# TrevorS/voxtral-mini-realtime-rs

Hardware: NVIDIA H100
Metric: decode_tokens_per_sec (higher is better)
Workload: dtype f32

## Files before the change

### voxtral_mini_realtime_rs_b200/csrc/capi.cu

```cuda
#include <cuda_profiler_api.h>
#include <cuda_runtime.h>

#include <cstring>
#include <memory>
#include <string>
#include <vector>

#include "audio_host.h"
#include "common.h"
#include "gguf.h"
#include "kernels.h"
#include "model.h"
#include "stream.h"
#include "tokenizer.h"

namespace vox {
static thread_local std::string g_last_error;
void set_last_error(const std::string &m) { g_last_error = m; }
}

using namespace vox;

#define VOX_API_BEGIN try {
#define VOX_API_END                                \
    }                                              \
    catch (const vox::Error &e) {                  \
        vox::set_last_error(e.what());             \
        return e.code;                             \
    }                                              \
    catch (const std::bad_alloc &) {               \
        vox::set_last_error("out of host memory"); \
        return VOX_ENOMEM;                         \
    }                                              \
    catch (const std::exception &e) {              \
        vox::set_last_error(e.what());             \
        return VOX_EINVAL;                         \
    }                                              \
    return VOX_OK;

#define REQUIRE(p) VOX_CHECK((p) != nullptr, VOX_EINVAL, "null argument: " #p)

struct vox_gguf { Gguf *g; };
struct vox_mel {
    int device;
    DeviceArena arena;
    MelTables tables;
    cudaStream_t st = nullptr;
    float *in = nullptr, *out = nullptr;
    size_t in_cap = 0, out_cap = 0;
};
struct vox_q4 {
    int device;
    DeviceArena arena;
    Q4Weight w;
    float *x = nullptr, *y = nullptr, *bias = nullptr;
    size_t x_cap = 0, y_cap = 0;
    TcWork wk;
    void *xt = nullptr;
    size_t xt_elems = 0;
    GemmWork gw;
};
struct vox_model { Model *m; };
struct vox_session { Session *s; };
struct vox_tokenizer { Tokenizer *t; };
struct vox_stream_pool { StreamPool *p; };

static void require_device(int device) {
    int n = 0;
    cudaError_t e = cudaGetDeviceCount(&n);
    VOX_CHECK(e == cudaSuccess && n > 0, VOX_ECUDA, "no CUDA device available (%s); this library has no CPU fallback",
              cudaGetErrorString(e));
    VOX_CHECK(device >= 0 && device < n, VOX_EINVAL, "device %d out of range (have %d)", device, n);
    CUDA_OK(cudaSetDevice(device));
}

extern "C" {

const char *vox_last_error(void) { return g_last_error.c_str(); }
int32_t vox_version(void) { return 100; }
int32_t vox_device_count(void) {
    int n = 0;
    if (cudaGetDeviceCount(&n) != cudaSuccess) { cudaGetLastError(); return 0; }
    return n;
}

int32_t vox_gguf_open(const char *path, vox_gguf **out) {
    VOX_API_BEGIN
    REQUIRE(path); REQUIRE(out);
    Gguf *g = Gguf::open_file(path);
    *out = new vox_gguf{g};
    VOX_API_END
}
int32_t vox_gguf_open_shards(const void *const *bufs, const size_t *lens, size_t n, vox_gguf **out) {
    VOX_API_BEGIN
    REQUIRE(bufs); REQUIRE(lens); REQUIRE(out);
    Gguf *g = Gguf::open_shards(bufs, lens, n);
    *out = new vox_gguf{g};
    VOX_API_END
}
int32_t vox_gguf_version(const vox_gguf *g, uint32_t *v) {
    VOX_API_BEGIN
    REQUIRE(g); REQUIRE(v);
    *v = g->g->version();
    VOX_API_END
}
int32_t vox_gguf_tensor_count(const vox_gguf *g, uint64_t *c) {
    VOX_API_BEGIN
    REQUIRE(g); REQUIRE(c);
    *c = g->g->tensor_count();
    VOX_API_END
}
int32_t vox_gguf_tensor_name(const vox_gguf *g, uint64_t i, const char **name) {
    VOX_API_BEGIN
    REQUIRE(g); REQUIRE(name);
    VOX_CHECK(i < g->g->names().size(), VOX_EINVAL, "tensor index %llu out of range", (unsigned long long)i);
    *name = g->g->names()[(size_t)i].c_str();
    VOX_API_END
}
int32_t vox_gguf_tensor_info(const vox_gguf *g, const char *name, uint32_t *dtype, uint32_t *ndim, uint64_t dims[4],
                             uint64_t *nbytes) {
    VOX_API_BEGIN
    REQUIRE(g); REQUIRE(name);
    const GgufTensorInfo *t = g->g->find(name);
    VOX_CHECK(t != nullptr, VOX_ENOTFOUND, "Tensor '%s' not found in GGUF", name);
    if (dtype) *dtype = t->dtype;
    if (ndim) *ndim = (uint32_t)t->dims.size();
    if (dims)
        for (size_t i = 0; i < 4; ++i) dims[i] = i < t->dims.size() ? t->dims[i] : 1;
    if (nbytes) *nbytes = t->byte_size();
    VOX_API_END
}
int32_t vox_gguf_tensor_data(vox_gguf *g, const char *name, void *dst, size_t cap) {
    VOX_API_BEGIN
    REQUIRE(g); REQUIRE(name); REQUIRE(dst);
    const GgufTensorInfo *t = g->g->find(name);
    VOX_CHECK(t != nullptr, VOX_ENOTFOUND, "Tensor '%s' not found in GGUF", name);
    VOX_CHECK(cap >= t->byte_size(), VOX_ECAPACITY, "buffer too small for '%s' (%zu < %llu)", name, cap,
              (unsigned long long)t->byte_size());
    g->g->read_tensor(*t, dst);
    VOX_API_END
}
void vox_gguf_close(vox_gguf *g) {
    if (!g) return;
    delete g->g;
    delete g;
}

int32_t vox_peak_normalize(float *s, size_t n, float target) {
    VOX_API_BEGIN
    if (n) REQUIRE(s);
    peak_normalize(s, n, target);
    VOX_API_END
}
void vox_pad_config_default(vox_pad_config *c) { if (c) pad_config_default(c); }
size_t vox_pad_audio_len(size_t n, const vox_pad_config *cfg) {
    vox_pad_config c;
    if (cfg) c = *cfg; else pad_config_default(&c);
    return pad_audio_len(n, c);
}
int32_t vox_pad_audio(const float *in, size_t n, const vox_pad_config *cfg, float *out, size_t cap, size_t *out_len) {
    VOX_API_BEGIN
    REQUIRE(out);
    if (n) REQUIRE(in);
    vox_pad_config c;
    if (cfg) c = *cfg; else pad_config_default(&c);
    VOX_CHECK(c.frame_rate > 0 && c.sample_rate > 0, VOX_EINVAL, "bad pad config");
    const size_t total = pad_audio_len(n, c);
    VOX_CHECK(cap >= total, VOX_ECAPACITY, "pad_audio: capacity %zu < %zu", cap, total);
    memset(out, 0, sizeof(float) * total);
    if (n) memcpy(out + pad_left(c), in, sizeof(float) * n);
    if (out_len) *out_len = total;
    VOX_API_END
}
int32_t vox_chunk_plan(size_t n, size_t max_mel_frames, size_t overlap, vox_chunk *out, size_t cap, size_t *n_chunks) {
    VOX_API_BEGIN
    REQUIRE(n_chunks);
    std::vector<vox_chunk> v = chunk_plan(n, max_mel_frames, overlap);
    *n_chunks = v.size();
    if (out) {
        VOX_CHECK(cap >= v.size(), VOX_ECAPACITY, "chunk_plan: capacity %zu < %zu", cap, v.size());
        for (size_t i = 0; i < v.size(); ++i) out[i] = v[i];
    }
    VOX_API_END
}
int32_t vox_stream_progress(size_t n_samples, int32_t ended, int32_t reshape_factor, int32_t prefix_len, int64_t out[5]) {
    VOX_API_BEGIN
    REQUIRE(out);
    VOX_CHECK(reshape_factor > 0 && prefix_len > 0, VOX_EINVAL, "stream_progress: reshape_factor %d / prefix_len %d must be positive",
              reshape_factor, prefix_len);
    stream_progress(n_samples, ended != 0, reshape_factor, prefix_len, out);
    VOX_API_END
}
int32_t vox_time_embedding(float t, int32_t dim, float *out) {
    VOX_API_BEGIN
    REQUIRE(out);
    VOX_CHECK(dim > 0 && dim % 2 == 0, VOX_EINVAL, "time_embedding: dim %d must be even", dim);
    time_embedding(t, dim, out);
    VOX_API_END
}

int32_t vox_mel_create(int32_t device, vox_mel **out) {
    VOX_API_BEGIN
    REQUIRE(out);
    require_device(device);
    std::unique_ptr<vox_mel> m(new vox_mel());
    m->device = device;
    m->arena.device = device;
    m->tables.build(m->arena);
    CUDA_OK(cudaStreamCreateWithFlags(&m->st, cudaStreamNonBlocking));
    *out = m.release();
    VOX_API_END
}
size_t vox_mel_num_frames(size_t n) { return mel_num_frames(n); }
int32_t vox_mel_compute_log(vox_mel *mel, const float *samples, size_t n, float *out, size_t cap) {
    VOX_API_BEGIN
    REQUIRE(mel); REQUIRE(out);
    if (n) REQUIRE(samples);
    const size_t frames = mel_num_frames(n);
    VOX_CHECK(cap >= frames * kMelBins, VOX_ECAPACITY, "mel: capacity %zu < %zu", cap, frames * kMelBins);
    if (frames == 0) return VOX_OK;
    CUDA_OK(cudaSetDevice(mel->device));
    if (n > mel->in_cap) {
        mel->in = mel->arena.alloc_n<float>(n);
        mel->in_cap = n;
    }
    if (frames * kMelBins > mel->out_cap) {
        mel->out = mel->arena.alloc_n<float>(frames * kMelBins);
        mel->out_cap = frames * kMelBins;
    }
    CUDA_OK(cudaMemcpyAsync(mel->in, samples, sizeof(float) * n, cudaMemcpyHostToDevice, mel->st));
    launch_mel(mel->in, 1, n, n, mel->tables.window, mel->tables.fb_vals, mel->tables.fb_start, mel->tables.fb_len,
               mel->tables.fb_stride, mel->out, (int)frames, 0, mel->st);
    CUDA_OK(cudaMemcpyAsync(out, mel->out, sizeof(float) * frames * kMelBins, cudaMemcpyDeviceToHost, mel->st));
    CUDA_OK(cudaStreamSynchronize(mel->st));
    VOX_API_END
}
int32_t vox_mel_compute_log_dev(vox_mel *mel, const float *samples_dev, size_t n, float *out_dev, int32_t layout,
                                void *stream) {
    VOX_API_BEGIN
    REQUIRE(mel); REQUIRE(samples_dev); REQUIRE(out_dev);
    VOX_CHECK(layout == 0 || layout == 1, VOX_EINVAL, "mel layout must be 0 or 1");
    CUDA_OK(cudaSetDevice(mel->device));
    const size_t frames = mel_num_frames(n);
    launch_mel(samples_dev, 1, n, n, mel->tables.window, mel->tables.fb_vals, mel->tables.fb_start, mel->tables.fb_len,
               mel->tables.fb_stride, out_dev, (int)frames, layout, stream ? (cudaStream_t)stream : mel->st);
    VOX_API_END
}
int32_t vox_mel_filterbank(const vox_mel *mel, float *out) {
    VOX_API_BEGIN
    REQUIRE(mel); REQUIRE(out);
    memcpy(out, mel->tables.fb_dense.data(), sizeof(float) * kMelBins * kMelFreqs);
    VOX_API_END
}
int32_t vox_mel_window(const vox_mel *mel, float *out) {
    VOX_API_BEGIN
    REQUIRE(mel); REQUIRE(out);
    memcpy(out, mel->tables.window_host.data(), sizeof(float) * kMelNfft);
    VOX_API_END
}
void vox_mel_free(vox_mel *mel) {
    if (!mel) return;
    cudaSetDevice(mel->device);
    if (mel->st) cudaStreamDestroy(mel->st);
    delete mel;
}

int32_t vox_q4_tensor_create(const uint8_t *bytes, size_t nbytes, int64_t n, int64_t k, int32_t device, vox_q4 **out) {
    VOX_API_BEGIN
    REQUIRE(bytes); REQUIRE(out);
    VOX_CHECK(n > 0 && k > 0, VOX_EINVAL, "Q4 tensor shape must be positive");
    VOX_CHECK((n * k) % 32 == 0, VOX_EINVAL, "Q4_0 requires element count divisible by 32, got %lld", (long long)(n * k));
    VOX_CHECK(k % 32 == 0, VOX_EINVAL, "Q4_0 rows must be block aligned: K=%lld is not a multiple of 32", (long long)k);
    const size_t expect = (size_t)(n * k / 32) * 18;
    VOX_CHECK(nbytes == expect, VOX_EINVAL, "Q4_0 byte count mismatch: expected %zu for %lld blocks, got %zu", expect,
              (long long)(n * k / 32), nbytes);
    require_device(device);
    std::unique_ptr<vox_q4> q(new vox_q4());
    q->device = device;
    q->arena.device = device;
    q->w = upload_q4(q->arena, {bytes}, {(int)n}, (int)k, false, true);
    q->wk = q4_matvec_tc_work_size(q->w.N, q->w.K);
    alloc_split_k(q->arena, q->wk);
    *out = q.release();
    VOX_API_END
}
int32_t vox_q4_tensor_shape(const vox_q4 *w, int64_t *n, int64_t *k) {
    VOX_API_BEGIN
    REQUIRE(w);
    if (n) *n = w->w.N;
    if (k) *k = w->w.K;
    VOX_API_END
}
int32_t vox_q4_tensor_dequantize(const vox_q4 *w, float *out) {
    VOX_API_BEGIN
    REQUIRE(w); REQUIRE(out);
    CUDA_OK(cudaSetDevice(w->device));
    const size_t nb = (size_t)w->w.N * (w->w.K / 32);
    std::vector<uint8_t> qs(nb * 16);
    std::vector<__half> ds(nb);
    CUDA_OK(cudaMemcpy(qs.data(), w->w.qs, qs.size(), cudaMemcpyDeviceToHost));
    CUDA_OK(cudaMemcpy(ds.data(), w->w.d, ds.size() * sizeof(__half), cudaMemcpyDeviceToHost));
    for (size_t b = 0; b < nb; ++b) {
        const float d = __half2float(ds[b]);
        for (int i = 0; i < 16; ++i) {
            const uint8_t byte = qs[b * 16 + i];
            out[b * 32 + i] = ((float)(byte & 0xF) - 8.0f) * d;
            out[b * 32 + i + 16] = ((float)(byte >> 4) - 8.0f) * d;
        }
    }
    VOX_API_END
}
static Q4Path g_q4_path = {!(getenv("VOX_MATVEC") && std::string(getenv("VOX_MATVEC")) == "simt"), true};
static Q4Scratch q4_scratch(vox_q4 *h, int rows) {
    if (rows > 8) {
        const size_t need = gemm_tc5_split_elems(rows, h->w.K);
        if (need > h->xt_elems) {
            h->xt = h->arena.alloc(need * 2);
            h->xt_elems = need;
        }
        if (!h->gw.partial) {
            h->gw = gemm_tc5_work_size();
            alloc_split_k(h->arena, h->gw);
        }
    }
    return Q4Scratch{h->xt, h->xt_elems, &h->gw, &h->wk};
}
int32_t vox_q4_set_matvec_mode(int32_t mode) {
    VOX_API_BEGIN
    VOX_CHECK(mode >= 0 && mode <= 3, VOX_EINVAL, "mode bits: 1 = SIMT matvec (M<=8), 2 = SIMT GEMM (M>8)");
    g_q4_path.matvec_tc = (mode & 1) == 0;
    g_q4_path.gemm_tc = (mode & 2) == 0;
    VOX_API_END
}
int32_t vox_q4_matmul(const vox_q4 *w, const float *x_dev, float *y_dev, int32_t b, int32_t m, const float *bias_dev,
                      void *stream) {
    VOX_API_BEGIN
    REQUIRE(w); REQUIRE(x_dev); REQUIRE(y_dev);
    VOX_CHECK(b > 0 && m > 0, VOX_EINVAL, "q4_matmul: B and M must be positive");
    CUDA_OK(cudaSetDevice(w->device));
    launch_q4_linear(w->w, x_dev, b * m, y_dev, w->w.N, bias_dev, nullptr, EPI_NONE, nullptr, nullptr, 0.0f, nullptr,
                     q4_scratch(const_cast<vox_q4 *>(w), b * m), g_q4_path, (cudaStream_t)stream);
    VOX_API_END
}
int32_t vox_q4_matmul_host(const vox_q4 *wc, const float *x, float *y, int32_t b, int32_t m, const float *bias) {
    VOX_API_BEGIN
    vox_q4 *w = const_cast<vox_q4 *>(wc);
    REQUIRE(w); REQUIRE(x); REQUIRE(y);
    VOX_CHECK(b > 0 && m > 0, VOX_EINVAL, "q4_matmul: B and M must be positive");
    CUDA_OK(cudaSetDevice(w->device));
    const size_t rows = (size_t)b * m, xn = rows * w->w.K, yn = rows * w->w.N;
    if (xn > w->x_cap) { w->x = w->arena.alloc_n<float>(xn); w->x_cap = xn; }
    if (yn > w->y_cap) { w->y = w->arena.alloc_n<float>(yn); w->y_cap = yn; }
    if (bias && !w->bias) w->bias = w->arena.alloc_n<float>(w->w.N);
    CUDA_OK(cudaMemcpyAsync(w->x, x, sizeof(float) * xn, cudaMemcpyHostToDevice, 0));
    if (bias) CUDA_OK(cudaMemcpyAsync(w->bias, bias, sizeof(float) * w->w.N, cudaMemcpyHostToDevice, 0));
    launch_q4_linear(w->w, w->x, (int)rows, w->y, w->w.N, bias ? w->bias : nullptr, nullptr, EPI_NONE, nullptr, nullptr,
                     0.0f, nullptr, q4_scratch(w, (int)rows), g_q4_path, 0);
    CUDA_OK(cudaMemcpyAsync(y, w->y, sizeof(float) * yn, cudaMemcpyDeviceToHost, 0));
    CUDA_OK(cudaStreamSynchronize(0));
    VOX_API_END
}
void vox_q4_tensor_free(vox_q4 *w) {
    if (!w) return;
    cudaSetDevice(w->device);
    delete w;
}

int32_t vox_dev_malloc(int32_t device, size_t bytes, void **p) {
    VOX_API_BEGIN
    REQUIRE(p);
    require_device(device);
    cudaError_t e = cudaMalloc(p, bytes ? bytes : 16);
    VOX_CHECK(e == cudaSuccess, VOX_ENOMEM, "cudaMalloc(%zu) failed: %s", bytes, cudaGetErrorString(e));
    VOX_API_END
}
int32_t vox_dev_free(int32_t device, void *p) {
    VOX_API_BEGIN
    require_device(device);
    CUDA_OK(cudaFree(p));
    VOX_API_END
}
int32_t vox_dev_upload(int32_t device, void *dst, const void *src, size_t bytes) {
    VOX_API_BEGIN
    require_device(device);
    CUDA_OK(cudaMemcpy(dst, src, bytes, cudaMemcpyHostToDevice));
    VOX_API_END
}
int32_t vox_dev_download(int32_t device, void *dst, const void *src, size_t bytes) {
    VOX_API_BEGIN
    require_device(device);
    CUDA_OK(cudaMemcpy(dst, src, bytes, cudaMemcpyDeviceToHost));
    VOX_API_END
}
int32_t vox_dev_sync(int32_t device) {
    VOX_API_BEGIN
    require_device(device);
    CUDA_OK(cudaDeviceSynchronize());
    VOX_API_END
}
int32_t vox_profiler_start(void) {
    VOX_API_BEGIN
    CUDA_OK(cudaProfilerStart());
    VOX_API_END
}
int32_t vox_profiler_stop(void) {
    VOX_API_BEGIN
    CUDA_OK(cudaProfilerStop());
    VOX_API_END
}
int32_t vox_host_alloc_pinned(size_t bytes, void **p) {
    VOX_API_BEGIN
    REQUIRE(p);
    cudaError_t e = cudaHostAlloc(p, bytes ? bytes : 16, cudaHostAllocDefault);
    VOX_CHECK(e == cudaSuccess, VOX_ECUDA, "cudaHostAlloc(%zu) failed: %s", bytes, cudaGetErrorString(e));
    VOX_API_END
}
int32_t vox_host_free_pinned(void *p) {
    VOX_API_BEGIN
    CUDA_OK(cudaFreeHost(p));
    VOX_API_END
}
int32_t vox_q4_matmul_bench(const vox_q4 *const *ws, int32_t n_w, int32_t m, int32_t iters, int32_t warmup, float *avg_ms) {
    VOX_API_BEGIN
    REQUIRE(ws); REQUIRE(avg_ms);
    VOX_CHECK(n_w > 0 && m > 0 && iters > 0, VOX_EINVAL, "bad bench arguments");
    const vox_q4 *w0 = ws[0];
    CUDA_OK(cudaSetDevice(w0->device));
    DeviceArena arena;
    arena.device = w0->device;
    const int K = w0->w.K, N = w0->w.N;
    std::vector<float> hx((size_t)m * K);
    for (size_t i = 0; i < hx.size(); ++i) hx[i] = sinf((float)i * 0.001f) * 0.1f;
    float *x = arena.upload(hx.data(), hx.size());
    float *y = arena.alloc_n<float>((size_t)m * N);
    cudaStream_t st;
    CUDA_OK(cudaStreamCreateWithFlags(&st, cudaStreamNonBlocking));
    cudaEvent_t e0, e1;
    CUDA_OK(cudaEventCreate(&e0));
    CUDA_OK(cudaEventCreate(&e1));
    auto run = [&](int i) {
        launch_q4_linear(ws[i % n_w]->w, x, m, y, ws[i % n_w]->w.N, nullptr, nullptr, EPI_NONE, nullptr, nullptr, 0.0f, nullptr,
                         Q4Scratch{}, g_q4_path, st);
    };
    for (int i = 0; i < warmup; ++i) run(i);
    CUDA_OK(cudaStreamSynchronize(st));
    CUDA_OK(cudaEventRecord(e0, st));
    for (int i = 0; i < iters; ++i) run(i);
    CUDA_OK(cudaEventRecord(e1, st));
    CUDA_OK(cudaStreamSynchronize(st));
    float ms = 0;
    CUDA_OK(cudaEventElapsedTime(&ms, e0, e1));
    *avg_ms = ms / iters;
    cudaEventDestroy(e0);
    cudaEventDestroy(e1);
    cudaStreamDestroy(st);
    VOX_API_END
}

int32_t vox_model_load_gguf_handle(vox_gguf *g, int32_t device, vox_model **out) {
    VOX_API_BEGIN
    REQUIRE(g); REQUIRE(out);
    Model *m = Model::load(*g->g, device);
    *out = new vox_model{m};
    VOX_API_END
}
int32_t vox_model_load_gguf(const char *path, int32_t device, vox_model **out) {
    VOX_API_BEGIN
    REQUIRE(path); REQUIRE(out);
    std::unique_ptr<Gguf> g(Gguf::open_file(path));
    Model *m = Model::load(*g, device);
    *out = new vox_model{m};
    VOX_API_END
}
int32_t vox_model_get_info(const vox_model *m, vox_model_info *info) {
    VOX_API_BEGIN
    REQUIRE(m); REQUIRE(info);
    *info = m->m->info;
    VOX_API_END
}
void vox_model_free(vox_model *m) {
    if (!m) return;
    cudaSetDevice(m->m->device);
    delete m->m;
    delete m;
}

int32_t vox_session_create(vox_model *m, int32_t max_batch, int32_t max_mel_frames, vox_session **out) {
    VOX_API_BEGIN
    REQUIRE(m); REQUIRE(out);
    Session *s = Session::create(m->m, max_batch, max_mel_frames);
    *out = new vox_session{s};
    VOX_API_END
}
int32_t vox_session_set_delay(vox_session *s, float delay) {
    VOX_API_BEGIN
    REQUIRE(s);
    s->s->set_delay(delay);
    VOX_API_END
}
static void require_any_device();
int32_t vox_session_set_delays(vox_session *s, const float *delays, int32_t b) {
    VOX_API_BEGIN
    require_any_device();
    REQUIRE(s); REQUIRE(delays);
    s->s->set_delays(delays, b);
    VOX_API_END
}

static void upload_mel(Session *s, const float *mel, int b, int t) {
    const vox_model_info &c = s->m->info;
    VOX_CHECK(b >= 1 && b <= s->max_batch, VOX_EINVAL, "batch %d exceeds session max_batch %d", b, s->max_batch);
    VOX_CHECK(t >= 1 && t <= s->max_mel_frames, VOX_EINVAL, "mel frames %d exceed session max_mel_frames %d", t,
              s->max_mel_frames);
    CUDA_OK(cudaSetDevice(s->m->device));
    CUDA_OK(cudaMemcpyAsync(s->mel, mel, sizeof(float) * (size_t)b * c.n_mels * t, cudaMemcpyHostToDevice, s->st));
    launch_transpose_mel(s->mel, s->mel_tm, b, c.n_mels, t, s->st);
}

int32_t vox_encode_audio(vox_session *sh, const float *mel, int32_t b, int32_t t, float *audio_embeds, size_t cap,
                         int32_t *seq_len) {
    VOX_API_BEGIN
    REQUIRE(sh); REQUIRE(mel);
    Session *s = sh->s;
    upload_mel(s, mel, b, t);
    s->encode(b, t);
    const size_t n = (size_t)b * s->cur_S4 * s->m->info.dec_dim;
    if (audio_embeds) {
        VOX_CHECK(cap >= n, VOX_ECAPACITY, "audio_embeds capacity %zu < %zu", cap, n);
        if (n) CUDA_OK(cudaMemcpyAsync(audio_embeds, s->audio, sizeof(float) * n, cudaMemcpyDeviceToHost, s->st));
    }
    CUDA_OK(cudaStreamSynchronize(s->st));
    if (seq_len) *seq_len = s->cur_S4;
    VOX_API_END
}

static void fill_timings(Session *s, vox_timings *tm) {
    if (!tm) return;
    float pre = 0, enc = 0, dec = 0, pf = 0;
    CUDA_OK(cudaEventElapsedTime(&pf, s->ev[2], s->ev[4]));
    tm->prefill_ms = pf;
    CUDA_OK(cudaEventElapsedTime(&pre, s->ev[0], s->ev[1]));
    CUDA_OK(cudaEventElapsedTime(&enc, s->ev[1], s->ev[2]));
    CUDA_OK(cudaEventElapsedTime(&dec, s->ev[2], s->ev[3]));
    tm->preprocess_ms = pre;
    tm->encode_ms = enc;
    tm->decode_ms = dec;
    tm->total_ms = pre + enc + dec;
}

int32_t vox_transcribe_streaming(vox_session *sh, const float *mel, int32_t b, int32_t t, int32_t *out_ids, size_t cap,
                                 int32_t *n_out, vox_timings *tm) {
    VOX_API_BEGIN
    REQUIRE(sh); REQUIRE(mel); REQUIRE(out_ids); REQUIRE(n_out);
    Session *s = sh->s;
    CUDA_OK(cudaSetDevice(s->m->device));
    CUDA_OK(cudaEventRecord(s->ev[0], s->st));
    upload_mel(s, mel, b, t);
    CUDA_OK(cudaEventRecord(s->ev[1], s->st));
    *n_out = s->transcribe_from_mel(b, t, out_ids, cap, tm, true);
    fill_timings(s, tm);
    VOX_API_END
}

static int32_t transcribe_pcm_impl(Session *s, const float *host, const float *dev, int b, size_t n, int normalize,
                                   int32_t *out_ids, size_t cap, int32_t *n_out, vox_timings *tm) {
    const vox_model_info &c = s->m->info;
    VOX_CHECK(b >= 1 && b <= s->max_batch, VOX_EINVAL, "batch %d exceeds session max_batch %d", b, s->max_batch);
    VOX_CHECK(n >= 1, VOX_EINVAL, "empty audio");
    CUDA_OK(cudaSetDevice(s->m->device));
    vox_pad_config pc;
    pad_config_default(&pc);
    const size_t padded = pad_audio_len(n, pc), left = pad_left(pc);
    const size_t frames = mel_num_frames(padded);
    VOX_CHECK(frames >= 1, VOX_EINVAL, "Audio too short to produce mel frames");
    VOX_CHECK(frames <= (size_t)s->max_mel_frames, VOX_EINVAL,
              "audio needs %zu mel frames > session max_mel_frames %d (chunk it: vox_chunk_plan)", frames, s->max_mel_frames);
    if ((size_t)b * padded > s->pcm_pad_cap) {
        s->pcm_pad = s->arena.alloc_n<float>((size_t)b * padded);
        s->pcm_pad_cap = (size_t)b * padded;
    }
    CUDA_OK(cudaEventRecord(s->ev[0], s->st));
    const float *src = dev;
    if (host) {
        if ((size_t)b * n > s->pcm_cap) {
            s->pcm = s->arena.alloc_n<float>((size_t)b * n);
            s->pcm_cap = (size_t)b * n;
        }
        CUDA_OK(cudaMemcpyAsync(s->pcm, host, sizeof(float) * (size_t)b * n, cudaMemcpyHostToDevice, s->st));
        src = s->pcm;
    }
    launch_peak_normalize_pad(src, b, n, 0.95f, normalize, s->pcm_pad, padded, left, s->peak_scale, s->st);
    launch_mel(s->pcm_pad, b, padded, padded, s->m->mel.window, s->m->mel.fb_vals, s->m->mel.fb_start, s->m->mel.fb_len,
               s->m->mel.fb_stride, s->mel_tm, (int)frames, 0, s->st);
    CUDA_OK(cudaEventRecord(s->ev[1], s->st));
    (void)c;
    *n_out = s->transcribe_from_mel(b, (int)frames, out_ids, cap, tm, true);
    fill_timings(s, tm);
    return VOX_OK;
}

int32_t vox_transcribe_pcm(vox_session *sh, const float *samples, int32_t b, size_t n, int32_t normalize,
                           int32_t *out_ids, size_t cap, int32_t *n_out, vox_timings *tm) {
    VOX_API_BEGIN
    REQUIRE(sh); REQUIRE(samples); REQUIRE(out_ids); REQUIRE(n_out);
    return transcribe_pcm_impl(sh->s, samples, nullptr, b, n, normalize, out_ids, cap, n_out, tm);
    VOX_API_END
}
int32_t vox_transcribe_pcm_dev(vox_session *sh, const float *samples_dev, int32_t b, size_t n, int32_t *out_ids,
                               size_t cap, int32_t *n_out, vox_timings *tm) {
    VOX_API_BEGIN
    REQUIRE(sh); REQUIRE(samples_dev); REQUIRE(out_ids); REQUIRE(n_out);
    return transcribe_pcm_impl(sh->s, nullptr, samples_dev, b, n, 1, out_ids, cap, n_out, tm);
    VOX_API_END
}

int32_t vox_generate_step_with_cache(vox_session *sh, const int32_t *ids, int32_t b, int32_t m, float *logits, size_t cap) {
    VOX_API_BEGIN
    REQUIRE(sh); REQUIRE(ids); REQUIRE(logits);
    Session *s = sh->s;
    const vox_model_info &c = s->m->info;
    VOX_CHECK(b >= 1 && b <= s->max_batch, VOX_EINVAL, "batch %d exceeds session max_batch %d", b, s->max_batch);
    VOX_CHECK(m >= 1 && m <= s->M_max, VOX_EINVAL, "M=%d out of range [1,%d]", m, s->M_max);
    VOX_CHECK(s->cache_len + m <= s->out_ld, VOX_EINVAL, "KV cache full (%d + %d > %d)", s->cache_len, m, s->out_ld);
    for (int i = 0; i < b * m; ++i)
        VOX_CHECK(ids[i] >= 0 && ids[i] < c.vocab, VOX_EINVAL, "token id %d out of range", ids[i]);
    const size_t n = (size_t)b * m * c.vocab;
    VOX_CHECK(cap >= n, VOX_ECAPACITY, "logits capacity %zu < %zu", cap, n);
    CUDA_OK(cudaSetDevice(s->m->device));
    if (n > s->logits_all_cap) {
        s->logits_all = s->arena.alloc_n<float>(n);
        s->logits_all_cap = n;
    }
    CUDA_OK(cudaMemcpyAsync(s->d_ids, ids, sizeof(int) * (size_t)b * m, cudaMemcpyHostToDevice, s->st));
    launch_embed(s->m->tok_emb, s->d_ids, nullptr, 0, b, m, nullptr, s->x_dec, s->fused_decode(b * m) ? s->ssq_x : nullptr, s->st);
    const bool pending = s->decoder_forward(b, m);
    s->lm_head_rows(b * m, pending, s->logits_all);
    launch_advance(s->d_pos, m, nullptr, 0, b, s->st);
    CUDA_OK(cudaMemcpyAsync(logits, s->logits_all, sizeof(float) * n, cudaMemcpyDeviceToHost, s->st));
    CUDA_OK(cudaStreamSynchronize(s->st));
    s->cache_len += m;
    VOX_API_END
}
int32_t vox_forward_streaming(vox_session *sh, const float *mel, int32_t b, int32_t t, const int32_t *ids, int32_t n_ids,
                              float *logits, size_t cap) {
    VOX_API_BEGIN
    REQUIRE(sh); REQUIRE(mel); REQUIRE(ids); REQUIRE(logits);
    Session *s = sh->s;
    const vox_model_info &c = s->m->info;
    upload_mel(s, mel, b, t);
    s->encode(b, t);
    const int S4 = s->cur_S4;
    VOX_CHECK(n_ids == S4, VOX_EINVAL, "forward_streaming needs one token id per audio position (%d), got %d", S4, n_ids);
    VOX_CHECK(S4 <= s->out_ld, VOX_EINVAL, "sequence %d exceeds the session KV capacity %d", S4, s->out_ld);
    for (int i = 0; i < b * n_ids; ++i) VOX_CHECK(ids[i] >= 0 && ids[i] < c.vocab, VOX_EINVAL, "token id %d out of range", ids[i]);
    const size_t n = (size_t)b * S4 * c.vocab;
    VOX_CHECK(cap >= n, VOX_ECAPACITY, "logits capacity %zu < %zu", cap, n);
    s->reset();
    const int Mc = s->M_max;
    const size_t chunk_floats = (size_t)b * Mc * c.vocab;
    if (chunk_floats > s->logits_all_cap) {
        s->logits_all = s->arena.alloc_n<float>(chunk_floats);
        s->logits_all_cap = chunk_floats;
    }
    std::vector<int> chunk_ids;
    for (int p0 = 0; p0 < S4; p0 += Mc) {
        const int m = std::min(Mc, S4 - p0);
        chunk_ids.resize((size_t)b * m);
        for (int bb = 0; bb < b; ++bb)
            for (int i = 0; i < m; ++i) chunk_ids[(size_t)bb * m + i] = ids[(size_t)bb * S4 + p0 + i];
        CUDA_OK(cudaMemcpyAsync(s->d_ids, chunk_ids.data(), sizeof(int) * chunk_ids.size(), cudaMemcpyHostToDevice, s->st));
        launch_embed(s->m->tok_emb, s->d_ids, s->audio, S4, b, m, s->d_pos, s->x_dec, s->fused_decode(b * m) ? s->ssq_x : nullptr, s->st);
        const bool pending = s->decoder_forward(b, m);
        s->lm_head_rows(b * m, pending, s->logits_all);
        launch_advance(s->d_pos, m, nullptr, 0, b, s->st);
        for (int bb = 0; bb < b; ++bb)
            CUDA_OK(cudaMemcpyAsync(logits + ((size_t)bb * S4 + p0) * c.vocab, s->logits_all + (size_t)bb * m * c.vocab,
                                    sizeof(float) * (size_t)m * c.vocab, cudaMemcpyDeviceToHost, s->st));
        CUDA_OK(cudaStreamSynchronize(s->st));
    }
    s->cache_len = S4;
    VOX_API_END
}

static void record_step_scores(Session *s, int b) {
    s->scores_k = s->top_k;
    s->scores_b = b;
    s->scores_n = 1;
    s->scores_pos.assign(s->out_rows.begin(), s->out_rows.begin() + b);
    for (int &p : s->scores_pos) p -= 1;
}

int32_t vox_prefill(vox_session *sh, const int32_t *ids, int32_t b, int32_t m, int32_t add_audio, int32_t *next_tok) {
    VOX_API_BEGIN
    REQUIRE(sh); REQUIRE(ids);
    Session *s = sh->s;
    const vox_model_info &c = s->m->info;
    VOX_CHECK(b >= 1 && b <= s->max_batch, VOX_EINVAL, "batch %d exceeds session max_batch %d", b, s->max_batch);
    VOX_CHECK(m >= 1 && m <= s->M_max, VOX_EINVAL, "M=%d out of range [1,%d]", m, s->M_max);
    VOX_CHECK(s->cache_len + m <= s->out_ld, VOX_EINVAL, "KV cache full (%d + %d > %d)", s->cache_len, m, s->out_ld);
    if (add_audio)
        VOX_CHECK(b == s->cur_B && s->cache_len + m <= s->cur_S4, VOX_EINVAL,
                  "add_audio: positions %d..%d need audio embeddings of %d streams (have %d positions for %d streams; call vox_encode_audio first)",
                  s->cache_len, s->cache_len + m, b, s->cur_S4, s->cur_B);
    for (int i = 0; i < b * m; ++i) VOX_CHECK(ids[i] >= 0 && ids[i] < c.vocab, VOX_EINVAL, "token id %d out of range", ids[i]);
    CUDA_OK(cudaSetDevice(s->m->device));
    s->prefill(b, m, ids, add_audio != 0);
    s->cache_len += m;
    record_step_scores(s, b);
    if (next_tok) CUDA_OK(cudaMemcpyAsync(next_tok, s->d_tok, sizeof(int) * b, cudaMemcpyDeviceToHost, s->st));
    CUDA_OK(cudaStreamSynchronize(s->st));
    VOX_API_END
}
int32_t vox_decode_step(vox_session *sh, const int32_t *tok, int32_t b, int32_t add_audio, int32_t *next_tok) {
    VOX_API_BEGIN
    REQUIRE(sh);
    Session *s = sh->s;
    const vox_model_info &c = s->m->info;
    VOX_CHECK(b >= 1 && b <= s->max_batch, VOX_EINVAL, "batch %d exceeds session max_batch %d", b, s->max_batch);
    VOX_CHECK(s->cache_len + 1 <= s->out_ld, VOX_EINVAL, "KV cache full (%d + 1 > %d)", s->cache_len, s->out_ld);
    if (add_audio)
        VOX_CHECK(b == s->cur_B && s->cache_len < s->cur_S4, VOX_EINVAL,
                  "add_audio: position %d has no audio embedding (%d positions, %d streams encoded)", s->cache_len, s->cur_S4, s->cur_B);
    CUDA_OK(cudaSetDevice(s->m->device));
    if (tok) {
        for (int i = 0; i < b; ++i) VOX_CHECK(tok[i] >= 0 && tok[i] < c.vocab, VOX_EINVAL, "token id %d out of range", tok[i]);
        CUDA_OK(cudaMemcpyAsync(s->d_tok, tok, sizeof(int) * b, cudaMemcpyHostToDevice, s->st));
    }
    s->decode_step(b, add_audio != 0);
    s->mega_steps_host += 1;
    s->cache_len += 1;
    record_step_scores(s, b);
    if (next_tok) CUDA_OK(cudaMemcpyAsync(next_tok, s->d_tok, sizeof(int) * b, cudaMemcpyDeviceToHost, s->st));
    if (next_tok || tok) CUDA_OK(cudaStreamSynchronize(s->st));
    VOX_API_END
}
static_assert(VOX_MAX_TOP_K == TOPK_MAX, "the score buffers hold VOX_MAX_TOP_K entries per position");
int32_t vox_session_set_top_k(vox_session *s, int32_t k) {
    VOX_API_BEGIN
    REQUIRE(s);
    s->s->set_top_k(k);
    VOX_API_END
}
int32_t vox_session_token_scores(vox_session *sh, int32_t *top_ids, float *top_logprobs, size_t cap, int32_t *b, int32_t *n,
                                 int32_t *k) {
    VOX_API_BEGIN
// ... 327 lines not shown
```

### voxtral_mini_realtime_rs_b200/csrc/gemm_tc5.cu

```cuda
#include <cuda_fp16.h>

#include "common.h"
#include "kernels.h"

namespace vox {

void tc_count_launch(const char *name);

namespace {

constexpr int G5_WGS = 4;
constexpr int G5_THREADS = G5_WGS * 128;
constexpr int G5_BM = 128;
constexpr int G5_BN = 128;
constexpr int G5_BK = 64;
constexpr int G5_TILE_BYTES = G5_BM * G5_BK * 2;
constexpr int G5_PIECES = 2;
constexpr int G5_STAGES = 3;
constexpr int G5_STAGE_BYTES = 2 * G5_PIECES * G5_TILE_BYTES;
constexpr int G5_SMEM_BYTES = G5_STAGES * G5_STAGE_BYTES;
constexpr float G5_WSCALE = 256.0f;

__device__ __forceinline__ uint32_t smem_u32(const void *p) { return (uint32_t)__cvta_generic_to_shared(p); }
__device__ __forceinline__ void mbar_init(uint64_t *bar, uint32_t count) {
    asm volatile("mbarrier.init.shared::cta.b64 [%0], %1;\n" ::"r"(smem_u32(bar)), "r"(count));
}
__device__ __forceinline__ void mbar_expect_tx(uint64_t *bar, uint32_t bytes) {
    asm volatile("mbarrier.arrive.expect_tx.shared::cta.b64 _, [%0], %1;\n" ::"r"(smem_u32(bar)), "r"(bytes) : "memory");
}
__device__ __forceinline__ void mbar_wait(uint64_t *bar, uint32_t parity) {
    asm volatile(
        "{\n"
        ".reg .pred p;\n"
        "G5_WAIT:\n"
        "mbarrier.try_wait.parity.shared::cta.b64 p, [%0], %1;\n"
        "@p bra G5_DONE;\n"
        "bra G5_WAIT;\n"
        "G5_DONE:\n"
        "}\n" ::"r"(smem_u32(bar)), "r"(parity) : "memory");
}
__device__ __forceinline__ void bulk_g2s(void *dst_smem, const void *src_gmem, uint32_t bytes, uint64_t *bar) {
    asm volatile("cp.async.bulk.shared::cluster.global.mbarrier::complete_tx::bytes [%0], [%1], %2, [%3];\n" ::"r"(
                     smem_u32(dst_smem)),
                 "l"(src_gmem), "r"(bytes), "r"(smem_u32(bar))
                 : "memory");
}

__device__ __forceinline__ uint64_t gmma_desc(uint32_t smem_addr, uint32_t lbo_bytes, uint32_t sbo_bytes) {
    uint64_t d = 0;
    d |= (uint64_t)((smem_addr >> 4) & 0x3FFF);
    d |= (uint64_t)((lbo_bytes >> 4) & 0x3FFF) << 16;
    d |= (uint64_t)((sbo_bytes >> 4) & 0x3FFF) << 32;
    return d;
}
__device__ __forceinline__ void wgmma_m64n64k16(float (&d)[32], uint64_t adesc, uint64_t bdesc) {
    asm volatile(
        "{\n"
        ".reg .pred p;\n"
        "setp.ne.b32 p, %34, 0;\n"
        "wgmma.mma_async.sync.aligned.m64n64k16.f32.f16.f16 "
        "{%0,%1,%2,%3,%4,%5,%6,%7,%8,%9,%10,%11,%12,%13,%14,%15,%16,%17,%18,%19,%20,%21,%22,%23,%24,%25,%26,%27,%28,%29,%30,%31}, "
        "%32, %33, p, 1, 1, 0, 0;\n"
        "}\n"
        : "+f"(d[0]), "+f"(d[1]), "+f"(d[2]), "+f"(d[3]), "+f"(d[4]), "+f"(d[5]), "+f"(d[6]), "+f"(d[7]), "+f"(d[8]),
          "+f"(d[9]), "+f"(d[10]), "+f"(d[11]), "+f"(d[12]), "+f"(d[13]), "+f"(d[14]), "+f"(d[15]), "+f"(d[16]),
          "+f"(d[17]), "+f"(d[18]), "+f"(d[19]), "+f"(d[20]), "+f"(d[21]), "+f"(d[22]), "+f"(d[23]), "+f"(d[24]),
          "+f"(d[25]), "+f"(d[26]), "+f"(d[27]), "+f"(d[28]), "+f"(d[29]), "+f"(d[30]), "+f"(d[31])
        : "l"(adesc), "l"(bdesc), "r"(1)
        : "memory");
}
__device__ __forceinline__ void wgmma_fence() { asm volatile("wgmma.fence.sync.aligned;\n" ::: "memory"); }
__device__ __forceinline__ void wgmma_commit() { asm volatile("wgmma.commit_group.sync.aligned;\n" ::: "memory"); }
template <int N>
__device__ __forceinline__ void wgmma_wait() { asm volatile("wgmma.wait_group.sync.aligned %0;\n" ::"n"(N) : "memory"); }
__device__ __forceinline__ void acc_fence(float (&d)[32]) {
#pragma unroll
    for (int i = 0; i < 32; ++i) asm volatile("" : "+f"(d[i])::"memory");
}

__device__ __forceinline__ uint32_t g5_pack_f16x2(const float v0, const float v1) {
    const uint32_t b0 = __float_as_uint(v0), b1 = __float_as_uint(v1);
    const uint32_t em = ((b0 >> 13) & 0x00007FFFu) | ((b1 << 3) & 0x7FFF0000u);
    const uint32_t sg = ((b0 >> 16) & 0x00008000u) | (b1 & 0x80000000u);
    return em | sg;
}

struct G5Args {
    const uint4 *qs;
    const __half *ds;
    int N, K, M;
    const __half *xt;
    const float *oscale;
    int TT, KC;
    float *y;
    int ldy;
    const float *bias, *res;
    int SK, KCs;
    float *partial;
    int *counters;
};

template <int EPI>
__global__ void __launch_bounds__(G5_THREADS, 1) gemm_tc5_kernel(const G5Args a) {
    extern __shared__ __align__(1024) unsigned char smem[];
    __shared__ __align__(8) uint64_t full_bar[G5_STAGES];
    const int tid = threadIdx.x, warp = tid >> 5, lane = tid & 31, wg = tid >> 7;
    const int f0 = blockIdx.x * G5_BM, tt = blockIdx.y, tok0 = tt * G5_BN;
    const int bpr = a.K >> 5;
    const int kc_begin = blockIdx.z * a.KCs, kc_end = min(a.KC, kc_begin + a.KCs), nk = kc_end - kc_begin;
    const size_t xt_piece = (size_t)a.TT * a.KC * (G5_TILE_BYTES / 2);

    auto fetch_x = [&](int it) {
        const int s = it % G5_STAGES;
        unsigned char *dst = smem + (size_t)s * G5_STAGE_BYTES + G5_PIECES * G5_TILE_BYTES;
        mbar_expect_tx(&full_bar[s], G5_PIECES * G5_TILE_BYTES);
#pragma unroll
        for (int p = 0; p < G5_PIECES; ++p) {
            const __half *src = a.xt + p * xt_piece + ((size_t)tt * a.KC + kc_begin + it) * (G5_TILE_BYTES / 2);
            bulk_g2s(dst + p * G5_TILE_BYTES, src, G5_TILE_BYTES, &full_bar[s]);
        }
    };
    if (tid == 0) {
        for (int s = 0; s < G5_STAGES; ++s) mbar_init(&full_bar[s], 1);
        asm volatile("fence.mbarrier_init.release.cluster;\n" ::: "memory");
        if (nk > 0) fetch_x(0);
    }
    __syncthreads();

    const int drow = tid >> 2, dblk = (tid >> 1) & 1, dhalf = tid & 1;
    const int gn = f0 + drow;
    const int fq = wg & 1, tq = wg >> 1;
    float acc[32];
#pragma unroll
    for (int i = 0; i < 32; ++i) acc[i] = 0.0f;

    uint4 q_cur = make_uint4(0x88888888u, 0x88888888u, 0x88888888u, 0x88888888u);
    __half d_cur = __float2half(0.0f);
    if (gn < a.N && nk > 0) {
        const size_t blk = (size_t)gn * bpr + (size_t)kc_begin * 2 + dblk;
        q_cur = __ldg(a.qs + blk);
        d_cur = __ldg(a.ds + blk);
    }
    for (int it = 0; it < nk; ++it) {
        const int kc = kc_begin + it, s = it % G5_STAGES;
        unsigned char *stage = smem + (size_t)s * G5_STAGE_BYTES;
        const uint4 q = q_cur;
        const float dd = __half2float(d_cur) * G5_WSCALE * 1.92592994438723585305597794258492732e-34f;
        if (gn < a.N && kc + 1 < kc_end) {
            const size_t blk = (size_t)gn * bpr + (size_t)(kc + 1) * 2 + dblk;
            q_cur = __ldg(a.qs + blk);
            d_cur = __ldg(a.ds + blk);
        }
        const uint32_t w4[4] = {q.x, q.y, q.z, q.w};
        uint32_t ph[8], pl[8];
#pragma unroll
        for (int wi = 0; wi < 4; ++wi) {
            const uint32_t nib = dhalf ? (w4[wi] >> 4) : w4[wi];
            float hi[4], lo[4];
#pragma unroll
            for (int t = 0; t < 4; ++t) {
                const uint32_t n = (nib >> (8 * t)) & 0xFu;
                const float w = __fmul_rn(__fsub_rn(__uint_as_float(0x4B000000u | n), 8388616.0f), dd);
                const float c = __fmul_rn(w, 8193.0f);
                hi[t] = __fsub_rn(c, __fsub_rn(c, w));
                lo[t] = __fsub_rn(w, hi[t]);
            }
            ph[wi * 2 + 0] = g5_pack_f16x2(hi[0], hi[1]);
            ph[wi * 2 + 1] = g5_pack_f16x2(hi[2], hi[3]);
            pl[wi * 2 + 0] = g5_pack_f16x2(lo[0], lo[1]);
            pl[wi * 2 + 1] = g5_pack_f16x2(lo[2], lo[3]);
        }
        wgmma_wait<1>();
        unsigned char *thi = stage, *tlo = stage + G5_TILE_BYTES;
#pragma unroll
        for (int c = 0; c < 2; ++c) {
            const int off = (dblk * 4 + dhalf * 2 + c) * (G5_BM * 16) + drow * 16;
            *reinterpret_cast<uint4 *>(thi + off) = make_uint4(ph[4 * c + 0], ph[4 * c + 1], ph[4 * c + 2], ph[4 * c + 3]);
            *reinterpret_cast<uint4 *>(tlo + off) = make_uint4(pl[4 * c + 0], pl[4 * c + 1], pl[4 * c + 2], pl[4 * c + 3]);
        }
        asm volatile("fence.proxy.async.shared::cta;\n" ::: "memory");
        __syncthreads();
        if (tid == 0 && it + 1 < nk) fetch_x(it + 1);
        mbar_wait(&full_bar[s], (uint32_t)((it / G5_STAGES) & 1));
        const uint32_t wbase = smem_u32(stage) + fq * 64 * 16, xbase = smem_u32(stage + G5_PIECES * G5_TILE_BYTES) + tq * 64 * 16;
        const uint32_t lbo = G5_BM * 16, sbo = 128;
        acc_fence(acc);
        wgmma_fence();
#pragma unroll
        for (int ks = 0; ks < G5_BK / 16; ++ks) {
            const uint32_t koff = (uint32_t)ks * 2u * lbo;
            const uint64_t whi = gmma_desc(wbase + 0 * G5_TILE_BYTES + koff, lbo, sbo);
            const uint64_t wlo = gmma_desc(wbase + 1 * G5_TILE_BYTES + koff, lbo, sbo);
            const uint64_t xh = gmma_desc(xbase + 0 * G5_TILE_BYTES + koff, lbo, sbo);
            const uint64_t xm = gmma_desc(xbase + 1 * G5_TILE_BYTES + koff, lbo, sbo);
            wgmma_m64n64k16(acc, wlo, xh);
            wgmma_m64n64k16(acc, whi, xm);
            wgmma_m64n64k16(acc, whi, xh);
        }
        wgmma_commit();
        acc_fence(acc);
    }
    wgmma_wait<0>();
    acc_fence(acc);

    {
        __shared__ int is_last;
        const int frow = fq * 64 + (warp & 3) * 16 + (lane >> 2);
        const int tcol = tq * 64 + (lane & 3) * 2;
        auto fr = [&](int i) { return frow + ((i >> 1) & 1) * 8; };
        auto tc = [&](int i) { return tcol + (i >> 2) * 8 + (i & 1); };
        auto emit = [&](float (&r)[32]) {
#pragma unroll
            for (int i = 0; i < 32; ++i) {
                const int feat = f0 + fr(i), tok = tok0 + tc(i);
                float v = r[i] * a.oscale[tok];
                if (EPI == EPI_SILU_MUL) {
                    const float other = __shfl_xor_sync(0xffffffffu, v, 4);
                    if (((lane >> 2) & 1) == 0 && tok < a.M && feat + 1 < a.N)
                        a.y[(size_t)tok * a.ldy + (feat >> 1)] = (v / (1.0f + expf(-v))) * other;
                } else if (tok < a.M && feat < a.N) {
                    if (a.bias) v += a.bias[feat];
                    if (EPI == EPI_RESIDUAL) v += a.res[(size_t)tok * a.ldy + feat];
                    if (EPI == EPI_GELU) v = 0.5f * v * (1.0f + erff(v * 0.70710678118654752440f));
                    a.y[(size_t)tok * a.ldy + feat] = v;
                }
            }
        };
        if (a.SK <= 1) {
            emit(acc);
        } else {
            const int tile_id = blockIdx.y * gridDim.x + blockIdx.x, n_tile = gridDim.x * gridDim.y;
            float *ptile = a.partial + ((size_t)blockIdx.z * n_tile + tile_id) * (G5_BM * G5_BN);
#pragma unroll
            for (int i = 0; i < 32; ++i) __stcg(ptile + (size_t)tc(i) * G5_BM + fr(i), acc[i]);
            __syncthreads();
            if (tid == 0) {
                __threadfence();
                const int old = atomicAdd(&a.counters[tile_id], 1);
                const int last = (old == a.SK - 1);
                if (last) {
                    a.counters[tile_id] = 0;
                    __threadfence();
                }
                is_last = last;
            }
            __syncthreads();
            if (is_last != 0) {
#pragma unroll
                for (int i = 0; i < 32; ++i) {
                    float v = 0.0f;
                    for (int z = 0; z < a.SK; ++z)
                        v += __ldcg(a.partial + ((size_t)z * n_tile + tile_id) * (G5_BM * G5_BN) + (size_t)tc(i) * G5_BM + fr(i));
                    acc[i] = v;
                }
                emit(acc);
            }
        }
    }
}

template <bool ROWS>
__device__ __forceinline__ void split_tiles_body(const float *__restrict__ x, int M, int K, const float *__restrict__ gamma,
                                                 const float *__restrict__ ada_shared, const AdaRows &ada_rows, float eps,
                                                 __half *__restrict__ xt, float *__restrict__ oscale, int TT, int KC, int BN) {
    __shared__ float ssq_part[32][8], max_part[32][8];
    __shared__ float rms_s[8], sc_s[8];
    const int r8 = threadIdx.x & 7, cth = threadIdx.x >> 3;
    const int row = blockIdx.x * 8 + r8;
    const int nchunk = K >> 3;
    const bool valid = row < M;
    const float *xr = x + (size_t)(valid ? row : 0) * K;
    const float *__restrict__ ada = ROWS ? (valid ? ada_rows.row(row) : nullptr) : ada_shared;
    {
        float ssq = 0.0f, mx = 0.0f;
        if (valid)
            for (int c = cth; c < nchunk; c += 32) {
                const float4 v0 = *reinterpret_cast<const float4 *>(xr + c * 8);
                const float4 v1 = *reinterpret_cast<const float4 *>(xr + c * 8 + 4);
                float v[8] = {v0.x, v0.y, v0.z, v0.w, v1.x, v1.y, v1.z, v1.w};
#pragma unroll
                for (int e = 0; e < 8; ++e) {
                    ssq = fmaf(v[e], v[e], ssq);
                    float g = v[e];
                    if (gamma) {
                        g *= gamma[c * 8 + e];
                        if (ada) g *= ada[c * 8 + e];
                    }
                    mx = fmaxf(mx, fabsf(g));
                }
            }
        ssq_part[cth][r8] = ssq;
        max_part[cth][r8] = mx;
        __syncthreads();
        if (threadIdx.x < 8) {
            float s = 0.0f, m = 0.0f;
            for (int i = 0; i < 32; ++i) {
                s += ssq_part[i][threadIdx.x];
                m = fmaxf(m, max_part[i][threadIdx.x]);
            }
            const float rms = gamma ? sqrtf(s / (float)K + eps) : 1.0f;
            rms_s[threadIdx.x] = rms;
            m = m / rms * 1.0001f;
            int e = (int)((__float_as_uint(m) >> 23) & 0xFF) - 127;
            if (!(m > 0.0f) || m > 3.0e38f) e = 7;
            e = e < -100 ? -100 : (e > 100 ? 100 : e);
            sc_s[threadIdx.x] = __uint_as_float((uint32_t)(7 - e + 127) << 23);
            const int grow = blockIdx.x * 8 + threadIdx.x;
            oscale[grow] = __uint_as_float((uint32_t)(e - 7 - 8 + 127) << 23);
        }
        __syncthreads();
    }
    const float rms = rms_s[r8], sc = sc_s[r8];
    const int tt = row / BN, rin = row % BN;
    const size_t tile_el = (size_t)BN * G5_BK;
    const size_t piece = (size_t)TT * KC * tile_el;
    for (int c = cth; c < nchunk; c += 32) {
        float v[8] = {0.f, 0.f, 0.f, 0.f, 0.f, 0.f, 0.f, 0.f};
        if (valid) {
            const float4 v0 = *reinterpret_cast<const float4 *>(xr + c * 8);
            const float4 v1 = *reinterpret_cast<const float4 *>(xr + c * 8 + 4);
            v[0] = v0.x; v[1] = v0.y; v[2] = v0.z; v[3] = v0.w; v[4] = v1.x; v[5] = v1.y; v[6] = v1.z; v[7] = v1.w;
            if (gamma) {
#pragma unroll
                for (int e = 0; e < 8; ++e) {
                    v[e] = (v[e] / rms) * gamma[c * 8 + e];
                    if (ada) v[e] *= ada[c * 8 + e];
                }
            }
        }
        uint32_t p[2][4];
#pragma unroll
        for (int e = 0; e < 4; ++e) {
            const float f0 = v[2 * e] * sc, f1 = v[2 * e + 1] * sc;
            const __half2 h = __floats2half2_rn(f0, f1);
            const float2 hf = __half22float2(h);
            const __half2 m = __floats2half2_rn(f0 - hf.x, f1 - hf.y);
            p[0][e] = *reinterpret_cast<const uint32_t *>(&h);
            p[1][e] = *reinterpret_cast<const uint32_t *>(&m);
        }
        const size_t off = ((size_t)tt * KC + (c >> 3)) * tile_el + (size_t)((c & 7) * BN + rin) * 8;
#pragma unroll
        for (int s = 0; s < G5_PIECES; ++s)
            *reinterpret_cast<uint4 *>(xt + s * piece + off) = make_uint4(p[s][0], p[s][1], p[s][2], p[s][3]);
    }
}

__global__ void __launch_bounds__(256) split_tiles_kernel(const float *__restrict__ x, int M, int K, const float *__restrict__ gamma,
                                                          const float *__restrict__ ada, float eps, __half *__restrict__ xt,
                                                          float *__restrict__ oscale, int TT, int KC, int BN) {
    split_tiles_body<false>(x, M, K, gamma, ada, AdaRows{}, eps, xt, oscale, TT, KC, BN);
}

__global__ void __launch_bounds__(256) split_tiles_rows_kernel(const float *__restrict__ x, int M, int K, const float *__restrict__ gamma,
                                                               const AdaRows ada_rows, float eps, __half *__restrict__ xt,
                                                               float *__restrict__ oscale, int TT, int KC, int BN) {
    split_tiles_body<true>(x, M, K, gamma, nullptr, ada_rows, eps, xt, oscale, TT, KC, BN);
}

}

bool gemm_tc5_supported(const Q4Weight &w, int M) { return w.N % G5_BM == 0 && w.K % G5_BK == 0 && M >= 1; }

static size_t g5_tiles_elems(int M, int K) {
    const size_t TT = (size_t)(M + G5_BN - 1) / G5_BN;
    return G5_PIECES * TT * (size_t)(K / G5_BK) * ((size_t)G5_BN * G5_BK);
}
size_t gemm_tc5_split_elems(int M, int K) {
    const size_t TT = (size_t)(M + G5_BN - 1) / G5_BN;
    return g5_tiles_elems(M, K) + 2 * TT * G5_BN + 16;
}
GemmWork gemm_tc5_work_size() {
    GemmWork w;
    w.partial_floats = (size_t)VOX_NUM_SMS * G5_BM * G5_BN;
    w.n_counters = 128;
    return w;
}
static float *g5_oscale_ptr(void *xt, int M, int K) {
    size_t off = g5_tiles_elems(M, K) * 2;
    off = (off + 15) & ~(size_t)15;
    return reinterpret_cast<float *>(reinterpret_cast<unsigned char *>(xt) + off);
}

void launch_split_tiles(const float *x, int M, int K, const float *gamma, const float *ada, float eps, void *xt,
                        cudaStream_t st, const AdaRows &ada_rows) {
    VOX_CHECK(K % G5_BK == 0, VOX_EINVAL, "split_tiles: K=%d not a multiple of 64", K);
    const int TT = (M + G5_BN - 1) / G5_BN, KC = K / G5_BK;
    if (ada_rows.rows)
        split_tiles_rows_kernel<<<TT * (G5_BN / 8), 256, 0, st>>>(x, M, K, gamma, ada_rows, eps, (__half *)xt, g5_oscale_ptr(xt, M, K),
                                                                  TT, KC, G5_BN);
    else
        split_tiles_kernel<<<TT * (G5_BN / 8), 256, 0, st>>>(x, M, K, gamma, ada, eps, (__half *)xt, g5_oscale_ptr(xt, M, K), TT, KC,
                                                             G5_BN);
    tc_count_launch("split_tiles");
}

void launch_q4_gemm_tc5(const Q4Weight &w, const void *xt, int M, float *y, int ldy, const float *bias, const float *res,
                        int epi, const GemmWork *gw, cudaStream_t st) {
    VOX_CHECK(gemm_tc5_supported(w, M), VOX_EINVAL, "gemm_tc5: unsupported shape N=%d K=%d", w.N, w.K);
    G5Args a{};
    a.qs = w.qs;
    a.ds = w.d;
    a.N = w.N;
    a.K = w.K;
    a.M = M;
    a.xt = (const __half *)xt;
    a.oscale = g5_oscale_ptr(const_cast<void *>(xt), M, w.K);
    a.TT = (M + G5_BN - 1) / G5_BN;
    a.KC = w.K / G5_BK;
    a.y = y;
    a.ldy = ldy;
    a.bias = bias;
    a.res = res;
    const size_t smem = (size_t)G5_SMEM_BYTES;
    const int tiles = (w.N / G5_BM) * a.TT;
    int SK = 1;
    if (gw && gw->partial && gw->counters && tiles < VOX_NUM_SMS * 2 / 3) {
        SK = VOX_NUM_SMS / tiles;
        SK = SK > 8 ? 8 : SK;
        while (SK > 1 && a.KC / SK < 4) --SK;
        while (SK > 1 && ((size_t)SK * tiles * G5_BM * G5_BN > gw->partial_floats || tiles > gw->n_counters)) --SK;
    }
    a.KCs = (a.KC + SK - 1) / SK;
    SK = (a.KC + a.KCs - 1) / a.KCs;
    a.SK = SK;
    a.partial = SK > 1 ? gw->partial : nullptr;
    a.counters = SK > 1 ? gw->counters : nullptr;
    dim3 grid(w.N / G5_BM, a.TT, SK);
#define G5_CASE(E)                                                                      \
    case E: {                                                                           \
        static SmemAttr attr;                                                           \
        smem_attr_check(ensure_dyn_smem(gemm_tc5_kernel<E>, smem, attr), "gemm_tc5");   \
        gemm_tc5_kernel<E><<<grid, G5_THREADS, smem, st>>>(a);                          \
        break;                                                                          \
    }
    switch (epi) {
        G5_CASE(EPI_NONE)
        G5_CASE(EPI_RESIDUAL)
        G5_CASE(EPI_SILU_MUL)
        G5_CASE(EPI_GELU)
        default: fail(VOX_EINVAL, "bad epilogue");
    }
#undef G5_CASE
    tc_count_launch("gemm_tc5");
}

}
```

### voxtral_mini_realtime_rs_b200/csrc/kernels.cu

```cuda
#include "kernels.h"

#include <atomic>
#include <cfloat>
#include <cmath>
#include <string>

#include "common.h"

namespace vox {

void smem_attr_check(cudaError_t e, const char *what) {
    if (e != cudaSuccess) fail(VOX_ECUDA, fmt("cudaFuncSetAttribute(%s, MaxDynamicSharedMemorySize): %s", what, cudaGetErrorString(e)));
}


static std::atomic<uint64_t> g_launches{0};
uint64_t kernel_launch_count() { return g_launches.load(); }
void add_graph_launches(int64_t n) { g_launches.fetch_add((uint64_t)n, std::memory_order_relaxed); }

static inline void post_launch(const char *name) {
    g_launches.fetch_add(1, std::memory_order_relaxed);
    cudaError_t e = cudaGetLastError();
    if (e != cudaSuccess) fail(VOX_ECUDA, fmt("%s launch failed: %s", name, cudaGetErrorString(e)));
}
// ... 135 lines not shown
                        y[(size_t)m * ldy + r1] = v;
                    }
                }
            }
        }
    };

    if (n_chunks == 1) {
        const int nb = stage(0);
        for (int rg = blockIdx.x; rg < n_rg; rg += gridDim.x) {
            float acc0[M], acc1[M];
#pragma unroll
            for (int m = 0; m < M; ++m) acc0[m] = acc1[m] = 0.0f;
            accumulate(rg, 0, nb, acc0, acc1);
            epilogue(rg, acc0, acc1);
        }
    } else {
        const int rg = blockIdx.x;
        float acc0[M], acc1[M];
#pragma unroll
        for (int m = 0; m < M; ++m) acc0[m] = acc1[m] = 0.0f;
        for (int c = 0; c < n_chunks; ++c) {
            const int nb = stage(c);
            accumulate(rg, c, nb, acc0, acc1);
            __syncthreads();
        }
        epilogue(rg, acc0, acc1);
    }
}

template <int M, int EPI>
static void matvec_launch_t(const Q4Weight &w, const float *x, float *y, int ldy, const float *bias,
                            const float *res, cudaStream_t st) {
    const int bpr = w.K / 32;
    const size_t budget = 96 * 1024;
    int kcb = (int)(budget / ((size_t)M * (XPAD + 1) * sizeof(float)));
    if (kcb >= bpr) kcb = bpr;
    else kcb = (kcb / 32) * 32;
    const int n_chunks = (bpr + kcb - 1) / kcb;
    const size_t smem = (size_t)M * kcb * (XPAD + 1) * sizeof(float);
    static SmemAttr attr;
    smem_attr_check(ensure_dyn_smem(q4_matvec_kernel<M, EPI>, 100 * 1024, attr), "q4_matvec");
    const int n_rg = (w.N + MV_ROWS - 1) / MV_ROWS;
    int grid = n_rg;
    if (n_chunks == 1 && grid > VOX_NUM_SMS * 8) grid = VOX_NUM_SMS * 8;
    q4_matvec_kernel<M, EPI><<<grid, MV_THREADS, smem, st>>>(w.qs, w.d, w.N, w.K, x, y, ldy, bias, res, kcb, n_chunks);
    post_launch("q4_matvec");
}

template <int M>
static void matvec_launch_m(const Q4Weight &w, const float *x, float *y, int ldy, const float *bias,
                            const float *res, int epi, cudaStream_t st) {
    switch (epi) {
        case EPI_NONE: matvec_launch_t<M, EPI_NONE>(w, x, y, ldy, bias, res, st); break;
        case EPI_RESIDUAL: matvec_launch_t<M, EPI_RESIDUAL>(w, x, y, ldy, bias, res, st); break;
        case EPI_SILU_MUL: matvec_launch_t<M, EPI_SILU_MUL>(w, x, y, ldy, bias, res, st); break;
        case EPI_GELU: matvec_launch_t<M, EPI_GELU>(w, x, y, ldy, bias, res, st); break;
        default: fail(VOX_EINVAL, "bad epilogue");
    }
}

void launch_q4_matvec(const Q4Weight &w, const float *x, int M, float *y, int ldy, const float *bias,
                      const float *res, int epi, cudaStream_t st) {
    VOX_CHECK(M >= 1 && M <= 8, VOX_EINVAL, "q4_matvec: M=%d out of range", M);
    VOX_CHECK(w.K % 32 == 0, VOX_EINVAL, "q4_matvec: K=%d not a multiple of 32", w.K);
    switch (M) {
        case 1: matvec_launch_m<1>(w, x, y, ldy, bias, res, epi, st); break;
        case 2: matvec_launch_m<2>(w, x, y, ldy, bias, res, epi, st); break;
        case 3: matvec_launch_m<3>(w, x, y, ldy, bias, res, epi, st); break;
        case 4: matvec_launch_m<4>(w, x, y, ldy, bias, res, epi, st); break;
        case 5: matvec_launch_m<5>(w, x, y, ldy, bias, res, epi, st); break;
        case 6: matvec_launch_m<6>(w, x, y, ldy, bias, res, epi, st); break;
        case 7: matvec_launch_m<7>(w, x, y, ldy, bias, res, epi, st); break;
        default: matvec_launch_m<8>(w, x, y, ldy, bias, res, epi, st); break;
    }
}

constexpr int GB_M = 64, GB_N = 64, GB_K = 32, GB_PAD = 4, GB_THREADS = 256;

struct GemmArgs {
    const float *a;
    int M, N, K, lda;
    const uint4 *qs;
    const __half *ds;
    const float *wf;
    float *y;
    int ldy;
    const float *bias;
    const float *res;
    int T_in, T_out, C_in;
    int t_off;
    int in0;
};

template <int BMODE, int AMODE, int EPI>
__global__ void __launch_bounds__(GB_THREADS) gemm_kernel(const GemmArgs p) {
    __shared__ __align__(16) float As[GB_K][GB_M + GB_PAD];
    __shared__ __align__(16) float Ws[GB_K][GB_N + GB_PAD];
    const int tid = threadIdx.x;
    const int tx = tid & 15, ty = tid >> 4;
    const int m0 = blockIdx.y * GB_M, n0 = blockIdx.x * GB_N;
    const int bpr = p.K >> 5;
    float c[4][4];
#pragma unroll
    for (int i = 0; i < 4; ++i)
#pragma unroll
        for (int j = 0; j < 4; ++j) c[i][j] = 0.0f;

    for (int k0 = 0; k0 < p.K; k0 += GB_K) {
#pragma unroll
        for (int it = 0; it < 2; ++it) {
            const int idx = tid + it * GB_THREADS;
            const int row = idx >> 3, kq = idx & 7;
            const int gm = m0 + row;
            float4 v = make_float4(0.f, 0.f, 0.f, 0.f);
            if (gm < p.M) {
                if (AMODE == 0) {
                    v = *reinterpret_cast<const float4 *>(p.a + (size_t)gm * p.lda + k0 + kq * 4);
                } else {
                    const int b = gm / p.T_out, t = gm - b * p.T_out;
                    const int tap = k0 / p.C_in, c0 = k0 - tap * p.C_in;
                    const int tin = 2 * (t + p.t_off) - 1 + tap;
                    if (tin >= 0 && tin < p.T_in)
                        v = *reinterpret_cast<const float4 *>(p.a + ((size_t)b * p.T_in + (tin - p.in0)) * p.C_in + c0 + kq * 4);
                }
            }
            As[kq * 4 + 0][row] = v.x;
            As[kq * 4 + 1][row] = v.y;
            As[kq * 4 + 2][row] = v.z;
            As[kq * 4 + 3][row] = v.w;
        }
        if (BMODE == 0) {
            const int row = tid >> 2, wi = tid & 3;
            const int gn = n0 + row;
            float lo[4] = {0.f, 0.f, 0.f, 0.f}, hi[4] = {0.f, 0.f, 0.f, 0.f};
            if (gn < p.N) {
                const size_t blk = (size_t)gn * bpr + (k0 >> 5);
                const uint32_t w = reinterpret_cast<const uint32_t *>(p.qs + blk)[wi];
                const float dd = __half2float(p.ds[blk]);
#pragma unroll
                for (int t = 0; t < 4; ++t) {
                    const uint32_t byte = (w >> (8 * t)) & 0xFFu;
                    lo[t] = ((float)(byte & 0xFu) - 8.0f) * dd;
                    hi[t] = ((float)(byte >> 4) - 8.0f) * dd;
                }
            }
#pragma unroll
            for (int t = 0; t < 4; ++t) {
                Ws[wi * 4 + t][row] = lo[t];
                Ws[16 + wi * 4 + t][row] = hi[t];
            }
        } else {
#pragma unroll
            for (int it = 0; it < 2; ++it) {
                const int idx = tid + it * GB_THREADS;
                const int row = idx >> 3, kq = idx & 7;
                const int gn = n0 + row;
                float4 v = make_float4(0.f, 0.f, 0.f, 0.f);
                if (gn < p.N) v = *reinterpret_cast<const float4 *>(p.wf + (size_t)gn * p.K + k0 + kq * 4);
                Ws[kq * 4 + 0][row] = v.x;
                Ws[kq * 4 + 1][row] = v.y;
                Ws[kq * 4 + 2][row] = v.z;
                Ws[kq * 4 + 3][row] = v.w;
            }
        }
        __syncthreads();
#pragma unroll
        for (int k = 0; k < GB_K; ++k) {
            const float4 a = *reinterpret_cast<const float4 *>(&As[k][ty * 4]);
            const float4 b = *reinterpret_cast<const float4 *>(&Ws[k][tx * 4]);
            const float av[4] = {a.x, a.y, a.z, a.w};
            const float bv[4] = {b.x, b.y, b.z, b.w};
#pragma unroll
            for (int i = 0; i < 4; ++i)
#pragma unroll
                for (int j = 0; j < 4; ++j) c[i][j] = fmaf(av[i], bv[j], c[i][j]);
        }
        __syncthreads();
    }
#pragma unroll
    for (int i = 0; i < 4; ++i) {
        const int gm = m0 + ty * 4 + i;
        if (gm >= p.M) continue;
        if (EPI == EPI_SILU_MUL) {
#pragma unroll
            for (int j = 0; j < 4; j += 2) {
                const int gn = n0 + tx * 4 + j;
                if (gn + 1 < p.N) p.y[(size_t)gm * p.ldy + (gn >> 1)] = silu_f(c[i][j]) * c[i][j + 1];
            }
        } else {
#pragma unroll
            for (int j = 0; j < 4; ++j) {
                const int gn = n0 + tx * 4 + j;
                if (gn >= p.N) continue;
                float v = c[i][j] + (p.bias ? p.bias[gn] : 0.0f);
                if (EPI == EPI_RESIDUAL) v += p.res[(size_t)gm * p.ldy + gn];
                if (EPI == EPI_GELU) v = gelu_erf(v);
                p.y[(size_t)gm * p.ldy + gn] = v;
            }
        }
    }
}

template <int BMODE, int AMODE>
static void gemm_launch(const GemmArgs &p, int epi, cudaStream_t st) {
    dim3 grid((p.N + GB_N - 1) / GB_N, (p.M + GB_M - 1) / GB_M);
    switch (epi) {
        case EPI_NONE: gemm_kernel<BMODE, AMODE, EPI_NONE><<<grid, GB_THREADS, 0, st>>>(p); break;
        case EPI_RESIDUAL: gemm_kernel<BMODE, AMODE, EPI_RESIDUAL><<<grid, GB_THREADS, 0, st>>>(p); break;
        case EPI_SILU_MUL: gemm_kernel<BMODE, AMODE, EPI_SILU_MUL><<<grid, GB_THREADS, 0, st>>>(p); break;
        case EPI_GELU: gemm_kernel<BMODE, AMODE, EPI_GELU><<<grid, GB_THREADS, 0, st>>>(p); break;
        default: fail(VOX_EINVAL, "bad epilogue");
    }
    post_launch("gemm");
}

void launch_q4_gemm(const Q4Weight &w, const float *a, int M, float *y, int ldy, const float *bias,
                    const float *res, int epi, cudaStream_t st) {
    VOX_CHECK(w.K % 32 == 0, VOX_EINVAL, "q4_gemm: K=%d not a multiple of 32", w.K);
    if (M <= 0) return;
    GemmArgs p{};
    p.a = a; p.M = M; p.N = w.N; p.K = w.K; p.lda = w.K;
    p.qs = w.qs; p.ds = w.d; p.y = y; p.ldy = ldy; p.bias = bias; p.res = res;
    gemm_launch<0, 0>(p, epi, st);
}

void launch_conv2_gemm(const float *in, const float *w, const float *bias, float *out, int B, int T_in,
                       int T_out, int C_in, int C_out, cudaStream_t st, int t_off, int in0) {
    VOX_CHECK(C_in % 32 == 0, VOX_EINVAL, "conv2: C_in=%d not a multiple of 32", C_in);
    VOX_CHECK((t_off == 0 && in0 == 0) || B == 1, VOX_EINVAL, "conv2: a frame offset needs B == 1");
    VOX_CHECK(in0 <= 2 * t_off - 1 || in0 == 0, VOX_EINVAL, "conv2: input row %d is no longer resident", 2 * t_off - 1);
    if (B * T_out <= 0) return;
    GemmArgs p{};
    p.a = in; p.M = B * T_out; p.N = C_out; p.K = 3 * C_in; p.lda = 0;
    p.wf = w; p.y = out; p.ldy = C_out; p.bias = bias; p.res = nullptr;
    p.T_in = T_in; p.T_out = T_out; p.C_in = C_in; p.t_off = t_off; p.in0 = in0;
    gemm_launch<1, 1>(p, EPI_GELU, st);
}

__global__ void transpose_mel_kernel(const float *__restrict__ in, float *__restrict__ out, int C, int T) {
    __shared__ float tile[32][33];
    const int b = blockIdx.z, c0 = blockIdx.y * 32, t0 = blockIdx.x * 32;
    for (int i = threadIdx.y; i < 32; i += blockDim.y) {
        const int c = c0 + i, t = t0 + threadIdx.x;
        tile[i][threadIdx.x] = (c < C && t < T) ? in[((size_t)b * C + c) * T + t] : 0.0f;
    }
    __syncthreads();
    for (int i = threadIdx.y; i < 32; i += blockDim.y) {
        const int t = t0 + i, c = c0 + threadIdx.x;
        if (t < T && c < C) out[((size_t)b * T + t) * C + c] = tile[threadIdx.x][i];
    }
}
void launch_transpose_mel(const float *in, float *out, int B, int C, int T, cudaStream_t st) {
    dim3 grid((T + 31) / 32, (C + 31) / 32, B), block(32, 8);
    transpose_mel_kernel<<<grid, block, 0, st>>>(in, out, C, T);
    post_launch("transpose_mel");
}

__device__ __forceinline__ void rmsnorm_row(const float *__restrict__ xr, const float *__restrict__ gamma,
                                            const float *__restrict__ scale, float *__restrict__ yr, int dim, float eps) {
    __shared__ float red[32];
    float s = 0.0f;
    for (int i = threadIdx.x; i < dim; i += blockDim.x) s = fmaf(xr[i], xr[i], s);
    s = warp_sum(s);
    if ((threadIdx.x & 31) == 0) red[threadIdx.x >> 5] = s;
    __syncthreads();
    if (threadIdx.x < 32) {
        float v = threadIdx.x < (blockDim.x >> 5) ? red[threadIdx.x] : 0.0f;
        v = warp_sum(v);
        if (threadIdx.x == 0) red[0] = v;
    }
    __syncthreads();
    const float rms = sqrtf(red[0] / (float)dim + eps);
    for (int i = threadIdx.x; i < dim; i += blockDim.x) {
        float v = (xr[i] / rms) * gamma[i];
        if (scale) v *= scale[i];
        yr[i] = v;
    }
}

__global__ void rmsnorm_kernel(const float *__restrict__ x, const float *__restrict__ gamma,
                               const float *__restrict__ scale, float *__restrict__ y, int dim, float eps) {
    rmsnorm_row(x + (size_t)blockIdx.x * dim, gamma, scale, y + (size_t)blockIdx.x * dim, dim, eps);
}

__global__ void rmsnorm_rows_kernel(const float *__restrict__ x, const float *__restrict__ gamma, const AdaRows ada_rows,
                                    float *__restrict__ y, int dim, float eps) {
    rmsnorm_row(x + (size_t)blockIdx.x * dim, gamma, ada_rows.row(blockIdx.x), y + (size_t)blockIdx.x * dim, dim, eps);
}

void launch_rmsnorm(const float *x, const float *gamma, const float *scale, float *y, int rows, int dim,
                    float eps, cudaStream_t st, const AdaRows &ada_rows) {
    if (rows <= 0) return;
    if (ada_rows.rows) rmsnorm_rows_kernel<<<rows, 256, 0, st>>>(x, gamma, ada_rows, y, dim, eps);
    else rmsnorm_kernel<<<rows, 256, 0, st>>>(x, gamma, scale, y, dim, eps);
    post_launch("rmsnorm");
}

void launch_q4_linear(const Q4Weight &w, const float *x, int M, float *y, int ldy, const float *bias, const float *res,
                      int epi, const float *gamma, const float *ada, float eps, float *tmp, const Q4Scratch &sc,
                      const Q4Path &path, cudaStream_t st, const AdaRows &ada_rows) {
    VOX_CHECK(!ada_rows.rows || (gamma && !ada), VOX_EINVAL, "q4_linear: per-row ADA vectors need a norm and no shared vector");
    if (M > 8 && path.gemm_tc && gemm_tc5_supported(w, M) && gemm_tc5_split_elems(M, w.K) <= sc.xt_elems) {
        launch_split_tiles(x, M, w.K, gamma, ada, gamma ? eps : 0.0f, sc.xt, st, ada_rows);
        launch_q4_gemm_tc5(w, sc.xt, M, y, ldy, bias, res, epi, sc.gw, st);
        return;
    }
    const bool tc = M <= 8 && path.matvec_tc && w.qs_tc;
    AdaRows rows = ada_rows;
    if (gamma && !(tc && sc.tc && sc.tc->ssq_in)) {
        launch_rmsnorm(x, gamma, ada, tmp, M, w.K, eps, st, rows);
        x = tmp;
        gamma = ada = nullptr;
        rows = AdaRows{};
    }
    if (tc) launch_q4_matvec_tc_ex(w, x, M, y, ldy, bias, res, epi, gamma, ada, gamma ? eps : 0.0f, sc.tc, st, rows);
    else if (M <= 8) launch_q4_matvec(w, x, M, y, ldy, bias, res, epi, st);
    else launch_q4_gemm(w, x, M, y, ldy, bias, res, epi, st);
}

__global__ void rope_inplace_kernel(float *buf, int ld, int q_off, int n_q, int k_off, int n_k, int hd,
                                    int seq, int pos0, const float *__restrict__ cos_t,
                                    const float *__restrict__ sin_t) {
    const int r = blockIdx.x;
    const int pos = pos0 + (r % seq);
    const int half = hd >> 1;
    float *row = buf + (size_t)r * ld;
    const int total = (n_q + n_k) * half;
    for (int i = threadIdx.x; i < total; i += blockDim.x) {
        const int h = i / half, p = i - h * half;
        float *v = (h < n_q) ? row + q_off + h * hd + 2 * p : row + k_off + (h - n_q) * hd + 2 * p;
        const float c = cos_t[(size_t)pos * half + p], s = sin_t[(size_t)pos * half + p];
        const float xr = v[0], xi = v[1];
        v[0] = xr * c - xi * s;
        v[1] = xr * s + xi * c;
    }
}

void launch_rope_inplace(float *buf, int rows, int ld, int q_off, int n_q, int k_off, int n_k, int hd,
                         int seq, int pos0, const float *cos_t, const float *sin_t, cudaStream_t st) {
    if (rows <= 0) return;
    rope_inplace_kernel<<<rows, 256, 0, st>>>(buf, ld, q_off, n_q, k_off, n_k, hd, seq, pos0, cos_t, sin_t);
    post_launch("rope");
}

constexpr int EA_BQ = 32, EA_BK = 64, EA_THREADS = 128;

template <int HD>
__global__ void __launch_bounds__(EA_THREADS)
enc_attention_kernel(const float *__restrict__ qkv, float *__restrict__ out, int S, int H, int ld, int q_off,
                     int k_off, int v_off, int window, float scale) {
    extern __shared__ __align__(16) float sm[];
    float *Qs = sm;
    float *Ks = Qs + EA_BQ * (HD + 1);
    float *Vs = Ks + EA_BK * (HD + 1);
    float *Ps = Vs + EA_BK * HD;
    const int b = blockIdx.z, h = blockIdx.y, q0 = blockIdx.x * EA_BQ;
    const int tid = threadIdx.x, r = tid >> 2, c = tid & 3;
    constexpr int DQ = HD / 4;
    const float *base = qkv + (size_t)b * S * ld;
    for (int i = tid; i < EA_BQ * HD; i += EA_THREADS) {
        const int rr = i / HD, d = i - rr * HD;
        const int gi = q0 + rr;
        Qs[rr * (HD + 1) + d] = gi < S ? base[(size_t)gi * ld + q_off + h * HD + d] : 0.0f;
    }
    const int gi = q0 + r;
    float o[DQ];
#pragma unroll
    for (int d = 0; d < DQ; ++d) o[d] = 0.0f;
    float m_run = -INFINITY, l_run = 0.0f;
    const int q_last = min(q0 + EA_BQ - 1, S - 1);
    int j_begin = q0 - window;
    if (j_begin < 0) j_begin = 0;
    j_begin = (j_begin / EA_BK) * EA_BK;
    for (int j0 = j_begin; j0 <= q_last; j0 += EA_BK) {
        __syncthreads();
        for (int i = tid; i < EA_BK * HD; i += EA_THREADS) {
            const int kk = i / HD, d = i - kk * HD;
            const int gj = j0 + kk;
            float kv = 0.0f, vv = 0.0f;
            if (gj < S) {
                kv = base[(size_t)gj * ld + k_off + h * HD + d];
                vv = base[(size_t)gj * ld + v_off + h * HD + d];
            }
            Ks[kk * (HD + 1) + d] = kv;
            Vs[kk * HD + d] = vv;
        }
        __syncthreads();
        float s[16];
        float m_t = -INFINITY;
#pragma unroll
        for (int jj = 0; jj < 16; ++jj) {
            const int kk = c + 4 * jj;
            const int gj = j0 + kk;
            const float *qr = Qs + r * (HD + 1);
            const float *kr = Ks + kk * (HD + 1);
            float acc = 0.0f;
#pragma unroll 16
            for (int d = 0; d < HD; ++d) acc = fmaf(qr[d], kr[d], acc);
            const bool valid = (gj < S) && (gj <= gi) && (gi - gj <= window);
            s[jj] = valid ? acc * scale : -INFINITY;
            m_t = fmaxf(m_t, s[jj]);
        }
        m_t = fmaxf(m_t, __shfl_xor_sync(0xffffffffu, m_t, 1));
        m_t = fmaxf(m_t, __shfl_xor_sync(0xffffffffu, m_t, 2));
        const float m_new = fmaxf(m_run, m_t);
        float alpha = 1.0f, psum = 0.0f;
        if (m_new == -INFINITY) {
#pragma unroll
            for (int jj = 0; jj < 16; ++jj) Ps[r * (EA_BK + 1) + c + 4 * jj] = 0.0f;
        } else {
            alpha = expf(m_run - m_new);
#pragma unroll
            for (int jj = 0; jj < 16; ++jj) {
                const float pv = expf(s[jj] - m_new);
                psum += pv;
                Ps[r * (EA_BK + 1) + c + 4 * jj] = pv;
            }
        }
        psum += __shfl_xor_sync(0xffffffffu, psum, 1);
        psum += __shfl_xor_sync(0xffffffffu, psum, 2);
        l_run = l_run * alpha + psum;
        m_run = m_new;
#pragma unroll
        for (int d = 0; d < DQ; ++d) o[d] *= alpha;
        __syncwarp();
        for (int kk = 0; kk < EA_BK; ++kk) {
            const float pv = Ps[r * (EA_BK + 1) + kk];
            const float *vr = Vs + kk * HD + c;
#pragma unroll
            for (int d = 0; d < DQ; ++d) o[d] = fmaf(pv, vr[4 * d], o[d]);
        }
    }
    if (gi < S) {
        const float inv = 1.0f / l_run;
        float *orow = out + ((size_t)b * S + gi) * (H * HD) + h * HD + c;
#pragma unroll
        for (int d = 0; d < DQ; ++d) orow[4 * d] = o[d] * inv;
    }
}

void launch_enc_attention(const float *qkv, float *out, int B, int S, int H, int hd, int ld, int q_off,
                          int k_off, int v_off, int window, float scale, cudaStream_t st) {
    if (S <= 0) return;
    dim3 grid((S + EA_BQ - 1) / EA_BQ, H, B);
    const size_t smem = (size_t)(EA_BQ * (hd + 1) + EA_BK * (hd + 1) + EA_BK * hd + EA_BQ * (EA_BK + 1)) * sizeof(float);
#define ENC_ATTN_CASE(HD)                                                                                   \
    case HD: {                                                                                              \
        static SmemAttr attr;                                                                               \
        smem_attr_check(ensure_dyn_smem(enc_attention_kernel<HD>, smem, attr), "enc_attention");              \
        enc_attention_kernel<HD><<<grid, EA_THREADS, smem, st>>>(qkv, out, S, H, ld, q_off, k_off, v_off,   \
                                                                 window, scale);                            \
        break;                                                                                              \
    }
    switch (hd) {
        ENC_ATTN_CASE(32)
        ENC_ATTN_CASE(64)
        ENC_ATTN_CASE(128)
        default: fail(VOX_EINVAL, fmt("enc_attention: unsupported head_dim %d", hd));
    }
#undef ENC_ATTN_CASE
    post_launch("enc_attention");
}

template <bool RING>
__global__ void dec_rope_append_kernel(float *qkv, int M, int ld, int H, int Hkv, int hd, const KvView kv, const RopeView rope) {
    const int i = blockIdx.x, b = blockIdx.y;
    const int pos = kv.pos[b] + i;
    if (!RING && pos >= kv.max_seq()) return;
    const int half = hd >> 1;
    float *row = qkv + ((size_t)b * M + i) * ld;
    const size_t rr = (size_t)(RING ? pos % rope.rows : pos) * half;
    const float *cr = rope.cos_t + rr, *sr = rope.sin_t + rr;
    for (int t = threadIdx.x; t < H * half; t += blockDim.x) {
        const int h = t / half, p = t - h * half;
        float *v = row + h * hd + 2 * p;
        const float xr = v[0], xi = v[1];
        v[0] = xr * cr[p] - xi * sr[p];
        v[1] = xr * sr[p] + xi * cr[p];
    }
    const float *krow = row + H * hd;
    const float *vrow = krow + Hkv * hd;
    for (int t = threadIdx.x; t < Hkv * half; t += blockDim.x) {
        const int h = t / half, p = t - h * half;
        const float xr = krow[h * hd + 2 * p], xi = krow[h * hd + 2 * p + 1];
        float *dst = kv.k + kv_index<RING>(kv, b, Hkv, h, pos, hd) + 2 * p;
        dst[0] = xr * cr[p] - xi * sr[p];
        dst[1] = xr * sr[p] + xi * cr[p];
    }
    for (int t = threadIdx.x; t < Hkv * hd; t += blockDim.x) {
        const int h = t / hd, d = t - h * hd;
        kv.v[kv_index<RING>(kv, b, Hkv, h, pos, hd) + d] = vrow[t];
    }
}

void launch_dec_rope_append(float *qkv, int B, int M, int ld, int H, int Hkv, int hd, const KvView &kv,
                            const RopeView &rope, cudaStream_t st) {
    dim3 grid(M, B);
    if (kv.ring) dec_rope_append_kernel<true><<<grid, 256, 0, st>>>(qkv, M, ld, H, Hkv, hd, kv, rope);
    else dec_rope_append_kernel<false><<<grid, 256, 0, st>>>(qkv, M, ld, H, Hkv, hd, kv, rope);
    post_launch("dec_rope_append");
}

template <bool RING>
__global__ void dec_attention_kernel(const float *__restrict__ qkv, int M, int ld, int H, int Hkv, int hd, const KvView kv,
                                     int window, float scale, float *__restrict__ out) {
    extern __shared__ float sm[];
    const int kvh = blockIdx.x, i = blockIdx.y, b = blockIdx.z;
    const int G = H / Hkv;
    const int warp = threadIdx.x >> 5, lane = threadIdx.x & 31;
    const int pos = kv.pos[b] + i;
    const int max_seq = kv.max_seq();
    if (!RING && pos >= max_seq) return;
    float *qsm = sm + warp * hd;
    float *sc = sm + G * hd + (size_t)warp * max_seq;
    const int h = kvh * G + warp;
    const float *qrow = qkv + ((size_t)b * M + i) * ld + h * hd;
    for (int d = lane; d < hd; d += 32) qsm[d] = qrow[d];
    __syncwarp();
    const int j_lo = pos - window > 0 ? pos - window : 0;
    const int base = RING ? j_lo : 0;
    float mx = -INFINITY;
    for (int j = j_lo + lane; j <= pos; j += 32) {
        const float4 *kr = reinterpret_cast<const float4 *>(kv.k + kv_index<RING>(kv, b, Hkv, kvh, j, hd));
        const float4 *q4 = reinterpret_cast<const float4 *>(qsm);
        float acc = 0.0f;
        for (int d = 0; d < (hd >> 2); ++d) {
            const float4 kk = kr[d];
            const float4 qv = q4[d];
            acc = fmaf(qv.x, kk.x, acc);
            acc = fmaf(qv.y, kk.y, acc);
            acc = fmaf(qv.z, kk.z, acc);
            acc = fmaf(qv.w, kk.w, acc);
        }
        acc *= scale;
        sc[j - base] = acc;
        mx = fmaxf(mx, acc);
    }
    mx = warp_max(mx);
    float sum = 0.0f;
    for (int j = j_lo + lane; j <= pos; j += 32) {
        const float pv = expf(sc[j - base] - mx);
        sc[j - base] = pv;
        sum += pv;
    }
    sum = warp_sum(sum);
    __syncwarp();
    const float inv = 1.0f / sum;
    float *orow = out + ((size_t)b * M + i) * (H * hd) + h * hd;
    for (int d = lane; d < hd; d += 32) {
        float acc = 0.0f;
        for (int j = j_lo; j <= pos; ++j) acc = fmaf(sc[j - base], kv.v[kv_index<RING>(kv, b, Hkv, kvh, j, hd) + d], acc);
        orow[d] = acc * inv;
    }
}

void launch_dec_attention(const float *qkv, int B, int M, int ld, int H, int Hkv, int hd, const KvView &kv, int window,
                          float scale, float *out, cudaStream_t st) {
    const int G = H / Hkv;
    dim3 grid(Hkv, M, B);
    const size_t smem = (size_t)G * (hd + kv.max_seq()) * sizeof(float);
    VOX_CHECK(smem <= 200 * 1024, VOX_EINVAL, "dec_attention: max_seq %d too large for the v1 kernel", kv.max_seq());
    static SmemAttr attr, attr_ring;
    if (kv.ring) {
        VOX_CHECK(window < kv.max_seq(), VOX_EINVAL, "dec_attention: window %d does not fit the KV ring", window);
        if (smem > 48 * 1024) smem_attr_check(ensure_dyn_smem(dec_attention_kernel<true>, smem, attr_ring), "dec_attention");
        dec_attention_kernel<true><<<grid, 32 * G, smem, st>>>(qkv, M, ld, H, Hkv, hd, kv, window, scale, out);
    } else {
        if (smem > 48 * 1024) smem_attr_check(ensure_dyn_smem(dec_attention_kernel<false>, smem, attr), "dec_attention");
        dec_attention_kernel<false><<<grid, 32 * G, smem, st>>>(qkv, M, ld, H, Hkv, hd, kv, window, scale, out);
    }
    post_launch("dec_attention");
}

__global__ void embed_kernel(const uint4 *__restrict__ qs, const __half *__restrict__ ds, int K,
                             const int *__restrict__ ids, const float *__restrict__ audio, int audio_seq, int M,
                             const int *__restrict__ pos_ptr, float *__restrict__ x, float *__restrict__ ssq_out,
                             const int rows_total, const float *const *__restrict__ audio_rows) {
    asm volatile("griddepcontrol.launch_dependents;\n" ::: "memory");
    const int i = blockIdx.x, b = blockIdx.y;
    const int r = b * M + i;
    const int id = ids[r];
    const int bpr = K >> 5;
    const float *arow = nullptr;
    if (audio_rows) {
        arow = audio_rows[b] ? audio_rows[b] + (size_t)i * K : nullptr;
    } else if (audio) {
        const int pos = (pos_ptr ? pos_ptr[b] : 0) + i;
        arow = audio + ((size_t)b * audio_seq + pos) * K;
    }
    for (int t = threadIdx.x; t < bpr * 16; t += blockDim.x) {
        const int blk = t >> 4, j = t & 15;
        const uint8_t byte = reinterpret_cast<const uint8_t *>(qs + (size_t)id * bpr + blk)[j];
        const float dd = __half2float(ds[(size_t)id * bpr + blk]);
        const int k = blk * 32 + j;
        float lo = ((float)(byte & 0xF) - 8.0f) * dd;
        float hi = ((float)(byte >> 4) - 8.0f) * dd;
        if (arow) {
            lo = arow[k] + lo;
            hi = arow[k + 16] + hi;
        }
        x[(size_t)r * K + k] = lo;
        x[(size_t)r * K + k + 16] = hi;
    }
    if (ssq_out) {
        __syncthreads();
        for (int t = threadIdx.x; t < (K >> 4); t += blockDim.x) {
            const float *p = x + (size_t)r * K + 16 * t;
            float s = 0.0f;
#pragma unroll
            for (int j = 0; j < 16; ++j) s = fmaf(p[j], p[j], s);
// ... 463 lines not shown
```

### voxtral_mini_realtime_rs_b200/csrc/kernels.h

```cpp
#pragma once
#include <cuda_fp16.h>
#include <cuda_runtime.h>

#include <atomic>

#include <cstdint>

namespace vox {

constexpr int VOX_NUM_SMS = 132;

struct SmemAttr {
    std::atomic<size_t> bytes[64];
};
template <typename F>
inline cudaError_t ensure_dyn_smem(F func, size_t bytes, SmemAttr &st) {
    int dev = 0;
    cudaError_t e = cudaGetDevice(&dev);
    if (e != cudaSuccess) return e;
    if (dev < 0 || dev >= 64) return cudaFuncSetAttribute(func, cudaFuncAttributeMaxDynamicSharedMemorySize, (int)bytes);
    if (st.bytes[dev].load(std::memory_order_acquire) >= bytes) return cudaSuccess;
    e = cudaFuncSetAttribute(func, cudaFuncAttributeMaxDynamicSharedMemorySize, (int)bytes);
    if (e == cudaSuccess) {
        size_t cur = st.bytes[dev].load(std::memory_order_relaxed);
        while (cur < bytes && !st.bytes[dev].compare_exchange_weak(cur, bytes, std::memory_order_release)) {}
    }
    return e;
}
void smem_attr_check(cudaError_t e, const char *what);


struct Q4Weight {
    const uint4 *qs = nullptr;
    const __half *d = nullptr;
    const uint4 *qs_tc = nullptr;
    const uint2 *d_tc = nullptr;
    int N = 0, K = 0;
    size_t bytes() const { return (size_t)N * (K / 32) * 18; }
};

enum Epi : int {
    EPI_NONE = 0,
    EPI_RESIDUAL = 1,
    EPI_SILU_MUL = 2,
    EPI_GELU = 3,
};

struct AdaRows {
    const float *const *rows = nullptr;
    int m = 1;
    size_t off = 0;
    __host__ __device__ const float *row(int r) const { return rows[r / m] + off; }
};

void launch_q4_matvec(const Q4Weight &w, const float *x, int M, float *y, int ldy, const float *bias,
                      const float *res, int epi, cudaStream_t st);
struct TcWork {
    float *partial = nullptr;
    size_t partial_floats = 0;
    int *counters = nullptr;
    int n_counters = 0;
    const float *ssq_in = nullptr;
    int ssq_in_parts = 0;
    float *ssq_out = nullptr;
};
void launch_q4_matvec_tc_ex(const Q4Weight &w, const float *x, int M, float *y, int ldy, const float *bias,
                            const float *res, int epi, const float *gamma, const float *ada, float eps,
                            const TcWork *wk, cudaStream_t st, const AdaRows &ada_rows = AdaRows{});
TcWork q4_matvec_tc_work_size(int N, int K);
constexpr int KV_PAGE = 16;
struct KvView {
    float *k = nullptr, *v = nullptr;
    const int *page_table = nullptr;
    int max_pages = 0;
    bool ring = false;
    const int *pos = nullptr;
    __host__ __device__ int max_seq() const { return max_pages * KV_PAGE; }
};
#ifdef __CUDACC__
template <bool RING = false>
__device__ __forceinline__ size_t kv_index(const KvView &kv, const int b, const int Hkv, const int kvh, const int j, const int hd) {
    const int lp = j / KV_PAGE;
    const int phys = kv.page_table[(size_t)b * kv.max_pages + (RING ? lp % kv.max_pages : lp)];
    return (((size_t)phys * Hkv + kvh) * KV_PAGE + (j % KV_PAGE)) * hd;
}
#endif
struct RopeView {
    const float *cos_t = nullptr, *sin_t = nullptr;
    int rows = 0;
};
bool dec_attn_fused_supported(int H, int Hkv, int hd);
void launch_dec_attn_fused(float *qkv, int B, int ld, int H, int Hkv, int hd, const KvView &kv, int window, float scale,
                           const RopeView &rope, float *out, cudaStream_t st);
void launch_q4_gemm(const Q4Weight &w, const float *a, int M, float *y, int ldy, const float *bias,
                    const float *res, int epi, cudaStream_t st);
bool gemm_tc5_supported(const Q4Weight &w, int M);
size_t gemm_tc5_split_elems(int M, int K);
void launch_split_tiles(const float *x, int M, int K, const float *gamma, const float *ada, float eps, void *xt,
                        cudaStream_t st, const AdaRows &ada_rows = AdaRows{});
struct GemmWork {
    float *partial = nullptr;
    size_t partial_floats = 0;
    int *counters = nullptr;
    int n_counters = 0;
};
void launch_q4_gemm_tc5(const Q4Weight &w, const void *xt, int M, float *y, int ldy, const float *bias, const float *res,
                        int epi, const GemmWork *gw, cudaStream_t st);
GemmWork gemm_tc5_work_size();

struct Q4Path {
    bool matvec_tc = true;
    bool gemm_tc = true;
};
struct Q4Scratch {
    void *xt = nullptr;
    size_t xt_elems = 0;
    const GemmWork *gw = nullptr;
    const TcWork *tc = nullptr;
};
void launch_q4_linear(const Q4Weight &w, const float *x, int M, float *y, int ldy, const float *bias, const float *res,
                      int epi, const float *gamma, const float *ada, float eps, float *tmp, const Q4Scratch &sc,
                      const Q4Path &path, cudaStream_t st, const AdaRows &ada_rows = AdaRows{});
void launch_conv2_gemm(const float *in, const float *w, const float *bias, float *out, int B, int T_in,
                       int T_out, int C_in, int C_out, cudaStream_t st, int t_off = 0, int in0 = 0);
void launch_transpose_mel(const float *in, float *out, int B, int C, int T, cudaStream_t st);
void launch_rmsnorm(const float *x, const float *gamma, const float *scale, float *y, int rows, int dim,
                    float eps, cudaStream_t st, const AdaRows &ada_rows = AdaRows{});
void launch_rope_inplace(float *buf, int rows, int ld, int q_off, int n_q, int k_off, int n_k, int hd,
                         int seq, int pos0, const float *cos_t, const float *sin_t, cudaStream_t st);
void launch_enc_attention(const float *qkv, float *out, int B, int S, int H, int hd, int ld, int q_off,
                          int k_off, int v_off, int window, float scale, cudaStream_t st);
bool enc_attention_tc_supported(int hd, int ld, int q_off, int k_off, int v_off);
void launch_enc_attention_tc(const float *qkv, float *out, int B, int S, int H, int hd, int ld, int q_off,
                             int k_off, int v_off, int window, float scale, cudaStream_t st);
void launch_dec_rope_append(float *qkv, int B, int M, int ld, int H, int Hkv, int hd, const KvView &kv,
                            const RopeView &rope, cudaStream_t st);
void launch_dec_attention(const float *qkv, int B, int M, int ld, int H, int Hkv, int hd, const KvView &kv, int window,
                          float scale, float *out, cudaStream_t st);
void launch_embed(const Q4Weight &emb, const int *ids, const float *audio, int audio_seq, int B, int M,
                  const int *pos, float *x, float *ssq_out, cudaStream_t st, const float *const *audio_rows = nullptr);
void launch_argmax(const float *logits, int B, int V, int *tok, int *out_ids, int out_ld,
                   const int *out_pos_ptr, cudaStream_t st);
constexpr int ARGMAX_PARTS = 64;
void launch_argmax_multi(const float *logits, int B, int V, int *tok, int *out_ids, int out_ld,
                         const int *out_pos_ptr, float *scratch_vals, int *scratch_idx, int *counters,
                         cudaStream_t st);
constexpr int TOPK_MAX = 8;
struct ScoreWork {
    float *m = nullptr, *l = nullptr, *vals = nullptr;
    int *idx = nullptr, *counters = nullptr;
};
void launch_token_scores(const float *logits, int B, int V, int k, const int *out_pos_ptr, int out_ld, int *top_ids,
                         float *top_logprobs, const ScoreWork &w, cudaStream_t st);
void launch_advance(int *a, int da, int *b, int db, int n, cudaStream_t st);
void launch_gather_last(const float *src, float *dst, int B, int M, int dim, cudaStream_t st);
void launch_reshape_rows(const float *src, float *dst, int B, int S, int S_out, int dim, int factor,
                         cudaStream_t st);
void launch_mul_vec(const float *a, const float *b, float *out, size_t n, cudaStream_t st);

void launch_mel(const float *samples, int B, size_t n, size_t sample_stride, const float *window,
                const float *fb_vals, const int *fb_start, const int *fb_len, int fb_stride, float *out,
                int frames, int layout, cudaStream_t st, int frame0 = 0, size_t sample0 = 0, int out0 = 0);
void launch_peak_normalize_pad(const float *in, int B, size_t n, float target, int do_norm, float *out,
                               size_t out_stride, size_t left, float *scale_buf, cudaStream_t st);

uint64_t kernel_launch_count();
void add_graph_launches(int64_t n);

}
```

### voxtral_mini_realtime_rs_b200/csrc/model.cu

```cuda
#include "model.h"

#include <algorithm>
#include <cmath>
#include <cstring>

#include "common.h"

namespace vox {

void cuda_check(cudaError_t e, const char *what) {
    if (e != cudaSuccess) fail(VOX_ECUDA, fmt("CUDA error: %s: %s", what, cudaGetErrorString(e)));
}

void *DeviceArena::alloc(size_t bytes) {
    if (bytes == 0) bytes = 16;
    void *p = nullptr;
    cudaError_t e = cudaMalloc(&p, bytes);
    if (e != cudaSuccess) fail(VOX_ENOMEM, fmt("cudaMalloc(%zu) failed: %s", bytes, cudaGetErrorString(e)));
    ptrs.push_back(p);
    total += bytes;
    return p;
}

void DeviceArena::release() {
    for (void *p : ptrs) cudaFree(p);
    ptrs.clear();
    total = 0;
}

void MelTables::build(DeviceArena &arena) {
    fb_dense.resize((size_t)kMelBins * kMelFreqs);
    mel_filterbank(fb_dense.data());
    window_host.resize(kMelNfft);
    hann_window(kMelNfft, window_host.data());
    std::vector<int> start(kMelBins), len(kMelBins);
    int maxlen = 1;
    for (int m = 0; m < kMelBins; ++m) {
        int lo = kMelFreqs, hi = -1;
        for (int j = 0; j < kMelFreqs; ++j)
            if (fb_dense[(size_t)m * kMelFreqs + j] != 0.0f) { lo = std::min(lo, j); hi = std::max(hi, j); }
        if (hi < 0) { lo = 0; hi = -1; }
        start[m] = lo;
        len[m] = hi - lo + 1;
        maxlen = std::max(maxlen, len[m]);
    }
    fb_stride = maxlen;
    std::vector<float> vals((size_t)kMelBins * maxlen, 0.0f);
    for (int m = 0; m < kMelBins; ++m)
        for (int j = 0; j < len[m]; ++j) vals[(size_t)m * maxlen + j] = fb_dense[(size_t)m * kMelFreqs + start[m] + j];
    window = arena.upload(window_host.data(), window_host.size());
    fb_vals = arena.upload(vals.data(), vals.size());
    fb_start = arena.upload(start.data(), start.size());
    fb_len = arena.upload(len.data(), len.size());
}

static void build_tc_layout(DeviceArena &arena, Q4Weight &w, const std::vector<uint8_t> &qs,
                            const std::vector<uint16_t> &ds);

Q4Weight upload_q4(DeviceArena &arena, const std::vector<const uint8_t *> &raw, const std::vector<int> &n_rows,
                   int K, bool interleave, bool tc_layout) {
    VOX_CHECK(K % 32 == 0, VOX_EINVAL, "Q4 weight with K=%d (not a multiple of 32)", K);
    const int bpr = K / 32;
    int N = 0;
    for (int n : n_rows) N += n;
    if (interleave) VOX_CHECK(raw.size() == 2 && n_rows[0] == n_rows[1], VOX_EINVAL, "interleave needs two equal parts");
    std::vector<uint8_t> qs((size_t)N * bpr * 16);
    std::vector<uint16_t> ds((size_t)N * bpr);
    int row_base = 0;
    for (size_t p = 0; p < raw.size(); ++p) {
        for (int r = 0; r < n_rows[p]; ++r) {
            const int dst_row = interleave ? 2 * r + (int)p : row_base + r;
            const uint8_t *src = raw[p] + (size_t)r * bpr * 18;
            uint8_t *qd = qs.data() + (size_t)dst_row * bpr * 16;
            uint16_t *dd = ds.data() + (size_t)dst_row * bpr;
            for (int b = 0; b < bpr; ++b) {
                memcpy(dd + b, src + (size_t)b * 18, 2);
                memcpy(qd + (size_t)b * 16, src + (size_t)b * 18 + 2, 16);
            }
        }
        row_base += n_rows[p];
    }
    Q4Weight w;
    w.N = N;
    w.K = K;
    w.qs = (const uint4 *)arena.upload(qs.data(), qs.size());
    w.d = (const __half *)arena.upload(ds.data(), ds.size());
    if (tc_layout) build_tc_layout(arena, w, qs, ds);
    return w;
}

static void build_tc_layout(DeviceArena &arena, Q4Weight &w, const std::vector<uint8_t> &qs,
                            const std::vector<uint16_t> &ds) {
    const int bpr = w.K / 32;
    const int n_tiles = (w.N + 15) / 16, n_pairs = (bpr + 1) / 2;
    std::vector<uint32_t> q((size_t)n_tiles * n_pairs * 32 * 4, 0u);
    std::vector<uint16_t> d((size_t)n_tiles * n_pairs * 8 * 4, 0);
    const uint32_t *src = reinterpret_cast<const uint32_t *>(qs.data());
    for (int T = 0; T < n_tiles; ++T)
        for (int P = 0; P < n_pairs; ++P) {
            uint32_t *qd = q.data() + ((size_t)T * n_pairs + P) * 128;
            uint16_t *dd = d.data() + ((size_t)T * n_pairs + P) * 32;
            for (int g = 0; g < 8; ++g)
                for (int bb = 0; bb < 2; ++bb) {
                    const int b = 2 * P + bb;
                    if (b >= bpr) continue;
                    for (int h = 0; h < 2; ++h) {
                        const int row = 16 * T + g + 8 * h;
                        if (row >= w.N) continue;
                        const size_t blk = (size_t)row * bpr + b;
                        for (int t = 0; t < 4; ++t) qd[(g * 4 + t) * 4 + bb * 2 + h] = src[blk * 4 + t];
                        dd[g * 4 + bb * 2 + h] = ds[blk];
                    }
                }
        }
    w.qs_tc = (const uint4 *)arena.upload(q.data(), q.size());
    w.d_tc = (const uint2 *)arena.upload(d.data(), d.size());
}

namespace {

const char *kEnc = "mm_streams_embeddings.embedding_module.whisper_encoder";
const char *kAdapter = "mm_streams_embeddings.embedding_module.audio_language_projection";
const char *kTokEmb = "mm_streams_embeddings.embedding_module.tok_embeddings.weight";
const char *kFinalNorm = "norm.weight";

float f16_to_f32(uint16_t h) {
    uint32_t sign = (uint32_t)(h & 0x8000u) << 16, exp = (h >> 10) & 0x1Fu, man = h & 0x3FFu, bits;
    if (exp == 0) {
        if (man == 0) bits = sign;
        else {
            int e = -1;
            do { e++; man <<= 1; } while ((man & 0x400u) == 0);
            man &= 0x3FFu;
            bits = sign | ((uint32_t)(127 - 15 - e) << 23) | (man << 13);
        }
    } else if (exp == 31) bits = sign | 0x7F800000u | (man << 13);
    else bits = sign | ((exp + 127 - 15) << 23) | (man << 13);
    float f;
    memcpy(&f, &bits, 4);
    return f;
}

struct Loader {
    const Gguf &g;
    Model &m;
    uint64_t q4_bytes = 0;

    const GgufTensorInfo &info(const std::string &name) {
        const GgufTensorInfo *t = g.find(name);
        VOX_CHECK(t != nullptr, VOX_ENOTFOUND, "Tensor '%s' not found in GGUF", name.c_str());
        return *t;
    }
    bool has(const std::string &name) { return g.find(name) != nullptr; }

    std::vector<float> f32(const std::string &name, const std::vector<int64_t> &shape) {
        const GgufTensorInfo &t = info(name);
        VOX_CHECK(t.dtype != VOX_DTYPE_Q4_0, VOX_EFORMAT, "Cannot load Q4_0 tensor '%s' as f32", name.c_str());
        VOX_CHECK(t.shape() == shape, VOX_EINVAL, "Tensor '%s' has unexpected shape", name.c_str());
        std::vector<uint8_t> raw((size_t)t.byte_size());
        g.read_tensor(t, raw.data());
        size_t n = (size_t)t.num_elements();
        std::vector<float> out(n);
        if (t.dtype == VOX_DTYPE_F32) memcpy(out.data(), raw.data(), n * 4);
        else
            for (size_t i = 0; i < n; ++i) {
                uint16_t h;
                memcpy(&h, raw.data() + 2 * i, 2);
                out[i] = f16_to_f32(h);
            }
        return out;
    }
    float *f32_dev(const std::string &name, const std::vector<int64_t> &shape) {
        std::vector<float> v = f32(name, shape);
        return m.arena.upload(v.data(), v.size());
    }
    std::vector<uint8_t> q4_raw(const std::string &name, int N, int K) {
        const GgufTensorInfo &t = info(name);
        VOX_CHECK(t.dtype == VOX_DTYPE_Q4_0, VOX_EFORMAT, "Expected Q4_0 for '%s', got dtype %u", name.c_str(), t.dtype);
        std::vector<int64_t> shp = t.shape();
        VOX_CHECK(shp.size() == 2 && shp[0] == N && shp[1] == K, VOX_EINVAL, "Tensor '%s' has unexpected shape (want [%d,%d])",
                  name.c_str(), N, K);
        std::vector<uint8_t> raw((size_t)t.byte_size());
        g.read_tensor(t, raw.data());
        q4_bytes += raw.size();
        return raw;
    }
    Q4Weight q4(const std::string &name, int N, int K, bool tc = false) {
        std::vector<uint8_t> raw = q4_raw(name, N, K);
        return upload_q4(m.arena, {raw.data()}, {N}, K, false, tc);
    }
    Q4Weight q4_concat(const std::vector<std::string> &names, const std::vector<int> &ns, int K, bool tc = false) {
        std::vector<std::vector<uint8_t>> raws;
        std::vector<const uint8_t *> ptrs;
        for (size_t i = 0; i < names.size(); ++i) raws.push_back(q4_raw(names[i], ns[i], K));
        for (auto &r : raws) ptrs.push_back(r.data());
        return upload_q4(m.arena, ptrs, ns, K, false, tc);
    }
    Q4Weight q4_interleave(const std::string &a, const std::string &b, int N, int K, bool tc = false) {
        std::vector<uint8_t> ra = q4_raw(a, N, K), rb = q4_raw(b, N, K);
        return upload_q4(m.arena, {ra.data(), rb.data()}, {N, N}, K, true, tc);
    }
    std::vector<float> bias_or_zero(const std::string &name, int n) {
        if (has(name)) return f32(name, {n});
        return std::vector<float>((size_t)n, 0.0f);
    }
};

void build_rope(DeviceArena &arena, int hd, int max_seq, float theta, float **cos_d, float **sin_d) {
    const int half = hd / 2;
    std::vector<float> c((size_t)max_seq * half), s((size_t)max_seq * half);
    rope_rows(hd, theta, 0, max_seq, c.data(), s.data());
    *cos_d = arena.upload(c.data(), c.size());
    *sin_d = arena.upload(s.data(), s.size());
}

}

void rope_rows(int hd, float theta, int64_t p0, int n, float *cos_out, float *sin_out) {
    const int half = hd / 2;
    std::vector<float> inv(half);
    for (int i = 0; i < half; ++i) inv[i] = 1.0f / powf(theta, (float)(2 * i) / (float)hd);
    for (int r = 0; r < n; ++r)
        for (int i = 0; i < half; ++i) {
            const float f = (float)(p0 + r) * inv[i];
            cos_out[(size_t)r * half + i] = cosf(f);
            sin_out[(size_t)r * half + i] = sinf(f);
        }
}

Model *Model::load(const Gguf &g, int device) {
    int ndev = 0;
    cudaError_t e = cudaGetDeviceCount(&ndev);
    VOX_CHECK(e == cudaSuccess && ndev > 0, VOX_ECUDA, "no CUDA device available (%s); this library has no CPU fallback",
              cudaGetErrorString(e));
    VOX_CHECK(device >= 0 && device < ndev, VOX_EINVAL, "device %d out of range (have %d)", device, ndev);
    CUDA_OK(cudaSetDevice(device));
    Model *mp = new Model();
    try {
        Model &m = *mp;
        m.device = device;
        m.arena.device = device;
        Loader L{g, m};
        vox_model_info &c = m.info;
        auto kv = [&](const char *k, int dflt) { uint32_t v; return g.kv_u32(k, &v) ? (int)v : dflt; };
        c.enc_layers = kv("voxtral.enc.n_layers", 32);
        c.enc_heads = kv("voxtral.enc.n_heads", 32);
        c.enc_head_dim = kv("voxtral.enc.head_dim", 64);
        c.enc_window = kv("voxtral.enc.sliding_window", 750);
        c.dec_layers = kv("voxtral.dec.n_layers", 26);
        c.dec_heads = kv("voxtral.dec.n_heads", 32);
        c.dec_kv_heads = kv("voxtral.dec.n_kv_heads", 8);
        c.dec_head_dim = kv("voxtral.dec.head_dim", 128);
        c.dec_window = kv("voxtral.dec.sliding_window", 8192);
        c.reshape_factor = kv("voxtral.reshape_factor", 4);
        c.prefix_len = 38;
        const std::string E = kEnc;
        {
            std::vector<int64_t> s = L.info(E + ".conv_layers.0.conv.weight").shape();
            VOX_CHECK(s.size() == 3 && s[2] == 3, VOX_EINVAL, "conv_layers.0 weight must be [C,mels,3]");
            c.enc_dim = (int)s[0];
            c.n_mels = (int)s[1];
            VOX_CHECK(c.n_mels == kMelBins, VOX_EINVAL, "n_mels=%d unsupported (mel front-end is 128-bin)", c.n_mels);
        }
        auto dim2 = [&](const std::string &name, int axis) {
            std::vector<int64_t> s = L.info(name).shape();
            VOX_CHECK(s.size() == 2, VOX_EINVAL, "Tensor '%s' must be 2-D (has %zu dims)", name.c_str(), s.size());
            VOX_CHECK(s[axis] >= 1 && s[axis] <= (1 << 24), VOX_EINVAL, "Tensor '%s' dim %d = %lld out of range", name.c_str(), axis,
                      (long long)s[axis]);
            return (int)s[axis];
        };
        c.enc_ffn = dim2(E + ".transformer.layers.0.feed_forward.w1.weight", 0);
        c.vocab = dim2(kTokEmb, 0);
        c.dec_dim = dim2(kTokEmb, 1);
        c.dec_ffn = dim2("layers.0.feed_forward.w1.weight", 0);
        c.t_cond_dim = dim2("layers.0.ada_rms_norm_t_cond.0.weight", 0);
        for (int v : {c.enc_layers, c.enc_heads, c.enc_head_dim, c.dec_layers, c.dec_heads, c.dec_kv_heads, c.dec_head_dim,
                      c.reshape_factor, c.enc_dim})
            VOX_CHECK(v >= 1 && v <= (1 << 20), VOX_EINVAL, "model dimension %d out of range (voxtral.* metadata)", v);
        VOX_CHECK(c.enc_window >= 0 && c.dec_window >= 0, VOX_EINVAL, "negative sliding window");
        VOX_CHECK(c.dec_heads % c.dec_kv_heads == 0, VOX_EINVAL, "dec_heads %% dec_kv_heads != 0");
        VOX_CHECK(c.enc_head_dim == 32 || c.enc_head_dim == 64 || c.enc_head_dim == 128, VOX_EINVAL,
                  "encoder head_dim %d unsupported", c.enc_head_dim);
        VOX_CHECK(c.dec_head_dim % 4 == 0, VOX_EINVAL, "decoder head_dim %d unsupported", c.dec_head_dim);

        const int d = c.enc_dim, hdq = c.enc_heads * c.enc_head_dim, D = c.dec_dim;
        {
            std::vector<float> w = L.f32(E + ".conv_layers.0.conv.weight", {d, c.n_mels, 3});
            std::vector<float> r((size_t)d * 3 * c.n_mels);
            for (int o = 0; o < d; ++o)
                for (int ci = 0; ci < c.n_mels; ++ci)
                    for (int t = 0; t < 3; ++t)
                        r[(size_t)o * 3 * c.n_mels + (size_t)t * c.n_mels + ci] = w[((size_t)o * c.n_mels + ci) * 3 + t];
            m.conv1_w = m.arena.upload(r.data(), r.size());
        }
        m.conv1_b = L.f32_dev(E + ".conv_layers.0.conv.bias", {d});
        {
            std::vector<float> w = L.f32(E + ".conv_layers.1.conv.weight", {d, d, 3});
            std::vector<float> r((size_t)d * 3 * d);
            for (int o = 0; o < d; ++o)
                for (int ci = 0; ci < d; ++ci)
                    for (int t = 0; t < 3; ++t) r[(size_t)o * 3 * d + (size_t)t * d + ci] = w[((size_t)o * d + ci) * 3 + t];
            m.conv2_w = m.arena.upload(r.data(), r.size());
        }
        m.conv2_b = L.f32_dev(E + ".conv_layers.1.conv.bias", {d});
        m.enc.resize(c.enc_layers);
        for (int i = 0; i < c.enc_layers; ++i) {
            const std::string p = E + ".transformer.layers." + std::to_string(i);
            EncLayerW &l = m.enc[i];
            l.attn_norm = L.f32_dev(p + ".attention_norm.weight", {d});
            l.ffn_norm = L.f32_dev(p + ".ffn_norm.weight", {d});
            l.wqkv = L.q4_concat({p + ".attention.wq.weight", p + ".attention.wk.weight", p + ".attention.wv.weight"},
                                 {hdq, hdq, hdq}, d);
            std::vector<float> bq = L.bias_or_zero(p + ".attention.wq.bias", hdq);
            std::vector<float> bv = L.bias_or_zero(p + ".attention.wv.bias", hdq);
            std::vector<float> bqkv((size_t)3 * hdq, 0.0f);
            memcpy(bqkv.data(), bq.data(), sizeof(float) * hdq);
            memcpy(bqkv.data() + 2 * hdq, bv.data(), sizeof(float) * hdq);
            l.bqkv = m.arena.upload(bqkv.data(), bqkv.size());
            l.wo = L.q4(p + ".attention.wo.weight", d, hdq);
            std::vector<float> bo = L.bias_or_zero(p + ".attention.wo.bias", d);
            l.bo = m.arena.upload(bo.data(), bo.size());
            l.w13 = L.q4_interleave(p + ".feed_forward.w1.weight", p + ".feed_forward.w3.weight", c.enc_ffn, d);
            l.w2 = L.q4(p + ".feed_forward.w2.weight", d, c.enc_ffn);
            std::vector<float> b2 = L.bias_or_zero(p + ".feed_forward.w2.bias", d);
            l.b2 = m.arena.upload(b2.data(), b2.size());
        }
        m.enc_norm = L.f32_dev(E + ".transformer.norm.weight", {d});
        m.adapter0 = L.q4(std::string(kAdapter) + ".0.weight", D, d * c.reshape_factor);
        m.adapter2 = L.q4(std::string(kAdapter) + ".2.weight", D, D);
        {
            const GgufTensorInfo &t = L.info(kTokEmb);
            VOX_CHECK(t.dtype == VOX_DTYPE_Q4_0, VOX_EFORMAT,
                      "tok_embeddings must be Q4_0 in this build (got dtype %u)", t.dtype);
            m.tok_emb = L.q4(kTokEmb, c.vocab, D, true);
        }
        const int qd = c.dec_heads * c.dec_head_dim, kvd = c.dec_kv_heads * c.dec_head_dim;
        m.dec.resize(c.dec_layers);
        uint64_t dec_q4 = 0;
        for (int j = 0; j < c.dec_layers; ++j) {
            const std::string p = "layers." + std::to_string(j);
            DecLayerW &l = m.dec[j];
            const uint64_t before = L.q4_bytes;
            l.ada0 = L.q4(p + ".ada_rms_norm_t_cond.0.weight", c.t_cond_dim, D);
            l.ada2 = L.q4(p + ".ada_rms_norm_t_cond.2.weight", D, c.t_cond_dim);
            l.attn_norm = L.f32_dev(p + ".attention_norm.weight", {D});
            l.ffn_norm = L.f32_dev(p + ".ffn_norm.weight", {D});
            l.wqkv = L.q4_concat({p + ".attention.wq.weight", p + ".attention.wk.weight", p + ".attention.wv.weight"},
                                 {qd, kvd, kvd}, D, true);
            l.wo = L.q4(p + ".attention.wo.weight", D, qd, true);
            l.w13 = L.q4_interleave(p + ".feed_forward.w1.weight", p + ".feed_forward.w3.weight", c.dec_ffn, D, true);
            l.w2 = L.q4(p + ".feed_forward.w2.weight", D, c.dec_ffn, true);
            dec_q4 += L.q4_bytes - before;
        }
        m.dec_norm = L.f32_dev(kFinalNorm, {D});
        build_rope(m.arena, c.enc_head_dim, m.enc_rope_len, m.rope_theta, &m.enc_cos, &m.enc_sin);
        build_rope(m.arena, c.dec_head_dim, m.dec_rope_len, m.rope_theta, &m.dec_cos, &m.dec_sin);
        m.mel.build(m.arena);
        c.q4_bytes = L.q4_bytes;
        c.device_bytes = m.arena.total;
        c.decode_step_bytes = dec_q4 + m.tok_emb.bytes();
        CUDA_OK(cudaDeviceSynchronize());
    } catch (...) {
        delete mp;
        throw;
    }
    return mp;
}

static int conv_out(int t) { return (t + 2 - 3) / 2 + 1; }

Session *Session::create(Model *m, int max_batch, int max_mel_frames, bool kv_ring) {
    VOX_CHECK(max_batch >= 1 && max_batch <= 64, VOX_EINVAL, "max_batch %d out of range [1,64]", max_batch);
    VOX_CHECK(max_mel_frames >= 16, VOX_EINVAL, "max_mel_frames %d too small", max_mel_frames);
    CUDA_OK(cudaSetDevice(m->device));
    Session *s = new Session();
    try {
        const vox_model_info &c = m->info;
        s->m = m;
        s->arena.device = m->device;
        s->max_batch = max_batch;
        s->max_mel_frames = max_mel_frames;
        s->T1_max = conv_out(max_mel_frames);
        s->S_max = conv_out(s->T1_max);
        s->S4_max = s->S_max / c.reshape_factor;
        s->M_max = std::max(c.prefix_len, 64);
        VOX_CHECK(s->S_max <= m->enc_rope_len, VOX_EINVAL, "max_mel_frames %d exceeds the encoder RoPE table", max_mel_frames);
        CUDA_OK(cudaStreamCreateWithFlags(&s->st, cudaStreamNonBlocking));
        for (auto &e : s->ev) CUDA_OK(cudaEventCreate(&e));
        const size_t B = max_batch;
        const int hdq = c.enc_heads * c.enc_head_dim;
        s->mel = s->arena.alloc_n<float>(B * c.n_mels * max_mel_frames);
        s->mel_tm = s->arena.alloc_n<float>(B * c.n_mels * max_mel_frames);
        s->peak_scale = s->arena.alloc_n<float>(B);
        s->h1 = s->arena.alloc_n<float>(B * s->T1_max * c.enc_dim);
        const size_t rows = B * s->S_max;
        s->x_enc = s->arena.alloc_n<float>(rows * c.enc_dim);
        s->h_enc = s->arena.alloc_n<float>(rows * c.enc_dim);
        s->qkv_enc = s->arena.alloc_n<float>(rows * 3 * hdq);
        s->attn_enc = s->arena.alloc_n<float>(rows * hdq);
        s->act_enc = s->arena.alloc_n<float>(rows * c.enc_ffn);
        const size_t rows4 = B * std::max(s->S4_max, 1);
        s->packed = s->arena.alloc_n<float>(rows4 * c.enc_dim * c.reshape_factor);
        s->adapter_h = s->arena.alloc_n<float>(rows4 * c.dec_dim);
        s->audio = s->arena.alloc_n<float>(rows4 * c.dec_dim);
        const int kv_cap = std::max(s->S4_max, s->M_max) + s->M_max;
        s->kv_max_pages = kv_ring ? (c.dec_window + s->M_max) / KV_PAGE + 1 : (kv_cap + KV_PAGE - 1) / KV_PAGE;
        s->kv_n_pages = max_batch * s->kv_max_pages;
        s->out_ld = s->kv_max_pages * KV_PAGE;
        s->kv_ring = kv_ring;
        s->dec_rope = m->dec_rope();
        const size_t kv_elems = (size_t)c.dec_layers * s->kv_n_pages * c.dec_kv_heads * KV_PAGE * c.dec_head_dim;
        s->kc = s->arena.alloc_n<float>(kv_elems);
        s->vc = s->arena.alloc_n<float>(kv_elems);
        s->page_table_host.resize((size_t)max_batch * s->kv_max_pages);
        for (int b = 0; b < max_batch; ++b)
            for (int pg = 0; pg < s->kv_max_pages; ++pg) s->page_table_host[(size_t)b * s->kv_max_pages + pg] = b * s->kv_max_pages + pg;
        s->d_page_table = s->arena.upload(s->page_table_host.data(), s->page_table_host.size());
        const size_t drows = B * s->M_max;
        const int qkvd = (c.dec_heads + 2 * c.dec_kv_heads) * c.dec_head_dim;
        s->x_dec = s->arena.alloc_n<float>(drows * c.dec_dim);
        s->h_dec = s->arena.alloc_n<float>(drows * c.dec_dim);
        s->qkv_dec = s->arena.alloc_n<float>(drows * qkvd);
        s->attn_dec = s->arena.alloc_n<float>(drows * c.dec_heads * c.dec_head_dim);
        s->act_dec = s->arena.alloc_n<float>(drows * c.dec_ffn);
        s->last_h = s->arena.alloc_n<float>(B * c.dec_dim);
        s->logits = s->arena.alloc_n<float>(B * c.vocab);
        s->ada = s->arena.alloc_n<float>((size_t)c.dec_layers * c.dec_dim);
        s->ffn_gamma_ada = s->arena.alloc_n<float>((size_t)c.dec_layers * c.dec_dim);
        s->ada_sets = s->arena.alloc_n<float>(B * s->ada_set_floats());
        s->delays.assign(B, 0.0f);
        s->d_ada_rows = (const float **)s->arena.alloc(sizeof(float *) * B);
        s->d_fga_rows = (const float **)s->arena.alloc(sizeof(float *) * B);
        s->t_embed = s->arena.alloc_n<float>(c.dec_dim);
        s->ada_tmp = s->arena.alloc_n<float>(c.t_cond_dim);
        s->d_pos = s->arena.alloc_n<int>(B);
        s->d_outpos = s->arena.alloc_n<int>(B);
        s->d_tok = s->arena.alloc_n<int>(B);
        s->d_ids = s->arena.alloc_n<int>(drows);
        s->d_out = s->arena.alloc_n<int>(B * s->out_ld);
        {
            const int rows_e = max_batch * s->S_max, rows_d = max_batch * s->M_max;
            size_t e = 0;
            for (int K : {c.enc_dim, c.enc_heads * c.enc_head_dim, c.enc_ffn}) e = std::max(e, gemm_tc5_split_elems(rows_e, K / 64 * 64));
            e = std::max(e, gemm_tc5_split_elems(max_batch * std::max(s->S4_max, 1), c.enc_dim * c.reshape_factor / 64 * 64));
            for (int K : {c.dec_dim, c.dec_heads * c.dec_head_dim, c.dec_ffn}) e = std::max(e, gemm_tc5_split_elems(std::max(rows_d, max_batch * std::max(s->S4_max, 1)), K / 64 * 64));
            s->xt_elems = e;
            s->xt_buf = s->arena.alloc(e * 2);
            s->gemm_work = gemm_tc5_work_size();
            alloc_split_k(s->arena, s->gemm_work);
            const char *gv = getenv("VOX_GEMM");
            s->path.gemm_tc = !(gv && std::string(gv) == "simt");
            const char *tv = getenv("VOX_MATVEC");
            s->path.matvec_tc = !(tv && std::string(tv) == "simt");
            const char *av = getenv("VOX_ENC_ATTN");
            s->use_enc_attn_tc = !(av && std::string(av) == "simt");
        }
        {
            std::vector<const Q4Weight *> ws{&m->tok_emb};
            for (const DecLayerW &l : m->dec) ws.insert(ws.end(), {&l.wqkv, &l.wo, &l.w13, &l.w2});
            for (const Q4Weight *w : ws) {
                const TcWork need = q4_matvec_tc_work_size(w->N, w->K);
                s->tc_split.partial_floats = std::max(s->tc_split.partial_floats, need.partial_floats);
                s->tc_split.n_counters = std::max(s->tc_split.n_counters, need.n_counters);
            }
            alloc_split_k(s->arena, s->tc_split);
            s->ssq_x = s->arena.alloc_n<float>((size_t)((c.dec_dim + 15) / 16) * 8);
            s->am_vals = s->arena.alloc_n<float>((size_t)max_batch * ARGMAX_PARTS);
            s->am_idx = s->arena.alloc_n<int>((size_t)max_batch * ARGMAX_PARTS);
            s->am_cnt = s->arena.alloc_n<int>(max_batch);
            CUDA_OK(cudaMemset(s->am_cnt, 0, sizeof(int) * max_batch));
        }
        {
            const char *mv = getenv("VOX_MEGA");
            s->use_mega = !(mv && mv[0] == '0');
            s->mega_grid = decode_mega_grid(m->device);
            s->mega_ops_cap = 6 * c.dec_layers + 4;
            s->mega_ops = s->arena.alloc_n<MegaOp>(s->mega_ops_cap);
            s->mega_bar = s->arena.alloc_n<unsigned>(4);
            CUDA_OK(cudaMemset(s->mega_bar, 0, sizeof(unsigned) * 4));
            s->mega_am_vals = s->arena.alloc_n<float>((size_t)s->mega_grid * 8);
            s->mega_am_idx = s->arena.alloc_n<int>((size_t)s->mega_grid * 8);
            s->mega_att_units = std::max(s->mega_grid, 8 * c.dec_kv_heads) + 8 * c.dec_kv_heads;
            s->mega_att_acc = s->arena.alloc_n<float>((size_t)2 * s->mega_att_units * (c.dec_heads / c.dec_kv_heads) * c.dec_head_dim);
            s->mega_att_ml = s->arena.alloc_n<float>((size_t)2 * s->mega_att_units * (c.dec_heads / c.dec_kv_heads) * 2);
            s->mega_epoch = s->arena.alloc_n<int>(1);
            CUDA_OK(cudaMemset(s->mega_att_acc, 0, sizeof(float) * 2 * s->mega_att_units * (c.dec_heads / c.dec_kv_heads) * c.dec_head_dim));
            CUDA_OK(cudaMemset(s->mega_att_ml, 0, sizeof(float) * 2 * s->mega_att_units * (c.dec_heads / c.dec_kv_heads) * 2));
            CUDA_OK(cudaMemset(s->mega_epoch, 0, sizeof(int)));
            {
                auto blocks = [](int K) { return (size_t)((K / 32 + 1) / 2) * 2; };
                s->mega_xf_blocks = blocks(c.dec_dim);
                s->mega_af_blocks = blocks(c.dec_heads * c.dec_head_dim);
                s->mega_cf_blocks = blocks(c.dec_ffn);
                s->mega_xf_bf = s->arena.alloc_n<uint2>(s->mega_xf_blocks * 16 * 8);
                s->mega_af_bf = s->arena.alloc_n<uint2>(s->mega_af_blocks * 16 * 8);
                s->mega_cf_bf = s->arena.alloc_n<uint2>(s->mega_cf_blocks * 16 * 8);
                s->mega_xf_off = s->arena.alloc_n<float2>(s->mega_xf_blocks * 8);
                s->mega_af_off = s->arena.alloc_n<float2>(s->mega_af_blocks * 8);
                s->mega_cf_off = s->arena.alloc_n<float2>(s->mega_cf_blocks * 8);
            }
            s->mega_trace = s->arena.alloc_n<unsigned long long>((size_t)s->mega_ops_cap * 6);
            CUDA_OK(cudaMemset(s->mega_trace, 0, sizeof(unsigned long long) * s->mega_ops_cap * 6));
            if (const char *ta = getenv("VOX_MEGA_TRACE_ALL")) {
                if (ta[0] == '1') {
                    const size_t n = (size_t)s->mega_grid * s->mega_ops_cap * 4;
                    s->mega_trace_all = s->arena.alloc_n<unsigned long long>(n);
                    CUDA_OK(cudaMemset(s->mega_trace_all, 0, sizeof(unsigned long long) * n));
                }
            }
        }
        CUDA_OK(cudaMemset(s->d_pos, 0, sizeof(int) * B));
        CUDA_OK(cudaMemset(s->d_outpos, 0, sizeof(int) * B));
        s->out_rows.assign(B, 0);
        s->set_delay(kDefaultDelay);
    } catch (...) {
        delete s;
        throw;
    }
    return s;
}

Session::~Session() {
    if (step_graph) cudaGraphExecDestroy(step_graph);
    for (auto &e : ev)
        if (e) cudaEventDestroy(e);
    if (st) cudaStreamDestroy(st);
}

void Session::linear(const Q4Weight &w, const float *x, int M, float *y, int ldy, const float *bias, const float *res,
                     int epi, const float *gamma, const float *ada, float *tmp, const TcWork *tc, const AdaRows &ada_rows) {
    launch_q4_linear(w, x, M, y, ldy, bias, res, epi, gamma, ada, m->norm_eps, tmp, Q4Scratch{xt_buf, xt_elems, &gemm_work, tc},
                     path, st, ada_rows);
}

static void compute_ada(Session &s, float delay, float *ada_dst, float *fga_dst) {
    const Model *m = s.m;
    const vox_model_info &c = m->info;
    std::vector<float> t(c.dec_dim);
    time_embedding(delay, c.dec_dim, t.data());
    CUDA_OK(cudaMemcpyAsync(s.t_embed, t.data(), sizeof(float) * c.dec_dim, cudaMemcpyHostToDevice, s.st));
    CUDA_OK(cudaStreamSynchronize(s.st));
    std::vector<float> ones(c.dec_dim, 1.0f);
    for (int j = 0; j < c.dec_layers; ++j) {
        float *dst = ada_dst + (size_t)j * c.dec_dim;
        CUDA_OK(cudaMemcpyAsync(dst, ones.data(), sizeof(float) * c.dec_dim, cudaMemcpyHostToDevice, s.st));
        launch_q4_matvec(m->dec[j].ada0, s.t_embed, 1, s.ada_tmp, c.t_cond_dim, nullptr, nullptr, EPI_GELU, s.st);
        launch_q4_matvec(m->dec[j].ada2, s.ada_tmp, 1, dst, c.dec_dim, nullptr, dst, EPI_RESIDUAL, s.st);
        launch_mul_vec(m->dec[j].ffn_norm, dst, fga_dst + (size_t)j * c.dec_dim, c.dec_dim, s.st);
    }
    CUDA_OK(cudaStreamSynchronize(s.st));
}

void Session::set_delay(float delay) {
    CUDA_OK(cudaSetDevice(m->device));
    const size_t LD = ada_set_floats() / 2;
    compute_ada(*this, delay, ada, ffn_gamma_ada);
    shared_delay = delay;
    for (int i = 0; i < max_batch; ++i) {
        CUDA_OK(cudaMemcpyAsync(ada_sets + i * 2 * LD, ada, sizeof(float) * LD, cudaMemcpyDeviceToDevice, st));
        CUDA_OK(cudaMemcpyAsync(ada_sets + i * 2 * LD + LD, ffn_gamma_ada, sizeof(float) * LD, cudaMemcpyDeviceToDevice, st));
        delays[i] = delay;
    }
    CUDA_OK(cudaStreamSynchronize(st));
}

static bool same_delay(float a, float b) { return a == b || (std::isnan(a) && std::isnan(b)); }

void Session::set_delays(const float *d, int b) {
    VOX_CHECK(b >= 1 && b <= max_batch, VOX_EINVAL, "set_delays: %d streams out of range [1,%d]", b, max_batch);
    for (int i = 0; i < b; ++i)
        VOX_CHECK(std::isfinite(d[i]) && d[i] >= 0.0f, VOX_EINVAL, "delay %g of stream %d must be finite and >= 0", d[i], i);
    CUDA_OK(cudaSetDevice(m->device));
    for (int i = 0; i < b; ++i) set_stream_delay(i, d[i]);
}

void Session::set_stream_delay(int i, float d) {
    if (same_delay(delays[i], d)) return;
    const size_t n = ada_set_floats();
    float *set = ada_sets + (size_t)i * n;
    int same = -1;
    for (int j = 0; j < max_batch && same < 0; ++j)
        if (j != i && same_delay(delays[j], d)) same = j;
    if (same >= 0) {
        CUDA_OK(cudaMemcpyAsync(set, ada_sets + (size_t)same * n, sizeof(float) * n, cudaMemcpyDeviceToDevice, st));
        CUDA_OK(cudaStreamSynchronize(st));
    } else {
        compute_ada(*this, d, set, set + n / 2);
    }
    delays[i] = d;
}

void Session::bind_delays(const int *streams, int n) {
    bool uniform = true;
    for (int i = 1; i < n; ++i) uniform &= same_delay(delays[streams[i]], delays[streams[0]]);
    if (uniform) {
        ada_per_row = false;
        if (!same_delay(delays[streams[0]], shared_delay)) {
            const size_t LD = ada_set_floats() / 2;
            const float *set = ada_sets + (size_t)streams[0] * 2 * LD;
            CUDA_OK(cudaMemcpyAsync(ada, set, sizeof(float) * LD, cudaMemcpyDeviceToDevice, st));
            CUDA_OK(cudaMemcpyAsync(ffn_gamma_ada, set + LD, sizeof(float) * LD, cudaMemcpyDeviceToDevice, st));
            shared_delay = delays[streams[0]];
        }
        return;
    }
    ada_per_row = true;
    if (ada_row_streams.size() >= (size_t)n && std::equal(streams, streams + n, ada_row_streams.begin())) return;
    std::vector<const float *> a(n), f(n);
    for (int i = 0; i < n; ++i) {
        a[i] = ada_sets + (size_t)streams[i] * ada_set_floats();
        f[i] = a[i] + ada_set_floats() / 2;
    }
    CUDA_OK(cudaMemcpyAsync(d_ada_rows, a.data(), sizeof(float *) * n, cudaMemcpyHostToDevice, st));
    CUDA_OK(cudaMemcpyAsync(d_fga_rows, f.data(), sizeof(float *) * n, cudaMemcpyHostToDevice, st));
    CUDA_OK(cudaStreamSynchronize(st));
    ada_row_streams.assign(streams, streams + n);
}

void Session::bind_delays_identity(int B) {
    std::vector<int> id(B);
    for (int b = 0; b < B; ++b) id[b] = b;
    bind_delays(id.data(), B);
}

void Session::encode(int B, int T) {
    const vox_model_info &c = m->info;
    VOX_CHECK(B >= 1 && B <= max_batch, VOX_EINVAL, "batch %d exceeds session max_batch %d", B, max_batch);
    VOX_CHECK(T >= 1 && T <= max_mel_frames, VOX_EINVAL, "mel frames %d exceed session max_mel_frames %d", T, max_mel_frames);
    const int T1 = conv_out(T), S = conv_out(T1), S4 = S / c.reshape_factor;
    const int d = c.enc_dim, hdq = c.enc_heads * c.enc_head_dim;
    const int rows = B * S;
    launch_conv2_gemm(mel_tm, m->conv1_w, m->conv1_b, h1, B, T, T1, c.n_mels, d, st);
    launch_conv2_gemm(h1, m->conv2_w, m->conv2_b, x_enc, B, T1, S, d, d, st);
    if (debug_capture && dbg_conv) CUDA_OK(cudaMemcpyAsync(dbg_conv, x_enc, sizeof(float) * rows * d, cudaMemcpyDeviceToDevice, st));
    const float scale = powf((float)c.enc_head_dim, -0.5f);
    for (int i = 0; i < c.enc_layers; ++i) {
        const EncLayerW &l = m->enc[i];
        linear(l.wqkv, x_enc, rows, qkv_enc, 3 * hdq, l.bqkv, nullptr, EPI_NONE, l.attn_norm, nullptr, h_enc);
        launch_rope_inplace(qkv_enc, rows, 3 * hdq, 0, c.enc_heads, hdq, c.enc_heads, c.enc_head_dim, S, 0,
                            m->enc_cos, m->enc_sin, st);
        if (use_enc_attn_tc && enc_attention_tc_supported(c.enc_head_dim, 3 * hdq, 0, hdq, 2 * hdq))
            launch_enc_attention_tc(qkv_enc, attn_enc, B, S, c.enc_heads, c.enc_head_dim, 3 * hdq, 0, hdq, 2 * hdq,
                                    c.enc_window, scale, st);
        else
            launch_enc_attention(qkv_enc, attn_enc, B, S, c.enc_heads, c.enc_head_dim, 3 * hdq, 0, hdq, 2 * hdq,
                                 c.enc_window, scale, st);
        linear(l.wo, attn_enc, rows, x_enc, d, l.bo, x_enc, EPI_RESIDUAL);
        linear(l.w13, x_enc, rows, act_enc, c.enc_ffn, nullptr, nullptr, EPI_SILU_MUL, l.ffn_norm, nullptr, h_enc);
        linear(l.w2, act_enc, rows, x_enc, d, l.b2, x_enc, EPI_RESIDUAL);
        if (debug_capture && dbg_layers)
            CUDA_OK(cudaMemcpyAsync(dbg_layers + (size_t)i * rows * d, x_enc, sizeof(float) * rows * d,
                                    cudaMemcpyDeviceToDevice, st));
    }
    launch_rmsnorm(x_enc, m->enc_norm, nullptr, h_enc, rows, d, m->norm_eps, st);
// ... 396 lines not shown
```

### voxtral_mini_realtime_rs_b200/csrc/model.h

```cpp
#pragma once
#include <cuda_runtime.h>

#include <cstdint>
#include <string>
#include <vector>

#include "audio_host.h"
#include "gguf.h"
#include "decode_mega.h"
#include "kernels.h"

namespace vox {

void cuda_check(cudaError_t e, const char *what);
#define CUDA_OK(x) ::vox::cuda_check((x), #x)

struct DeviceArena {
    int device = 0;
    std::vector<void *> ptrs;
    size_t total = 0;
    void *alloc(size_t bytes);
    template <typename T>
    T *alloc_n(size_t n) { return (T *)alloc(n * sizeof(T)); }
    template <typename T>
    T *upload(const T *host, size_t n) {
        T *d = alloc_n<T>(n);
        CUDA_OK(cudaMemcpy(d, host, n * sizeof(T), cudaMemcpyHostToDevice));
        return d;
    }
    void release();
    ~DeviceArena() { release(); }
};

template <typename Work>
void alloc_split_k(DeviceArena &arena, Work &w) {
    w.partial = arena.alloc_n<float>(w.partial_floats);
    w.counters = arena.alloc_n<int>(w.n_counters);
    CUDA_OK(cudaMemset(w.counters, 0, sizeof(int) * w.n_counters));
}

struct MelTables {
    float *window = nullptr;
    float *fb_vals = nullptr;
    int *fb_start = nullptr, *fb_len = nullptr;
    int fb_stride = 0;
    std::vector<float> fb_dense, window_host;
    void build(DeviceArena &arena);
};

struct EncLayerW {
    float *attn_norm = nullptr, *ffn_norm = nullptr;
    Q4Weight wqkv, wo, w13, w2;
    float *bqkv = nullptr, *bo = nullptr, *b2 = nullptr;
};
struct DecLayerW {
    float *attn_norm = nullptr, *ffn_norm = nullptr;
    Q4Weight ada0, ada2, wqkv, wo, w13, w2;
};

struct Model {
    int device = 0;
    vox_model_info info{};
    float rope_theta = 1e6f, norm_eps = 1e-5f;
    DeviceArena arena;
    float *conv1_w = nullptr, *conv1_b = nullptr, *conv2_w = nullptr, *conv2_b = nullptr;
    std::vector<EncLayerW> enc;
    float *enc_norm = nullptr;
    Q4Weight adapter0, adapter2, tok_emb;
    std::vector<DecLayerW> dec;
    float *dec_norm = nullptr;
    float *enc_cos = nullptr, *enc_sin = nullptr, *dec_cos = nullptr, *dec_sin = nullptr;
    int enc_rope_len = 4096, dec_rope_len = 16384;
    MelTables mel;
    RopeView dec_rope() const { return RopeView{dec_cos, dec_sin, dec_rope_len}; }

    static Model *load(const Gguf &g, int device);
};

void rope_rows(int hd, float theta, int64_t p0, int n, float *cos_out, float *sin_out);

Q4Weight upload_q4(DeviceArena &arena, const std::vector<const uint8_t *> &raw, const std::vector<int> &n_rows,
                   int K, bool interleave, bool tc_layout = false);

constexpr float kDefaultDelay = 6.0f;

struct Session {
    Model *m = nullptr;
    int max_batch = 0, max_mel_frames = 0;
    int T1_max = 0, S_max = 0, S4_max = 0, M_max = 0;
    cudaStream_t st = nullptr;
    DeviceArena arena;
    cudaEvent_t ev[5] = {nullptr, nullptr, nullptr, nullptr, nullptr};
    float *pcm = nullptr, *pcm_pad = nullptr, *peak_scale = nullptr;
    size_t pcm_cap = 0, pcm_pad_cap = 0;
    float *mel = nullptr;
    float *mel_tm = nullptr;
    float *h1 = nullptr, *x_enc = nullptr, *h_enc = nullptr, *qkv_enc = nullptr, *attn_enc = nullptr, *act_enc = nullptr;
    float *packed = nullptr, *adapter_h = nullptr, *audio = nullptr;
    int cur_B = 0, cur_S = 0, cur_S4 = 0;
    float *kc = nullptr, *vc = nullptr;
    int kv_max_pages = 0, kv_n_pages = 0;
    int *d_page_table = nullptr;
    std::vector<int> page_table_host;
    size_t kv_layer_stride() const { return (size_t)kv_n_pages * m->info.dec_kv_heads * KV_PAGE * m->info.dec_head_dim; }
    bool kv_ring = false;
    KvView kv_view(int layer) const;
    RopeView dec_rope;
    float *x_dec = nullptr, *h_dec = nullptr, *qkv_dec = nullptr, *attn_dec = nullptr, *act_dec = nullptr;
    float *last_h = nullptr, *logits = nullptr;
    float *logits_all = nullptr;
    size_t logits_all_cap = 0;
    float *ada = nullptr, *t_embed = nullptr, *ada_tmp = nullptr;
    float *ffn_gamma_ada = nullptr;
    float shared_delay = -1.0f;
    std::vector<float> delays;
    float *ada_sets = nullptr;
    size_t ada_set_floats() const { return (size_t)2 * m->info.dec_layers * m->info.dec_dim; }
    bool ada_per_row = false;
    const float **d_ada_rows = nullptr, **d_fga_rows = nullptr;
    std::vector<int> ada_row_streams;
    int *d_pos = nullptr, *d_outpos = nullptr, *d_tok = nullptr, *d_ids = nullptr, *d_out = nullptr;
    int out_ld = 0;
    int cache_len = 0;
    bool stream_mode = false;
    const float *const *audio_rows_dev = nullptr;
    const float *audio_base = nullptr;
    int top_k = 0;
    int *d_top_ids = nullptr;
    float *d_top_lp = nullptr;
    ScoreWork score_work;
    void set_top_k(int k);
    void token_scores(int B);
    int scores_k = 0, scores_b = 0, scores_n = 0;
    std::vector<int> scores_pos;
    std::vector<int> out_rows;
    cudaGraphExec_t step_graph = nullptr;
    int step_graph_B = 0, step_graph_S4 = 0, step_graph_top_k = 0;
    bool step_graph_per_row = false;
    uint64_t step_graph_nodes = 0;
    bool use_graph = true;
    TcWork tc_split;
    float *ssq_x = nullptr;
    float *am_vals = nullptr;
    int *am_idx = nullptr, *am_cnt = nullptr;
    TcWork tc_work(bool norm_in, bool ssq_out) const;
    bool use_mega = true;
    int mega_B = 0, mega_grid = 0, mega_n_ops = 0, mega_ops_cap = 0;
    MegaPlan mega_plan;
    std::vector<MegaOp> mega_ops_host;
    MegaOp *mega_ops = nullptr;
    unsigned *mega_bar = nullptr;
    float *mega_am_vals = nullptr;
    int *mega_am_idx = nullptr;
    float *mega_att_acc = nullptr, *mega_att_ml = nullptr;
    int mega_att_units = 0;
    int *mega_epoch = nullptr;
    unsigned mega_steps_host = 0;
    uint2 *mega_xf_bf = nullptr, *mega_af_bf = nullptr, *mega_cf_bf = nullptr;
    float2 *mega_xf_off = nullptr, *mega_af_off = nullptr, *mega_cf_off = nullptr;
    size_t mega_xf_blocks = 0, mega_af_blocks = 0, mega_cf_blocks = 0;
    void mega_clear_fragments();
    unsigned long long *mega_trace_all = nullptr;
    unsigned long long *mega_trace = nullptr;
    bool mega_prepare(int B);
    bool fused_decode(int rows) const;
    void decode_step_mega(int b0, int B, bool add_audio);
    void *xt_buf = nullptr;
    size_t xt_elems = 0;
    GemmWork gemm_work;
    bool use_enc_attn_tc = true;
    Q4Path path;
    std::vector<float> enc_debug;
    bool debug_capture = false;
    float *dbg_layers = nullptr;
    float *dbg_conv = nullptr;

    static Session *create(Model *m, int max_batch, int max_mel_frames, bool kv_ring = false);
    ~Session();
    void set_delay(float delay);
    void set_delays(const float *delays, int b);
    void set_stream_delay(int stream, float delay);
    void bind_delays(const int *streams, int n);
    void bind_delays_identity(int B);
    void encode(int B, int T);
    void linear(const Q4Weight &w, const float *x, int M, float *y, int ldy, const float *bias, const float *res,
                int epi, const float *gamma = nullptr, const float *ada = nullptr, float *tmp = nullptr,
                const TcWork *tc = nullptr, const AdaRows &ada_rows = AdaRows{});
    bool decoder_forward(int B, int M);
    void lm_head_rows(int rows, bool norm_pending, float *dst);
    void decode_step(int B, bool add_audio = true);
    void prefill(int B, int M, const int *ids_host, bool add_audio);
    int transcribe_from_mel(int B, int T, int32_t *out_ids, size_t cap_ids, vox_timings *tm, bool timed_pre);
    void reset();
    void rebase_epoch();
};

}
```

Measured before the change: 3270.

## Rework tc5 GEMM with register-A wgmma, warp specialization, and deep pipeline

Rewrites the Q4 tensor-core GEMM so weights are fetched in the tc layout and dequantized into register A fragments (hi/lo split) for wgmma with register A operands. The kernel gains templated N-tile widths, an smem-sized multi-stage pipeline with full and empty mbarriers, and a spin-wait timeout trap. Encoder and adapter weights now also build the tc layout through a new Q4Layout enum, and the matvec tc path is gated by a separate flag. This mainly targets encoder and prefill GEMM throughput. It costs extra weight memory and adds complexity and hang-detection risk.

New measurement: 3414, median of 6. 1.04x the previous value.

```diff
diff --git a/voxtral_mini_realtime_rs_b200/csrc/capi.cu b/voxtral_mini_realtime_rs_b200/csrc/capi.cu
--- a/voxtral_mini_realtime_rs_b200/csrc/capi.cu
+++ b/voxtral_mini_realtime_rs_b200/csrc/capi.cu
@@ -278,7 +278,7 @@
     std::unique_ptr<vox_q4> q(new vox_q4());
     q->device = device;
     q->arena.device = device;
-    q->w = upload_q4(q->arena, {bytes}, {(int)n}, (int)k, false, true);
+    q->w = upload_q4(q->arena, {bytes}, {(int)n}, (int)k, false, Q4_TC);
     q->wk = q4_matvec_tc_work_size(q->w.N, q->w.K);
     alloc_split_k(q->arena, q->wk);
     *out = q.release();
@@ -438,9 +438,15 @@
     cudaEvent_t e0, e1;
     CUDA_OK(cudaEventCreate(&e0));
     CUDA_OK(cudaEventCreate(&e1));
+    for (int i = 0; i < n_w; ++i) {
+        REQUIRE(ws[i]);
+        VOX_CHECK(ws[i]->w.K == K && ws[i]->w.N == N, VOX_EINVAL, "bench weights must share one shape");
+        q4_scratch(const_cast<vox_q4 *>(ws[i]), m);
+    }
     auto run = [&](int i) {
-        launch_q4_linear(ws[i % n_w]->w, x, m, y, ws[i % n_w]->w.N, nullptr, nullptr, EPI_NONE, nullptr, nullptr, 0.0f, nullptr,
-                         Q4Scratch{}, g_q4_path, st);
+        vox_q4 *w = const_cast<vox_q4 *>(ws[i % n_w]);
+        launch_q4_linear(w->w, x, m, y, w->w.N, nullptr, nullptr, EPI_NONE, nullptr, nullptr, 0.0f, nullptr,
+                         q4_scratch(w, m), g_q4_path, st);
     };
     for (int i = 0; i < warmup; ++i) run(i);
     CUDA_OK(cudaStreamSynchronize(st));
diff --git a/voxtral_mini_realtime_rs_b200/csrc/gemm_tc5.cu b/voxtral_mini_realtime_rs_b200/csrc/gemm_tc5.cu
--- a/voxtral_mini_realtime_rs_b200/csrc/gemm_tc5.cu
+++ b/voxtral_mini_realtime_rs_b200/csrc/gemm_tc5.cu
@@ -1,4 +1,6 @@
 #include <cuda_fp16.h>
+
+#include <algorithm>
 
 #include "common.h"
 #include "kernels.h"
@@ -9,17 +11,26 @@
 
 namespace {
 
-constexpr int G5_WGS = 4;
-constexpr int G5_THREADS = G5_WGS * 128;
+constexpr int G5_THREADS = 384;
 constexpr int G5_BM = 128;
-constexpr int G5_BN = 128;
 constexpr int G5_BK = 64;
-constexpr int G5_TILE_BYTES = G5_BM * G5_BK * 2;
 constexpr int G5_PIECES = 2;
-constexpr int G5_STAGES = 3;
-constexpr int G5_STAGE_BYTES = 2 * G5_PIECES * G5_TILE_BYTES;
-constexpr int G5_SMEM_BYTES = G5_STAGES * G5_STAGE_BYTES;
+constexpr int G5_WQ_BYTES = (G5_BM / 16) * 512;
+constexpr int G5_WD_BYTES = (G5_BM / 16) * 64;
+constexpr int G5_SMEM_MAX = 227 * 1024;
+constexpr int G5_MAX_STAGES = 8;
 constexpr float G5_WSCALE = 256.0f;
+constexpr long long G5_SPIN_CYCLES = 4000000000ll;
+
+template <int TN>
+struct G5Tile {
+    static constexpr int X_BYTES = TN * G5_BK * 2;
+    static constexpr int STAGE_BYTES = G5_PIECES * X_BYTES + G5_WQ_BYTES + G5_WD_BYTES;
+    static constexpr int FIT = (G5_SMEM_MAX - 256) / STAGE_BYTES;
+    static constexpr int STAGES = FIT < G5_MAX_STAGES ? FIT : G5_MAX_STAGES;
+    static constexpr int SMEM_BYTES = STAGES * STAGE_BYTES + 2 * STAGES * 8;
+    static_assert(STAGES >= 4, "fewer than 3 stages of lookahead");
+};
 
 __device__ __forceinline__ uint32_t smem_u32(const void *p) { return (uint32_t)__cvta_generic_to_shared(p); }
 __device__ __forceinline__ void mbar_init(uint64_t *bar, uint32_t count) {
@@ -28,16 +39,29 @@
 __device__ __forceinline__ void mbar_expect_tx(uint64_t *bar, uint32_t bytes) {
     asm volatile("mbarrier.arrive.expect_tx.shared::cta.b64 _, [%0], %1;\n" ::"r"(smem_u32(bar)), "r"(bytes) : "memory");
 }
-__device__ __forceinline__ void mbar_wait(uint64_t *bar, uint32_t parity) {
+__device__ __forceinline__ void mbar_arrive(uint64_t *bar) {
+    asm volatile("mbarrier.arrive.shared::cta.b64 _, [%0];\n" ::"r"(smem_u32(bar)) : "memory");
+}
+__device__ __forceinline__ bool mbar_try(uint64_t *bar, uint32_t parity) {
+    uint32_t ok;
     asm volatile(
         "{\n"
         ".reg .pred p;\n"
-        "G5_WAIT:\n"
-        "mbarrier.try_wait.parity.shared::cta.b64 p, [%0], %1;\n"
-        "@p bra G5_DONE;\n"
-        "bra G5_WAIT;\n"
-        "G5_DONE:\n"
-        "}\n" ::"r"(smem_u32(bar)), "r"(parity) : "memory");
+        "mbarrier.try_wait.parity.shared::cta.b64 p, [%1], %2;\n"
+        "selp.u32 %0, 1, 0, p;\n"
+        "}\n"
+        : "=r"(ok)
+        : "r"(smem_u32(bar)), "r"(parity)
+        : "memory");
+    return ok != 0;
+}
+__device__ __forceinline__ void mbar_wait(uint64_t *bar, uint32_t parity) {
+    if (mbar_try(bar, parity)) return;
+    const long long t0 = clock64();
+    unsigned n = 0;
+    while (!mbar_try(bar, parity)) {
+        if ((++n & 0x3FFFu) == 0 && clock64() - t0 > G5_SPIN_CYCLES) __trap();
+    }
 }
 __device__ __forceinline__ void bulk_g2s(void *dst_smem, const void *src_gmem, uint32_t bytes, uint64_t *bar) {
     asm volatile("cp.async.bulk.shared::cluster.global.mbarrier::complete_tx::bytes [%0], [%1], %2, [%3];\n" ::"r"(
@@ -45,6 +69,7 @@
                  "l"(src_gmem), "r"(bytes), "r"(smem_u32(bar))
                  : "memory");
 }
+__device__ __forceinline__ void wg_sync(int id) { asm volatile("bar.sync %0, 128;\n" ::"r"(id) : "memory"); }
 
 __device__ __forceinline__ uint64_t gmma_desc(uint32_t smem_addr, uint32_t lbo_bytes, uint32_t sbo_bytes) {
     uint64_t d = 0;
@@ -53,29 +78,106 @@
     d |= (uint64_t)((sbo_bytes >> 4) & 0x3FFF) << 32;
     return d;
 }
-__device__ __forceinline__ void wgmma_m64n64k16(float (&d)[32], uint64_t adesc, uint64_t bdesc) {
+template <int TN>
+__device__ __forceinline__ void wgmma_rs(float (&d)[TN / 2], const uint32_t (&a)[4], uint64_t bdesc);
+template <>
+__device__ __forceinline__ void wgmma_rs<64>(float (&d)[32], const uint32_t (&a)[4], uint64_t bdesc) {
     asm volatile(
         "{\n"
         ".reg .pred p;\n"
-        "setp.ne.b32 p, %34, 0;\n"
+        "setp.ne.b32 p, %37, 0;\n"
         "wgmma.mma_async.sync.aligned.m64n64k16.f32.f16.f16 "
         "{%0,%1,%2,%3,%4,%5,%6,%7,%8,%9,%10,%11,%12,%13,%14,%15,%16,%17,%18,%19,%20,%21,%22,%23,%24,%25,%26,%27,%28,%29,%30,%31}, "
-        "%32, %33, p, 1, 1, 0, 0;\n"
+        "{%32,%33,%34,%35}, %36, p, 1, 1, 0;\n"
         "}\n"
-        : "+f"(d[0]), "+f"(d[1]), "+f"(d[2]), "+f"(d[3]), "+f"(d[4]), "+f"(d[5]), "+f"(d[6]), "+f"(d[7]), "+f"(d[8]),
-          "+f"(d[9]), "+f"(d[10]), "+f"(d[11]), "+f"(d[12]), "+f"(d[13]), "+f"(d[14]), "+f"(d[15]), "+f"(d[16]),
-          "+f"(d[17]), "+f"(d[18]), "+f"(d[19]), "+f"(d[20]), "+f"(d[21]), "+f"(d[22]), "+f"(d[23]), "+f"(d[24]),
-          "+f"(d[25]), "+f"(d[26]), "+f"(d[27]), "+f"(d[28]), "+f"(d[29]), "+f"(d[30]), "+f"(d[31])
-        : "l"(adesc), "l"(bdesc), "r"(1)
+        : "+f"(d[0]), "+f"(d[1]), "+f"(d[2]), "+f"(d[3]), "+f"(d[4]), "+f"(d[5]), "+f"(d[6]), "+f"(d[7]),
+          "+f"(d[8]), "+f"(d[9]), "+f"(d[10]), "+f"(d[11]), "+f"(d[12]), "+f"(d[13]), "+f"(d[14]), "+f"(d[15]),
+          "+f"(d[16]), "+f"(d[17]), "+f"(d[18]), "+f"(d[19]), "+f"(d[20]), "+f"(d[21]), "+f"(d[22]), "+f"(d[23]),
+          "+f"(d[24]), "+f"(d[25]), "+f"(d[26]), "+f"(d[27]), "+f"(d[28]), "+f"(d[29]), "+f"(d[30]), "+f"(d[31])
+        : "r"(a[0]), "r"(a[1]), "r"(a[2]), "r"(a[3]), "l"(bdesc), "r"(1)
+        : "memory");
+}
+template <>
+__device__ __forceinline__ void wgmma_rs<128>(float (&d)[64], const uint32_t (&a)[4], uint64_t bdesc) {
+    asm volatile(
+        "{\n"
+        ".reg .pred p;\n"
+        "setp.ne.b32 p, %69, 0;\n"
+        "wgmma.mma_async.sync.aligned.m64n128k16.f32.f16.f16 "
+        "{%0,%1,%2,%3,%4,%5,%6,%7,%8,%9,%10,%11,%12,%13,%14,%15,%16,%17,%18,%19,%20,%21,%22,%23,%24,%25,%26,%27,%28,%29,%30,%31,%32,%33,%34,%35,%36,%37,%38,%39,%40,%41,%42,%43,%44,%45,%46,%47,%48,%49,%50,%51,%52,%53,%54,%55,%56,%57,%58,%59,%60,%61,%62,%63}, "
+        "{%64,%65,%66,%67}, %68, p, 1, 1, 0;\n"
+        "}\n"
+        : "+f"(d[0]), "+f"(d[1]), "+f"(d[2]), "+f"(d[3]), "+f"(d[4]), "+f"(d[5]), "+f"(d[6]), "+f"(d[7]),
+          "+f"(d[8]), "+f"(d[9]), "+f"(d[10]), "+f"(d[11]), "+f"(d[12]), "+f"(d[13]), "+f"(d[14]), "+f"(d[15]),
+          "+f"(d[16]), "+f"(d[17]), "+f"(d[18]), "+f"(d[19]), "+f"(d[20]), "+f"(d[21]), "+f"(d[22]), "+f"(d[23]),
+          "+f"(d[24]), "+f"(d[25]), "+f"(d[26]), "+f"(d[27]), "+f"(d[28]), "+f"(d[29]), "+f"(d[30]), "+f"(d[31]),
+          "+f"(d[32]), "+f"(d[33]), "+f"(d[34]), "+f"(d[35]), "+f"(d[36]), "+f"(d[37]), "+f"(d[38]), "+f"(d[39]),
+          "+f"(d[40]), "+f"(d[41]), "+f"(d[42]), "+f"(d[43]), "+f"(d[44]), "+f"(d[45]), "+f"(d[46]), "+f"(d[47]),
+          "+f"(d[48]), "+f"(d[49]), "+f"(d[50]), "+f"(d[51]), "+f"(d[52]), "+f"(d[53]), "+f"(d[54]), "+f"(d[55]),
+          "+f"(d[56]), "+f"(d[57]), "+f"(d[58]), "+f"(d[59]), "+f"(d[60]), "+f"(d[61]), "+f"(d[62]), "+f"(d[63])
+        : "r"(a[0]), "r"(a[1]), "r"(a[2]), "r"(a[3]), "l"(bdesc), "r"(1)
+        : "memory");
+}
+template <>
+__device__ __forceinline__ void wgmma_rs<160>(float (&d)[80], const uint32_t (&a)[4], uint64_t bdesc) {
+    asm volatile(
+        "{\n"
+        ".reg .pred p;\n"
+        "setp.ne.b32 p, %85, 0;\n"
+        "wgmma.mma_async.sync.aligned.m64n160k16.f32.f16.f16 "
+        "{%0,%1,%2,%3,%4,%5,%6,%7,%8,%9,%10,%11,%12,%13,%14,%15,%16,%17,%18,%19,%20,%21,%22,%23,%24,%25,%26,%27,%28,%29,%30,%31,%32,%33,%34,%35,%36,%37,%38,%39,%40,%41,%42,%43,%44,%45,%46,%47,%48,%49,%50,%51,%52,%53,%54,%55,%56,%57,%58,%59,%60,%61,%62,%63,%64,%65,%66,%67,%68,%69,%70,%71,%72,%73,%74,%75,%76,%77,%78,%79}, "
+        "{%80,%81,%82,%83}, %84, p, 1, 1, 0;\n"
+        "}\n"
+        : "+f"(d[0]), "+f"(d[1]), "+f"(d[2]), "+f"(d[3]), "+f"(d[4]), "+f"(d[5]), "+f"(d[6]), "+f"(d[7]),
+          "+f"(d[8]), "+f"(d[9]), "+f"(d[10]), "+f"(d[11]), "+f"(d[12]), "+f"(d[13]), "+f"(d[14]), "+f"(d[15]),
+          "+f"(d[16]), "+f"(d[17]), "+f"(d[18]), "+f"(d[19]), "+f"(d[20]), "+f"(d[21]), "+f"(d[22]), "+f"(d[23]),
+          "+f"(d[24]), "+f"(d[25]), "+f"(d[26]), "+f"(d[27]), "+f"(d[28]), "+f"(d[29]), "+f"(d[30]), "+f"(d[31]),
+          "+f"(d[32]), "+f"(d[33]), "+f"(d[34]), "+f"(d[35]), "+f"(d[36]), "+f"(d[37]), "+f"(d[38]), "+f"(d[39]),
+          "+f"(d[40]), "+f"(d[41]), "+f"(d[42]), "+f"(d[43]), "+f"(d[44]), "+f"(d[45]), "+f"(d[46]), "+f"(d[47]),
+          "+f"(d[48]), "+f"(d[49]), "+f"(d[50]), "+f"(d[51]), "+f"(d[52]), "+f"(d[53]), "+f"(d[54]), "+f"(d[55]),
+          "+f"(d[56]), "+f"(d[57]), "+f"(d[58]), "+f"(d[59]), "+f"(d[60]), "+f"(d[61]), "+f"(d[62]), "+f"(d[63]),
+          "+f"(d[64]), "+f"(d[65]), "+f"(d[66]), "+f"(d[67]), "+f"(d[68]), "+f"(d[69]), "+f"(d[70]), "+f"(d[71]),
+          "+f"(d[72]), "+f"(d[73]), "+f"(d[74]), "+f"(d[75]), "+f"(d[76]), "+f"(d[77]), "+f"(d[78]), "+f"(d[79])
+        : "r"(a[0]), "r"(a[1]), "r"(a[2]), "r"(a[3]), "l"(bdesc), "r"(1)
+        : "memory");
+}
+template <>
+__device__ __forceinline__ void wgmma_rs<192>(float (&d)[96], const uint32_t (&a)[4], uint64_t bdesc) {
+    asm volatile(
+        "{\n"
+        ".reg .pred p;\n"
+        "setp.ne.b32 p, %101, 0;\n"
+        "wgmma.mma_async.sync.aligned.m64n192k16.f32.f16.f16 "
+        "{%0,%1,%2,%3,%4,%5,%6,%7,%8,%9,%10,%11,%12,%13,%14,%15,%16,%17,%18,%19,%20,%21,%22,%23,%24,%25,%26,%27,%28,%29,%30,%31,%32,%33,%34,%35,%36,%37,%38,%39,%40,%41,%42,%43,%44,%45,%46,%47,%48,%49,%50,%51,%52,%53,%54,%55,%56,%57,%58,%59,%60,%61,%62,%63,%64,%65,%66,%67,%68,%69,%70,%71,%72,%73,%74,%75,%76,%77,%78,%79,%80,%81,%82,%83,%84,%85,%86,%87,%88,%89,%90,%91,%92,%93,%94,%95}, "
+        "{%96,%97,%98,%99}, %100, p, 1, 1, 0;\n"
+        "}\n"
+        : "+f"(d[0]), "+f"(d[1]), "+f"(d[2]), "+f"(d[3]), "+f"(d[4]), "+f"(d[5]), "+f"(d[6]), "+f"(d[7]),
+          "+f"(d[8]), "+f"(d[9]), "+f"(d[10]), "+f"(d[11]), "+f"(d[12]), "+f"(d[13]), "+f"(d[14]), "+f"(d[15]),
+          "+f"(d[16]), "+f"(d[17]), "+f"(d[18]), "+f"(d[19]), "+f"(d[20]), "+f"(d[21]), "+f"(d[22]), "+f"(d[23]),
+          "+f"(d[24]), "+f"(d[25]), "+f"(d[26]), "+f"(d[27]), "+f"(d[28]), "+f"(d[29]), "+f"(d[30]), "+f"(d[31]),
+          "+f"(d[32]), "+f"(d[33]), "+f"(d[34]), "+f"(d[35]), "+f"(d[36]), "+f"(d[37]), "+f"(d[38]), "+f"(d[39]),
+          "+f"(d[40]), "+f"(d[41]), "+f"(d[42]), "+f"(d[43]), "+f"(d[44]), "+f"(d[45]), "+f"(d[46]), "+f"(d[47]),
+          "+f"(d[48]), "+f"(d[49]), "+f"(d[50]), "+f"(d[51]), "+f"(d[52]), "+f"(d[53]), "+f"(d[54]), "+f"(d[55]),
+          "+f"(d[56]), "+f"(d[57]), "+f"(d[58]), "+f"(d[59]), "+f"(d[60]), "+f"(d[61]), "+f"(d[62]), "+f"(d[63]),
+          "+f"(d[64]), "+f"(d[65]), "+f"(d[66]), "+f"(d[67]), "+f"(d[68]), "+f"(d[69]), "+f"(d[70]), "+f"(d[71]),
+          "+f"(d[72]), "+f"(d[73]), "+f"(d[74]), "+f"(d[75]), "+f"(d[76]), "+f"(d[77]), "+f"(d[78]), "+f"(d[79]),
+          "+f"(d[80]), "+f"(d[81]), "+f"(d[82]), "+f"(d[83]), "+f"(d[84]), "+f"(d[85]), "+f"(d[86]), "+f"(d[87]),
+          "+f"(d[88]), "+f"(d[89]), "+f"(d[90]), "+f"(d[91]), "+f"(d[92]), "+f"(d[93]), "+f"(d[94]), "+f"(d[95])
+        : "r"(a[0]), "r"(a[1]), "r"(a[2]), "r"(a[3]), "l"(bdesc), "r"(1)
         : "memory");
 }
 __device__ __forceinline__ void wgmma_fence() { asm volatile("wgmma.fence.sync.aligned;\n" ::: "memory"); }
 __device__ __forceinline__ void wgmma_commit() { asm volatile("wgmma.commit_group.sync.aligned;\n" ::: "memory"); }
 template <int N>
 __device__ __forceinline__ void wgmma_wait() { asm volatile("wgmma.wait_group.sync.aligned %0;\n" ::"n"(N) : "memory"); }
-__device__ __forceinline__ void acc_fence(float (&d)[32]) {
-#pragma unroll
-    for (int i = 0; i < 32; ++i) asm volatile("" : "+f"(d[i])::"memory");
+template <int R>
+__device__ __forceinline__ void acc_fence(float (&d)[R]) {
+#pragma unroll
+    for (int i = 0; i < R; ++i) asm volatile("" : "+f"(d[i])::"memory");
+}
+__device__ __forceinline__ void frag_fence(uint32_t (&f)[4][4]) {
+#pragma unroll
+    for (int i = 0; i < 16; ++i) asm volatile("" : "+r"(f[i >> 2][i & 3])::"memory");
 }
 
 __device__ __forceinline__ uint32_t g5_pack_f16x2(const float v0, const float v1) {
@@ -85,138 +187,157 @@
     return em | sg;
 }
 
+__device__ __forceinline__ void g5_dequant(const uint4 q, const uint2 dv, uint32_t (&fh)[4][4], uint32_t (&fl)[4][4]) {
+    const uint32_t wd[4] = {q.x, q.y, q.z, q.w};
+    const float dd[4] = {__half2float(__ushort_as_half((unsigned short)(dv.x & 0xFFFFu))),
+                         __half2float(__ushort_as_half((unsigned short)(dv.x >> 16))),
+                         __half2float(__ushort_as_half((unsigned short)(dv.y & 0xFFFFu))),
+                         __half2float(__ushort_as_half((unsigned short)(dv.y >> 16)))};
+#pragma unroll
+    for (int ks = 0; ks < 4; ++ks) {
+#pragma unroll
+        for (int r = 0; r < 2; ++r) {
+            const uint32_t word = wd[(ks >> 1) * 2 + r] >> ((ks & 1) * 4);
+            const float d = dd[(ks >> 1) * 2 + r] * G5_WSCALE * 1.92592994438723585305597794258492732e-34f;
+            float hi[4], lo[4];
+#pragma unroll
+            for (int j = 0; j < 4; ++j) {
+                const uint32_t n = (word >> (8 * j)) & 0xFu;
+                const float w = __fmul_rn(__fsub_rn(__uint_as_float(0x4B000000u | n), 8388616.0f), d);
+                const float c = __fmul_rn(w, 8193.0f);
+                hi[j] = __fsub_rn(c, __fsub_rn(c, w));
+                lo[j] = __fsub_rn(w, hi[j]);
+            }
+            fh[ks][r] = g5_pack_f16x2(hi[0], hi[1]);
+            fh[ks][2 + r] = g5_pack_f16x2(hi[2], hi[3]);
+            fl[ks][r] = g5_pack_f16x2(lo[0], lo[1]);
+            fl[ks][2 + r] = g5_pack_f16x2(lo[2], lo[3]);
+        }
+    }
+}
+
 struct G5Args {
-    const uint4 *qs;
-    const __half *ds;
+    const uint4 *qs_tc;
+    const uint2 *d_tc;
     int N, K, M;
     const __half *xt;
     const float *oscale;
-    int TT, KC;
+    int Mpad, KC;
     float *y;
     int ldy;
     const float *bias, *res;
-    int SK, KCs;
+    int FT, TT, SK, KCs;
     float *partial;
     int *counters;
 };
 
-template <int EPI>
+template <int TN, int EPI>
 __global__ void __launch_bounds__(G5_THREADS, 1) gemm_tc5_kernel(const G5Args a) {
+    using T = G5Tile<TN>;
+    constexpr int S = T::STAGES;
     extern __shared__ __align__(1024) unsigned char smem[];
-    __shared__ __align__(8) uint64_t full_bar[G5_STAGES];
-    const int tid = threadIdx.x, warp = tid >> 5, lane = tid & 31, wg = tid >> 7;
-    const int f0 = blockIdx.x * G5_BM, tt = blockIdx.y, tok0 = tt * G5_BN;
-    const int bpr = a.K >> 5;
-    const int kc_begin = blockIdx.z * a.KCs, kc_end = min(a.KC, kc_begin + a.KCs), nk = kc_end - kc_begin;
-    const size_t xt_piece = (size_t)a.TT * a.KC * (G5_TILE_BYTES / 2);
-
-    auto fetch_x = [&](int it) {
-        const int s = it % G5_STAGES;
-        unsigned char *dst = smem + (size_t)s * G5_STAGE_BYTES + G5_PIECES * G5_TILE_BYTES;
-        mbar_expect_tx(&full_bar[s], G5_PIECES * G5_TILE_BYTES);
-#pragma unroll
-        for (int p = 0; p < G5_PIECES; ++p) {
-            const __half *src = a.xt + p * xt_piece + ((size_t)tt * a.KC + kc_begin + it) * (G5_TILE_BYTES / 2);
-            bulk_g2s(dst + p * G5_TILE_BYTES, src, G5_TILE_BYTES, &full_bar[s]);
-        }
-    };
+    uint64_t *full = reinterpret_cast<uint64_t *>(smem + S * T::STAGE_BYTES);
+    uint64_t *empty = full + S;
+    __shared__ int is_last[2];
+    const int tid = threadIdx.x, wg = tid >> 7, lane = tid & 31;
     if (tid == 0) {
-        for (int s = 0; s < G5_STAGES; ++s) mbar_init(&full_bar[s], 1);
+        for (int s = 0; s < S; ++s) {
+            mbar_init(&full[s], 1);
+            mbar_init(&empty[s], 8);
+        }
         asm volatile("fence.mbarrier_init.release.cluster;\n" ::: "memory");
-        if (nk > 0) fetch_x(0);
     }
     __syncthreads();
-
-    const int drow = tid >> 2, dblk = (tid >> 1) & 1, dhalf = tid & 1;
-    const int gn = f0 + drow;
-    const int fq = wg & 1, tq = wg >> 1;
-    float acc[32];
-#pragma unroll
-    for (int i = 0; i < 32; ++i) acc[i] = 0.0f;
-
-    uint4 q_cur = make_uint4(0x88888888u, 0x88888888u, 0x88888888u, 0x88888888u);
-    __half d_cur = __float2half(0.0f);
-    if (gn < a.N && nk > 0) {
-        const size_t blk = (size_t)gn * bpr + (size_t)kc_begin * 2 + dblk;
-        q_cur = __ldg(a.qs + blk);
-        d_cur = __ldg(a.ds + blk);
-    }
-    for (int it = 0; it < nk; ++it) {
-        const int kc = kc_begin + it, s = it % G5_STAGES;
-        unsigned char *stage = smem + (size_t)s * G5_STAGE_BYTES;
-        const uint4 q = q_cur;
-        const float dd = __half2float(d_cur) * G5_WSCALE * 1.92592994438723585305597794258492732e-34f;
-        if (gn < a.N && kc + 1 < kc_end) {
-            const size_t blk = (size_t)gn * bpr + (size_t)(kc + 1) * 2 + dblk;
-            q_cur = __ldg(a.qs + blk);
-            d_cur = __ldg(a.ds + blk);
-        }
-        const uint32_t w4[4] = {q.x, q.y, q.z, q.w};
-        uint32_t ph[8], pl[8];
-#pragma unroll
-        for (int wi = 0; wi < 4; ++wi) {
-            const uint32_t nib = dhalf ? (w4[wi] >> 4) : w4[wi];
-            float hi[4], lo[4];
-#pragma unroll
-            for (int t = 0; t < 4; ++t) {
-                const uint32_t n = (nib >> (8 * t)) & 0xFu;
-                const float w = __fmul_rn(__fsub_rn(__uint_as_float(0x4B000000u | n), 8388616.0f), dd);
-                const float c = __fmul_rn(w, 8193.0f);
-                hi[t] = __fsub_rn(c, __fsub_rn(c, w));
-                lo[t] = __fsub_rn(w, hi[t]);
-            }
-            ph[wi * 2 + 0] = g5_pack_f16x2(hi[0], hi[1]);
-            ph[wi * 2 + 1] = g5_pack_f16x2(hi[2], hi[3]);
-            pl[wi * 2 + 0] = g5_pack_f16x2(lo[0], lo[1]);
-            pl[wi * 2 + 1] = g5_pack_f16x2(lo[2], lo[3]);
-        }
-        wgmma_wait<1>();
-        unsigned char *thi = stage, *tlo = stage + G5_TILE_BYTES;
-#pragma unroll
-        for (int c = 0; c < 2; ++c) {
-            const int off = (dblk * 4 + dhalf * 2 + c) * (G5_BM * 16) + drow * 16;
-            *reinterpret_cast<uint4 *>(thi + off) = make_uint4(ph[4 * c + 0], ph[4 * c + 1], ph[4 * c + 2], ph[4 * c + 3]);
-            *reinterpret_cast<uint4 *>(tlo + off) = make_uint4(pl[4 * c + 0], pl[4 * c + 1], pl[4 * c + 2], pl[4 * c + 3]);
-        }
-        asm volatile("fence.proxy.async.shared::cta;\n" ::: "memory");
-        __syncthreads();
-        if (tid == 0 && it + 1 < nk) fetch_x(it + 1);
-        mbar_wait(&full_bar[s], (uint32_t)((it / G5_STAGES) & 1));
-        const uint32_t wbase = smem_u32(stage) + fq * 64 * 16, xbase = smem_u32(stage + G5_PIECES * G5_TILE_BYTES) + tq * 64 * 16;
-        const uint32_t lbo = G5_BM * 16, sbo = 128;
+    const int tiles = a.FT * a.TT, units = tiles * a.SK;
+
+    if (wg == 0) {
+        asm volatile("setmaxnreg.dec.sync.aligned.u32 40;\n");
+        if (tid >= 32) return;
+        const size_t xt_piece = (size_t)a.KC * a.Mpad * G5_BK;
+        uint32_t it = 0;
+        for (int u = blockIdx.x; u < units; u += gridDim.x) {
+            const int ft = u % a.FT, tt = (u / a.FT) % a.TT, z = u / tiles;
+            const int kc_end = min(a.KC, (z + 1) * a.KCs);
+            for (int kc = z * a.KCs; kc < kc_end; ++kc, ++it) {
+                const int s = (int)(it % S);
+                if (it >= (uint32_t)S) mbar_wait(&empty[s], ((it / S) - 1) & 1);
+                unsigned char *st = smem + (size_t)s * T::STAGE_BYTES;
+                if (lane == 0) mbar_expect_tx(&full[s], T::STAGE_BYTES);
+                __syncwarp();
+                if (lane < G5_PIECES) {
+                    bulk_g2s(st + lane * T::X_BYTES, a.xt + lane * xt_piece + ((size_t)kc * a.Mpad + (size_t)tt * TN) * G5_BK,
+                             T::X_BYTES, &full[s]);
+                } else if (lane < G5_PIECES + 8) {
+                    const int j = lane - G5_PIECES;
+                    bulk_g2s(st + G5_PIECES * T::X_BYTES + j * 512, a.qs_tc + ((size_t)(ft * 8 + j) * a.KC + kc) * 32, 512,
+                             &full[s]);
+                } else if (lane < G5_PIECES + 16) {
+                    const int j = lane - G5_PIECES - 8;
+                    bulk_g2s(st + G5_PIECES * T::X_BYTES + G5_WQ_BYTES + j * 64, a.d_tc + ((size_t)(ft * 8 + j) * a.KC + kc) * 8,
+                             64, &full[s]);
+                }
+            }
+        }
+        return;
+    }
+
+    asm volatile("setmaxnreg.inc.sync.aligned.u32 232;\n");
+    const int cw = wg - 1, warp = (tid >> 5) & 3, g = lane >> 2, t = lane & 3;
+    const int wtile = cw * 4 + warp;
+    float acc[TN / 2];
+    uint32_t it = 0;
+    for (int u = blockIdx.x; u < units; u += gridDim.x) {
+        const int ft = u % a.FT, tt = (u / a.FT) % a.TT, z = u / tiles, tile = u % tiles;
+        const int kc_begin = z * a.KCs, nk = min(a.KC, kc_begin + a.KCs) - kc_begin;
+#pragma unroll
+        for (int i = 0; i < TN / 2; ++i) acc[i] = 0.0f;
+        for (int i = 0; i < nk; ++i, ++it) {
+            const int s = (int)(it % S);
+            mbar_wait(&full[s], (it / S) & 1);
+            const unsigned char *st = smem + (size_t)s * T::STAGE_BYTES;
+            const uint4 q = *reinterpret_cast<const uint4 *>(st + G5_PIECES * T::X_BYTES + (wtile * 32 + lane) * 16);
+            const uint2 dv = *reinterpret_cast<const uint2 *>(st + G5_PIECES * T::X_BYTES + G5_WQ_BYTES + (wtile * 8 + g) * 8);
+            uint32_t fh[4][4], fl[4][4];
+            g5_dequant(q, dv, fh, fl);
+            wgmma_wait<0>();
+            if (i > 0) {
+                __syncwarp();
+                if (lane == 0) mbar_arrive(&empty[(it - 1) % S]);
+            }
+            frag_fence(fh);
+            frag_fence(fl);
+            acc_fence(acc);
+            wgmma_fence();
+            const uint32_t xb = smem_u32(st);
+#pragma unroll
+            for (int ks = 0; ks < G5_BK / 16; ++ks) {
+                const uint64_t xh = gmma_desc(xb + ks * 256, 128, 1024);
+                const uint64_t xm = gmma_desc(xb + T::X_BYTES + ks * 256, 128, 1024);
+                wgmma_rs<TN>(acc, fl[ks], xh);
+                wgmma_rs<TN>(acc, fh[ks], xm);
+                wgmma_rs<TN>(acc, fh[ks], xh);
+            }
+            wgmma_commit();
+            acc_fence(acc);
+        }
+        wgmma_wait<0>();
         acc_fence(acc);
-        wgmma_fence();
-#pragma unroll
-        for (int ks = 0; ks < G5_BK / 16; ++ks) {
-            const uint32_t koff = (uint32_t)ks * 2u * lbo;
-            const uint64_t whi = gmma_desc(wbase + 0 * G5_TILE_BYTES + koff, lbo, sbo);
-            const uint64_t wlo = gmma_desc(wbase + 1 * G5_TILE_BYTES + koff, lbo, sbo);
-            const uint64_t xh = gmma_desc(xbase + 0 * G5_TILE_BYTES + koff, lbo, sbo);
-            const uint64_t xm = gmma_desc(xbase + 1 * G5_TILE_BYTES + koff, lbo, sbo);
-            wgmma_m64n64k16(acc, wlo, xh);
-            wgmma_m64n64k16(acc, whi, xm);
-            wgmma_m64n64k16(acc, whi, xh);
-        }
-        wgmma_commit();
-        acc_fence(acc);
-    }
-    wgmma_wait<0>();
-    acc_fence(acc);
-
-    {
-        __shared__ int is_last;
-        const int frow = fq * 64 + (warp & 3) * 16 + (lane >> 2);
-        const int tcol = tq * 64 + (lane & 3) * 2;
-        auto fr = [&](int i) { return frow + ((i >> 1) & 1) * 8; };
-        auto tc = [&](int i) { return tcol + (i >> 2) * 8 + (i & 1); };
-        auto emit = [&](float (&r)[32]) {
-#pragma unroll
-            for (int i = 0; i < 32; ++i) {
+        if (nk > 0) {
+            __syncwarp();
+            if (lane == 0) mbar_arrive(&empty[(it - 1) % S]);
+        }
+
+        const int f0 = ft * G5_BM + cw * 64, tok0 = tt * TN;
+        auto fr = [&](int i) { return warp * 16 + g + ((i >> 1) & 1) * 8; };
+        auto tc = [&](int i) { return (i >> 2) * 8 + t * 2 + (i & 1); };
+        auto emit = [&]() {
+#pragma unroll
+            for (int i = 0; i < TN / 2; ++i) {
                 const int feat = f0 + fr(i), tok = tok0 + tc(i);
-                float v = r[i] * a.oscale[tok];
+                float v = acc[i] * a.oscale[tok];
                 if (EPI == EPI_SILU_MUL) {
                     const float other = __shfl_xor_sync(0xffffffffu, v, 4);
-                    if (((lane >> 2) & 1) == 0 && tok < a.M && feat + 1 < a.N)
+                    if ((g & 1) == 0 && tok < a.M && feat + 1 < a.N)
                         a.y[(size_t)tok * a.ldy + (feat >> 1)] = (v / (1.0f + expf(-v))) * other;
                 } else if (tok < a.M && feat < a.N) {
                     if (a.bias) v += a.bias[feat];
@@ -227,42 +348,45 @@
             }
         };
         if (a.SK <= 1) {
-            emit(acc);
+            emit();
         } else {
-            const int tile_id = blockIdx.y * gridDim.x + blockIdx.x, n_tile = gridDim.x * gridDim.y;
-            float *ptile = a.partial + ((size_t)blockIdx.z * n_tile + tile_id) * (G5_BM * G5_BN);
-#pragma unroll
-            for (int i = 0; i < 32; ++i) __stcg(ptile + (size_t)tc(i) * G5_BM + fr(i), acc[i]);
-            __syncthreads();
-            if (tid == 0) {
+            const int ht = tile * 2 + cw;
+            const size_t half_el = (size_t)64 * TN;
+#pragma unroll
+            for (int i = 0; i < TN / 2; ++i)
+                __stcg(a.partial + ((size_t)z * tiles * 2 + ht) * half_el + (size_t)tc(i) * 64 + fr(i), acc[i]);
+            wg_sync(1 + cw);
+            if ((tid & 127) == 0) {
                 __threadfence();
-                const int old = atomicAdd(&a.counters[tile_id], 1);
+                const int old = atomicAdd(&a.counters[ht], 1);
                 const int last = (old == a.SK - 1);
                 if (last) {
-                    a.counters[tile_id] = 0;
+                    a.counters[ht] = 0;
                     __threadfence();
                 }
-                is_last = last;
-            }
-            __syncthreads();
-            if (is_last != 0) {
-#pragma unroll
-                for (int i = 0; i < 32; ++i) {
+                is_last[cw] = last;
+            }
+            wg_sync(1 + cw);
+            if (is_last[cw] != 0) {
+#pragma unroll
+                for (int i = 0; i < TN / 2; ++i) {
                     float v = 0.0f;
-                    for (int z = 0; z < a.SK; ++z)
-                        v += __ldcg(a.partial + ((size_t)z * n_tile + tile_id) * (G5_BM * G5_BN) + (size_t)tc(i) * G5_BM + fr(i));
+                    for (int zz = 0; zz < a.SK; ++zz)
+                        v += __ldcg(a.partial + ((size_t)zz * tiles * 2 + ht) * half_el + (size_t)tc(i) * 64 + fr(i));
                     acc[i] = v;
                 }
-                emit(acc);
-            }
-        }
-    }
-}
+                emit();
+            }
+        }
+    }
+}
+
+__device__ __forceinline__ int g5_src_base(int c) { return 32 * (c >> 2) + 16 * ((c >> 1) & 1) + 2 * (c & 1); }
 
 template <bool ROWS>
 __device__ __forceinline__ void split_tiles_body(const float *__restrict__ x, int M, int K, const float *__restrict__ gamma,
                                                  const float *__restrict__ ada_shared, const AdaRows &ada_rows, float eps,
-                                                 __half *__restrict__ xt, float *__restrict__ oscale, int TT, int KC, int BN) {
+                                                 __half *__restrict__ xt, float *__restrict__ oscale, int Mpad) {
     __shared__ float ssq_part[32][8], max_part[32][8];
     __shared__ float rms_s[8], sc_s[8];
     const int r8 = threadIdx.x & 7, cth = threadIdx.x >> 3;
@@ -311,20 +435,23 @@
         __syncthreads();
     }
     const float rms = rms_s[r8], sc = sc_s[r8];
-    const int tt = row / BN, rin = row % BN;
-    const size_t tile_el = (size_t)BN * G5_BK;
-    const size_t piece = (size_t)TT * KC * tile_el;
+    const size_t piece = (size_t)(K / G5_BK) * Mpad * G5_BK;
     for (int c = cth; c < nchunk; c += 32) {
+        const int k0 = (c >> 3) * G5_BK + g5_src_base(c & 7);
         float v[8] = {0.f, 0.f, 0.f, 0.f, 0.f, 0.f, 0.f, 0.f};
         if (valid) {
-            const float4 v0 = *reinterpret_cast<const float4 *>(xr + c * 8);
-            const float4 v1 = *reinterpret_cast<const float4 *>(xr + c * 8 + 4);
-            v[0] = v0.x; v[1] = v0.y; v[2] = v0.z; v[3] = v0.w; v[4] = v1.x; v[5] = v1.y; v[6] = v1.z; v[7] = v1.w;
+#pragma unroll
+            for (int m = 0; m < 4; ++m) {
+                const float2 p = *reinterpret_cast<const float2 *>(xr + k0 + 4 * m);
+                v[2 * m] = p.x;
+                v[2 * m + 1] = p.y;
+            }
             if (gamma) {
 #pragma unroll
                 for (int e = 0; e < 8; ++e) {
-                    v[e] = (v[e] / rms) * gamma[c * 8 + e];
-                    if (ada) v[e] *= ada[c * 8 + e];
+                    const int k = k0 + 4 * (e >> 1) + (e & 1);
+                    v[e] = (v[e] / rms) * gamma[k];
+                    if (ada) v[e] *= ada[k];
                 }
             }
         }
@@ -338,7 +465,7 @@
             p[0][e] = *reinterpret_cast<const uint32_t *>(&h);
             p[1][e] = *reinterpret_cast<const uint32_t *>(&m);
         }
-        const size_t off = ((size_t)tt * KC + (c >> 3)) * tile_el + (size_t)((c & 7) * BN + rin) * 8;
+        const size_t off = ((((size_t)(c >> 3) * (Mpad >> 3) + (row >> 3)) * 8 + (c & 7)) * 8 + (row & 7)) * 8;
 #pragma unroll
         for (int s = 0; s < G5_PIECES; ++s)
             *reinterpret_cast<uint4 *>(xt + s * piece + off) = make_uint4(p[s][0], p[s][1], p[s][2], p[s][3]);
@@ -347,99 +474,133 @@
 
 __global__ void __launch_bounds__(256) split_tiles_kernel(const float *__restrict__ x, int M, int K, const float *__restrict__ gamma,
                                                           const float *__restrict__ ada, float eps, __half *__restrict__ xt,
-                                                          float *__restrict__ oscale, int TT, int KC, int BN) {
-    split_tiles_body<false>(x, M, K, gamma, ada, AdaRows{}, eps, xt, oscale, TT, KC, BN);
+                                                          float *__restrict__ oscale, int Mpad) {
+    split_tiles_body<false>(x, M, K, gamma, ada, AdaRows{}, eps, xt, oscale, Mpad);
 }
 
 __global__ void __launch_bounds__(256) split_tiles_rows_kernel(const float *__restrict__ x, int M, int K, const float *__restrict__ gamma,
                                                                const AdaRows ada_rows, float eps, __half *__restrict__ xt,
-                                                               float *__restrict__ oscale, int TT, int KC, int BN) {
-    split_tiles_body<true>(x, M, K, gamma, nullptr, ada_rows, eps, xt, oscale, TT, KC, BN);
+                                                               float *__restrict__ oscale, int Mpad) {
+    split_tiles_body<true>(x, M, K, gamma, nullptr, ada_rows, eps, xt, oscale, Mpad);
+}
+
+constexpr int G5_TNS[] = {64, 128, 160, 192};
+
+int g5_mpad_max(int M) {
+    int p = 8;
+    for (int tn : G5_TNS) p = std::max(p, (M + tn - 1) / tn * tn);
+    return p;
+}
+
+struct G5Plan {
+    int TN, TT, SK, KCs;
+};
+G5Plan g5_plan(int N, int M, int KC, const GemmWork *gw) {
+    const int FT = N / G5_BM;
+    G5Plan best{0, 0, 0, 0};
+    double best_cost = 0.0;
+    for (int TN : G5_TNS) {
+        const int TT = (M + TN - 1) / TN, tiles = FT * TT;
+        for (int sk = 1; sk <= 8; ++sk) {
+            const int KCs = (KC + sk - 1) / sk, SK = (KC + KCs - 1) / KCs;
+            if (SK > 1 && (KCs < 4 || !gw || !gw->partial || !gw->counters || (size_t)SK * tiles * G5_BM * TN > gw->partial_floats ||
+                           tiles * 2 > gw->n_counters))
+                break;
+            const int units = tiles * SK, waves = (units + VOX_NUM_SMS - 1) / VOX_NUM_SMS;
+            const double cost = (double)waves * (KCs + 1 + (SK > 1 ? 2 : 0)) * (TN + 64);
+            if (best.TN == 0 || cost < best_cost) {
+                best = G5Plan{TN, TT, SK, KCs};
+                best_cost = cost;
+            }
+        }
+    }
+    return best;
 }
 
 }
 
 bool gemm_tc5_supported(const Q4Weight &w, int M) { return w.N % G5_BM == 0 && w.K % G5_BK == 0 && M >= 1; }
 
-static size_t g5_tiles_elems(int M, int K) {
-    const size_t TT = (size_t)(M + G5_BN - 1) / G5_BN;
-    return G5_PIECES * TT * (size_t)(K / G5_BK) * ((size_t)G5_BN * G5_BK);
-}
-size_t gemm_tc5_split_elems(int M, int K) {
-    const size_t TT = (size_t)(M + G5_BN - 1) / G5_BN;
-    return g5_tiles_elems(M, K) + 2 * TT * G5_BN + 16;
+static size_t g5_tiles_elems(int Mpad, int K) { return G5_PIECES * (size_t)Mpad * (size_t)K; }
+size_t gemm_tc5_split_elems(int M, int K) { return g5_tiles_elems(g5_mpad_max(M), K) + 2 * (size_t)g5_mpad_max(M) + 16; }
+int gemm_tc5_rows(const Q4Weight &w, int M, const GemmWork *gw) {
+    const G5Plan p = g5_plan(w.N, M, w.K / G5_BK, gw);
+    return p.TT * p.TN;
 }
 GemmWork gemm_tc5_work_size() {
     GemmWork w;
-    w.partial_floats = (size_t)VOX_NUM_SMS * G5_BM * G5_BN;
-    w.n_counters = 128;
+    w.partial_floats = (size_t)VOX_NUM_SMS * G5_BM * 128;
+    w.n_counters = 2 * VOX_NUM_SMS;
     return w;
 }
-static float *g5_oscale_ptr(void *xt, int M, int K) {
-    size_t off = g5_tiles_elems(M, K) * 2;
+static float *g5_oscale_ptr(void *xt, int Mpad, int K) {
+    size_t off = g5_tiles_elems(Mpad, K) * 2;
     off = (off + 15) & ~(size_t)15;
     return reinterpret_cast<float *>(reinterpret_cast<unsigned char *>(xt) + off);
 }
 
-void launch_split_tiles(const float *x, int M, int K, const float *gamma, const float *ada, float eps, void *xt,
+void launch_split_tiles(const float *x, int M, int Mpad, int K, const float *gamma, const float *ada, float eps, void *xt,
                         cudaStream_t st, const AdaRows &ada_rows) {
     VOX_CHECK(K % G5_BK == 0, VOX_EINVAL, "split_tiles: K=%d not a multiple of 64", K);
-    const int TT = (M + G5_BN - 1) / G5_BN, KC = K / G5_BK;
+    VOX_CHECK(Mpad >= M && Mpad % 8 == 0 && Mpad <= g5_mpad_max(M), VOX_EINVAL, "split_tiles: %d rows cannot hold M=%d", Mpad, M);
     if (ada_rows.rows)
-        split_tiles_rows_kernel<<<TT * (G5_BN / 8), 256, 0, st>>>(x, M, K, gamma, ada_rows, eps, (__half *)xt, g5_oscale_ptr(xt, M, K),
-                                                                  TT, KC, G5_BN);
+        split_tiles_rows_kernel<<<Mpad / 8, 256, 0, st>>>(x, M, K, gamma, ada_rows, eps, (__half *)xt, g5_oscale_ptr(xt, Mpad, K), Mpad);
     else
-        split_tiles_kernel<<<TT * (G5_BN / 8), 256, 0, st>>>(x, M, K, gamma, ada, eps, (__half *)xt, g5_oscale_ptr(xt, M, K), TT, KC,
-                                                             G5_BN);
+        split_tiles_kernel<<<Mpad / 8, 256, 0, st>>>(x, M, K, gamma, ada, eps, (__half *)xt, g5_oscale_ptr(xt, Mpad, K), Mpad);
     tc_count_launch("split_tiles");
 }
 
 void launch_q4_gemm_tc5(const Q4Weight &w, const void *xt, int M, float *y, int ldy, const float *bias, const float *res,
                         int epi, const GemmWork *gw, cudaStream_t st) {
     VOX_CHECK(gemm_tc5_supported(w, M), VOX_EINVAL, "gemm_tc5: unsupported shape N=%d K=%d", w.N, w.K);
+    VOX_CHECK(w.qs_tc && w.d_tc, VOX_EINVAL, "gemm_tc5: weight N=%d K=%d has no tensor-core layout", w.N, w.K);
     G5Args a{};
-    a.qs = w.qs;
-    a.ds = w.d;
+    a.qs_tc = w.qs_tc;
+    a.d_tc = w.d_tc;
     a.N = w.N;
     a.K = w.K;
     a.M = M;
     a.xt = (const __half *)xt;
-    a.oscale = g5_oscale_ptr(const_cast<void *>(xt), M, w.K);
-    a.TT = (M + G5_BN - 1) / G5_BN;
     a.KC = w.K / G5_BK;
     a.y = y;
     a.ldy = ldy;
     a.bias = bias;
     a.res = res;
-    const size_t smem = (size_t)G5_SMEM_BYTES;
-    const int tiles = (w.N / G5_BM) * a.TT;
-    int SK = 1;
-    if (gw && gw->partial && gw->counters && tiles < VOX_NUM_SMS * 2 / 3) {
-        SK = VOX_NUM_SMS / tiles;
-        SK = SK > 8 ? 8 : SK;
-        while (SK > 1 && a.KC / SK < 4) --SK;
-        while (SK > 1 && ((size_t)SK * tiles * G5_BM * G5_BN > gw->partial_floats || tiles > gw->n_counters)) --SK;
-    }
-    a.KCs = (a.KC + SK - 1) / SK;
-    SK = (a.KC + a.KCs - 1) / a.KCs;
-    a.SK = SK;
-    a.partial = SK > 1 ? gw->partial : nullptr;
-    a.counters = SK > 1 ? gw->counters : nullptr;
-    dim3 grid(w.N / G5_BM, a.TT, SK);
-#define G5_CASE(E)                                                                      \
-    case E: {                                                                           \
-        static SmemAttr attr;                                                           \
-        smem_attr_check(ensure_dyn_smem(gemm_tc5_kernel<E>, smem, attr), "gemm_tc5");   \
-        gemm_tc5_kernel<E><<<grid, G5_THREADS, smem, st>>>(a);                          \
-        break;                                                                          \
-    }
-    switch (epi) {
-        G5_CASE(EPI_NONE)
-        G5_CASE(EPI_RESIDUAL)
-        G5_CASE(EPI_SILU_MUL)
-        G5_CASE(EPI_GELU)
-        default: fail(VOX_EINVAL, "bad epilogue");
-    }
+    const G5Plan p = g5_plan(w.N, M, a.KC, gw);
+    a.Mpad = p.TT * p.TN;
+    a.oscale = g5_oscale_ptr(const_cast<void *>(xt), a.Mpad, w.K);
+    a.FT = w.N / G5_BM;
+    a.TT = p.TT;
+    a.SK = p.SK;
+    a.KCs = p.KCs;
+    a.partial = p.SK > 1 ? gw->partial : nullptr;
+    a.counters = p.SK > 1 ? gw->counters : nullptr;
+    const int units = a.FT * a.TT * a.SK, grid = std::min(units, VOX_NUM_SMS);
+#define G5_CASE(TN, E)                                                                                    \
+    case E: {                                                                                             \
+        static SmemAttr attr;                                                                             \
+        smem_attr_check(ensure_dyn_smem(gemm_tc5_kernel<TN, E>, G5Tile<TN>::SMEM_BYTES, attr), "gemm_tc5"); \
+        gemm_tc5_kernel<TN, E><<<grid, G5_THREADS, G5Tile<TN>::SMEM_BYTES, st>>>(a);                      \
+        break;                                                                                            \
+    }
+#define G5_TN(TN)                                 \
+    case TN:                                      \
+        switch (epi) {                            \
+            G5_CASE(TN, EPI_NONE)                 \
+            G5_CASE(TN, EPI_RESIDUAL)             \
+            G5_CASE(TN, EPI_SILU_MUL)             \
+            G5_CASE(TN, EPI_GELU)                 \
+            default: fail(VOX_EINVAL, "bad epilogue"); \
+        }                                         \
+        break;
+    switch (p.TN) {
+        G5_TN(64)
+        G5_TN(128)
+        G5_TN(160)
+        G5_TN(192)
+        default: fail(VOX_EINVAL, "gemm_tc5: no token tile");
+    }
+#undef G5_TN
 #undef G5_CASE
     tc_count_launch("gemm_tc5");
 }
diff --git a/voxtral_mini_realtime_rs_b200/csrc/kernels.cu b/voxtral_mini_realtime_rs_b200/csrc/kernels.cu
--- a/voxtral_mini_realtime_rs_b200/csrc/kernels.cu
+++ b/voxtral_mini_realtime_rs_b200/csrc/kernels.cu
@@ -461,11 +461,11 @@
                       const Q4Path &path, cudaStream_t st, const AdaRows &ada_rows) {
     VOX_CHECK(!ada_rows.rows || (gamma && !ada), VOX_EINVAL, "q4_linear: per-row ADA vectors need a norm and no shared vector");
     if (M > 8 && path.gemm_tc && gemm_tc5_supported(w, M) && gemm_tc5_split_elems(M, w.K) <= sc.xt_elems) {
-        launch_split_tiles(x, M, w.K, gamma, ada, gamma ? eps : 0.0f, sc.xt, st, ada_rows);
+        launch_split_tiles(x, M, gemm_tc5_rows(w, M, sc.gw), w.K, gamma, ada, gamma ? eps : 0.0f, sc.xt, st, ada_rows);
         launch_q4_gemm_tc5(w, sc.xt, M, y, ldy, bias, res, epi, sc.gw, st);
         return;
     }
-    const bool tc = M <= 8 && path.matvec_tc && w.qs_tc;
+    const bool tc = M <= 8 && path.matvec_tc && w.matvec_tc;
     AdaRows rows = ada_rows;
     if (gamma && !(tc && sc.tc && sc.tc->ssq_in)) {
         launch_rmsnorm(x, gamma, ada, tmp, M, w.K, eps, st, rows);
diff --git a/voxtral_mini_realtime_rs_b200/csrc/kernels.h b/voxtral_mini_realtime_rs_b200/csrc/kernels.h
--- a/voxtral_mini_realtime_rs_b200/csrc/kernels.h
+++ b/voxtral_mini_realtime_rs_b200/csrc/kernels.h
@@ -35,6 +35,7 @@
     const __half *d = nullptr;
     const uint4 *qs_tc = nullptr;
     const uint2 *d_tc = nullptr;
+    bool matvec_tc = false;
     int N = 0, K = 0;
     size_t bytes() const { return (size_t)N * (K / 32) * 18; }
 };
@@ -96,7 +97,9 @@
                     const float *res, int epi, cudaStream_t st);
 bool gemm_tc5_supported(const Q4Weight &w, int M);
 size_t gemm_tc5_split_elems(int M, int K);
-void launch_split_tiles(const float *x, int M, int K, const float *gamma, const float *ada, float eps, void *xt,
+struct GemmWork;
+int gemm_tc5_rows(const Q4Weight &w, int M, const GemmWork *gw);
+void launch_split_tiles(const float *x, int M, int Mpad, int K, const float *gamma, const float *ada, float eps, void *xt,
                         cudaStream_t st, const AdaRows &ada_rows = AdaRows{});
 struct GemmWork {
     float *partial = nullptr;
diff --git a/voxtral_mini_realtime_rs_b200/csrc/model.cu b/voxtral_mini_realtime_rs_b200/csrc/model.cu
--- a/voxtral_mini_realtime_rs_b200/csrc/model.cu
+++ b/voxtral_mini_realtime_rs_b200/csrc/model.cu
@@ -58,7 +58,7 @@
                             const std::vector<uint16_t> &ds);
 
 Q4Weight upload_q4(DeviceArena &arena, const std::vector<const uint8_t *> &raw, const std::vector<int> &n_rows,
-                   int K, bool interleave, bool tc_layout) {
+                   int K, bool interleave, Q4Layout layout) {
     VOX_CHECK(K % 32 == 0, VOX_EINVAL, "Q4 weight with K=%d (not a multiple of 32)", K);
     const int bpr = K / 32;
     int N = 0;
@@ -85,7 +85,8 @@
     w.K = K;
     w.qs = (const uint4 *)arena.upload(qs.data(), qs.size());
     w.d = (const __half *)arena.upload(ds.data(), ds.size());
-    if (tc_layout) build_tc_layout(arena, w, qs, ds);
+    if (layout != Q4_PLAIN) build_tc_layout(arena, w, qs, ds);
+    w.matvec_tc = layout == Q4_TC;
     return w;
 }
 
@@ -185,20 +186,20 @@
         q4_bytes += raw.size();
         return raw;
     }
-    Q4Weight q4(const std::string &name, int N, int K, bool tc = false) {
+    Q4Weight q4(const std::string &name, int N, int K, Q4Layout layout = Q4_PLAIN) {
         std::vector<uint8_t> raw = q4_raw(name, N, K);
-        return upload_q4(m.arena, {raw.data()}, {N}, K, false, tc);
-    }
-    Q4Weight q4_concat(const std::vector<std::string> &names, const std::vector<int> &ns, int K, bool tc = false) {
+        return upload_q4(m.arena, {raw.data()}, {N}, K, false, layout);
+    }
+    Q4Weight q4_concat(const std::vector<std::string> &names, const std::vector<int> &ns, int K, Q4Layout layout = Q4_PLAIN) {
         std::vector<std::vector<uint8_t>> raws;
         std::vector<const uint8_t *> ptrs;
         for (size_t i = 0; i < names.size(); ++i) raws.push_back(q4_raw(names[i], ns[i], K));
         for (auto &r : raws) ptrs.push_back(r.data());
-        return upload_q4(m.arena, ptrs, ns, K, false, tc);
-    }
-    Q4Weight q4_interleave(const std::string &a, const std::string &b, int N, int K, bool tc = false) {
+        return upload_q4(m.arena, ptrs, ns, K, false, layout);
+    }
+    Q4Weight q4_interleave(const std::string &a, const std::string &b, int N, int K, Q4Layout layout = Q4_PLAIN) {
         std::vector<uint8_t> ra = q4_raw(a, N, K), rb = q4_raw(b, N, K);
-        return upload_q4(m.arena, {ra.data(), rb.data()}, {N, N}, K, true, tc);
+        return upload_q4(m.arena, {ra.data(), rb.data()}, {N, N}, K, true, layout);
     }
     std::vector<float> bias_or_zero(const std::string &name, int n) {
         if (has(name)) return f32(name, {n});
@@ -310,29 +311,29 @@
             l.attn_norm = L.f32_dev(p + ".attention_norm.weight", {d});
             l.ffn_norm = L.f32_dev(p + ".ffn_norm.weight", {d});
             l.wqkv = L.q4_concat({p + ".attention.wq.weight", p + ".attention.wk.weight", p + ".attention.wv.weight"},
-                                 {hdq, hdq, hdq}, d);
+                                 {hdq, hdq, hdq}, d, Q4_TC_GEMM);
             std::vector<float> bq = L.bias_or_zero(p + ".attention.wq.bias", hdq);
             std::vector<float> bv = L.bias_or_zero(p + ".attention.wv.bias", hdq);
             std::vector<float> bqkv((size_t)3 * hdq, 0.0f);
             memcpy(bqkv.data(), bq.data(), sizeof(float) * hdq);
             memcpy(bqkv.data() + 2 * hdq, bv.data(), sizeof(float) * hdq);
             l.bqkv = m.arena.upload(bqkv.data(), bqkv.size());
-            l.wo = L.q4(p + ".attention.wo.weight", d, hdq);
+            l.wo = L.q4(p + ".attention.wo.weight", d, hdq, Q4_TC_GEMM);
             std::vector<float> bo = L.bias_or_zero(p + ".attention.wo.bias", d);
             l.bo = m.arena.upload(bo.data(), bo.size());
-            l.w13 = L.q4_interleave(p + ".feed_forward.w1.weight", p + ".feed_forward.w3.weight", c.enc_ffn, d);
-            l.w2 = L.q4(p + ".feed_forward.w2.weight", d, c.enc_ffn);
+            l.w13 = L.q4_interleave(p + ".feed_forward.w1.weight", p + ".feed_forward.w3.weight", c.enc_ffn, d, Q4_TC_GEMM);
+            l.w2 = L.q4(p + ".feed_forward.w2.weight", d, c.enc_ffn, Q4_TC_GEMM);
             std::vector<float> b2 = L.bias_or_zero(p + ".feed_forward.w2.bias", d);
             l.b2 = m.arena.upload(b2.data(), b2.size());
         }
         m.enc_norm = L.f32_dev(E + ".transformer.norm.weight", {d});
-        m.adapter0 = L.q4(std::string(kAdapter) + ".0.weight", D, d * c.reshape_factor);
-        m.adapter2 = L.q4(std::string(kAdapter) + ".2.weight", D, D);
+        m.adapter0 = L.q4(std::string(kAdapter) + ".0.weight", D, d * c.reshape_factor, Q4_TC_GEMM);
+        m.adapter2 = L.q4(std::string(kAdapter) + ".2.weight", D, D, Q4_TC_GEMM);
         {
             const GgufTensorInfo &t = L.info(kTokEmb);
             VOX_CHECK(t.dtype == VOX_DTYPE_Q4_0, VOX_EFORMAT,
                       "tok_embeddings must be Q4_0 in this build (got dtype %u)", t.dtype);
-            m.tok_emb = L.q4(kTokEmb, c.vocab, D, true);
+            m.tok_emb = L.q4(kTokEmb, c.vocab, D, Q4_TC);
         }
         const int qd = c.dec_heads * c.dec_head_dim, kvd = c.dec_kv_heads * c.dec_head_dim;
         m.dec.resize(c.dec_layers);
@@ -346,10 +347,10 @@
             l.attn_norm = L.f32_dev(p + ".attention_norm.weight", {D});
             l.ffn_norm = L.f32_dev(p + ".ffn_norm.weight", {D});
             l.wqkv = L.q4_concat({p + ".attention.wq.weight", p + ".attention.wk.weight", p + ".attention.wv.weight"},
-                                 {qd, kvd, kvd}, D, true);
-            l.wo = L.q4(p + ".attention.wo.weight", D, qd, true);
-            l.w13 = L.q4_interleave(p + ".feed_forward.w1.weight", p + ".feed_forward.w3.weight", c.dec_ffn, D, true);
-            l.w2 = L.q4(p + ".feed_forward.w2.weight", D, c.dec_ffn, true);
+                                 {qd, kvd, kvd}, D, Q4_TC);
+            l.wo = L.q4(p + ".attention.wo.weight", D, qd, Q4_TC);
+            l.w13 = L.q4_interleave(p + ".feed_forward.w1.weight", p + ".feed_forward.w3.weight", c.dec_ffn, D, Q4_TC);
+            l.w2 = L.q4(p + ".feed_forward.w2.weight", D, c.dec_ffn, Q4_TC);
             dec_q4 += L.q4_bytes - before;
         }
         m.dec_norm = L.f32_dev(kFinalNorm, {D});
diff --git a/voxtral_mini_realtime_rs_b200/csrc/model.h b/voxtral_mini_realtime_rs_b200/csrc/model.h
--- a/voxtral_mini_realtime_rs_b200/csrc/model.h
+++ b/voxtral_mini_realtime_rs_b200/csrc/model.h
@@ -79,8 +79,9 @@
 
 void rope_rows(int hd, float theta, int64_t p0, int n, float *cos_out, float *sin_out);
 
+enum Q4Layout { Q4_PLAIN, Q4_TC_GEMM, Q4_TC };
 Q4Weight upload_q4(DeviceArena &arena, const std::vector<const uint8_t *> &raw, const std::vector<int> &n_rows,
-                   int K, bool interleave, bool tc_layout = false);
+                   int K, bool interleave, Q4Layout layout = Q4_PLAIN);
 
 constexpr float kDefaultDelay = 6.0f;
 
```
